# sj-shoff/ImageProcessor

Hardware: AMD Instinct MI355X
Metric: images/sec (resize+thumb+watermark) on 1080p batch at 1/2/4/8 MI355X (higher is better)
Workload: dtype f32+f64

## Files before the change

imageprocessor_amd/__init__.py:

```python
import ctypes as C

import numpy as np

from . import _lib
from ._lib import Config, Glyph, PlanInfo, PlanParams, Rect

OP_OVER = 0
DEEP_NRGBA64, DEEP_RGBA64, DEEP_GRAY16, DEEP_CMYK = 0, 1, 2, 3
PNG_GRAY, PNG_NRGBA, PNG_RGBA, PNG_PALETTED, PNG_GRAY16, PNG_RGBA64, PNG_NRGBA64 = range(7)
OP_SRC = 1
YCBCR_444, YCBCR_422, YCBCR_420, YCBCR_440, GRAY, YCBCR_411, YCBCR_410 = range(7)


class IpxError(RuntimeError):
    def __init__(self, status, text):
        super().__init__("ipx status %d: %s" % (status, text))
        self.status = status
        self.text = text


def lib():
    return _lib.load()


def _check(rc):
    if rc < 0:
        raise IpxError(rc, lib().ipx_last_error().decode(errors="replace"))
    return rc


def _rect(r):
    return r if isinstance(r, Rect) else Rect(*[int(v) for v in r])


def _bytes_array(files):
    keep = [bytes(f) for f in files]
    arr = (_lib.Bytes * max(len(keep), 1))()
    for i, f in enumerate(keep):
        arr[i].data = C.cast(C.c_char_p(f), C.c_void_p)
        arr[i].len = len(f)
    arr._keep = keep
    return arr


def _rows(a):
    a = np.asarray(a, dtype=np.uint8)
    row = int(np.prod(a.shape[1:]))
    if a.ndim < 2 or not a[:1].flags.c_contiguous or (a.shape[0] > 1 and a.strides[0] < row):
        a = np.ascontiguousarray(a)
    return a, (a.strides[0] if a.shape[0] > 1 else row)


def _frame(a):
    a, stride = _rows(a)
    if a.ndim != 3 or a.shape[2] != 4:
        raise ValueError("RGBA8 frame must be H x W x 4")
    return a, stride


def _dst(dst, shape=None):
    assert isinstance(dst, np.ndarray) and dst.dtype == np.uint8 and dst.ndim == 3 and dst.shape[2] == 4 and dst.flags.writeable
    assert shape is None or dst.shape == shape
    d, stride = _rows(dst)
    assert d is dst, "the destination's rows must be contiguous and strides[0] at least a row"
    return stride



def resize_dims(ow, oh, w, h, keep_aspect):
    nw, nh = C.c_int(), C.c_int()
    _check(lib().ipx_resize_dims(ow, oh, w, h, int(bool(keep_aspect)), C.byref(nw), C.byref(nh)))
    return nw.value, nh.value


def thumb_geometry(ow, oh, size, crop_to_fit):
    r, nw, nh = Rect(), C.c_int(), C.c_int()
    _check(lib().ipx_thumb_geometry(ow, oh, size, int(bool(crop_to_fit)), C.byref(r), C.byref(nw),
                                    C.byref(nh)))
    return (r.x0, r.y0, r.x1, r.y1), nw.value, nh.value


def text_height_px(font_size):
    return lib().ipx_text_height_px(float(font_size))


def watermark_anchor(position, w, h, width_px, height_px):
    px, py = C.c_int(), C.c_int()
    _check(lib().ipx_watermark_anchor(position.encode(), w, h, width_px, height_px, C.byref(px),
                                      C.byref(py)))
    return px.value, py.value


def parse_color(s, opacity):
    out = (C.c_uint8 * 4)()
    rc = _check(lib().ipx_parse_color(s.encode(), float(opacity), out))
    return tuple(out), rc == 1


def device_count():
    return lib().ipx_device_count()


def _glyph_array(glyphs):
    keep = []
    arr = (Glyph * max(1, len(glyphs)))()
    for i, g in enumerate(glyphs):
        m, mstride = _rows(g["mask"])
        if m.ndim != 2:
            raise ValueError("glyph mask must be mh x mw")
        keep.append(m)
        mp = g.get("mp", (0, 0))
        arr[i] = Glyph(m.ctypes.data, m.shape[1], m.shape[0], mstride, _rect(g["dr"]), int(mp[0]),
                       int(mp[1]))
    return arr, keep


def _text_array(texts):
    keep = []
    arr = (_lib.Text * max(1, len(texts)))()
    for i, (glyphs, col) in enumerate(texts):
        glyphs = list(glyphs)
        ga, gk = _glyph_array(glyphs)
        keep.append((ga, gk))
        arr[i].glyphs = ga if glyphs else None
        arr[i].n_glyphs = len(glyphs)
        for c in range(4):
            arr[i].col[c] = int(col[c])
    return arr, keep



class DevBuffer:

    def __init__(self, ctx, nbytes):
        self.ctx, self.nbytes = ctx, int(nbytes)
        self.ptr = lib().ipx_dev_alloc(ctx.handle, max(1, self.nbytes))
        if not self.ptr:
            raise IpxError(-2, lib().ipx_last_error().decode())

    def upload(self, arr, offset=0):
        arr = np.ascontiguousarray(arr)
        assert offset + arr.nbytes <= self.nbytes
        _check(lib().ipx_memcpy_h2d(self.ctx.handle, self.ptr + offset, arr.ctypes.data, arr.nbytes))
        return self

    def download(self, shape, dtype=np.uint8, offset=0):
        out = np.empty(shape, dtype)
        assert offset + out.nbytes <= self.nbytes
        _check(lib().ipx_memcpy_d2h(self.ctx.handle, out.ctypes.data, self.ptr + offset, out.nbytes))
        return out

    def free(self):
        if self.ptr:
            lib().ipx_dev_free(self.ctx.handle, self.ptr)
            self.ptr = None

    def __del__(self):
        try:
            self.free()
        except Exception:
            pass


class GlyphSet:

    def __init__(self, ctx, glyphs, col):
        self.ctx = ctx
        arr, keep = _glyph_array(list(glyphs))
        c = (C.c_uint8 * 4)(*[int(v) for v in col])
        h = C.c_void_p()
        _check(lib().ipx_glyphset_create(ctx.handle, arr, len(glyphs), c, C.byref(h)))
        self.handle = h.value

    def close(self):
        if self.handle:
            lib().ipx_glyphset_destroy(self.ctx.handle, self.handle)
            self.handle = None

    def __del__(self):
        try:
            self.close()
        except Exception:
            pass


class TextSet:

    def __init__(self, ctx, texts, w, h, stream=None):
        self.ctx = ctx
        texts = list(texts)
        arr, keep = _text_array(texts)
        hd = C.c_void_p()
        _check(lib().ipx_textset_create(ctx.handle, stream, arr, len(texts), int(w), int(h), C.byref(hd)))
        self.handle, self.n, self.w, self.h = hd.value, len(texts), int(w), int(h)

    def close(self):
        if self.handle:
            lib().ipx_textset_destroy(self.ctx.handle, self.handle)
            self.handle = None

    def __del__(self):
        try:
            self.close()
        except Exception:
            pass


class Plan:

    def __init__(self, ctx, sw, sh, resize=(1024, 768, True), thumbnail=(200, True), watermark=None):
        self.ctx = ctx
        self._sw, self._sh = sw, sh
        p = PlanParams()
        p.sw, p.sh = sw, sh
        if resize:
            p.do_resize, p.resize_w, p.resize_h, p.keep_aspect = 1, resize[0], resize[1], int(bool(resize[2]))
        if thumbnail:
            p.do_thumbnail, p.thumb_size, p.crop_to_fit = 1, thumbnail[0], int(bool(thumbnail[1]))
        self._gs = None
        if watermark is not None and watermark is not False:
            p.do_watermark = 1
            if isinstance(watermark, GlyphSet):
                self._gs = watermark
                p.glyphs = watermark.handle
        h = C.c_void_p()
        _check(lib().ipx_plan_create(ctx.handle, C.byref(p), C.byref(h)))
        self.handle = h.value
        self.info = PlanInfo()
        _check(lib().ipx_plan_query(self.handle, C.byref(self.info)))

    def _run(self, entry, head, n, src, ptrs, strides=(None, None, None)):
        i = self.info
        fs = [d if s is None else s for s, d in zip(strides, (i.resize_bytes, i.thumb_bytes, i.wm_bytes))]
        _check(entry(self.ctx.handle, *head, self.handle, n, *src, ptrs[0], fs[0], ptrs[1], fs[1], ptrs[2], fs[2]))

    def _run_host(self, entry, n, src, want, out=None):
        i = self.info
        out = dict(out) if out else {}
        for k, nbytes, h, w in (("resize", i.resize_bytes, i.resize_h, i.resize_w), ("thumbnail", i.thumb_bytes, i.thumb_h, i.thumb_w),
                                ("watermark", i.wm_bytes, i.wm_h, i.wm_w)):
            if k in want and nbytes and k not in out:
                out[k] = np.empty((n, h, w, 4), np.uint8)
        self._run(entry, (), n, src, [out[k].ctypes.data if k in out else None for k in ("resize", "thumbnail", "watermark")])
        return out

    def run_dev(self, n, src_ptr, resize_ptr=None, thumb_ptr=None, wm_ptr=None, stream=None,
                sstride=None, src_frame_stride=None, resize_frame_stride=None,
                thumb_frame_stride=None, wm_frame_stride=None):
        sstride = self._sw * 4 if sstride is None else sstride
        self._run(lib().ipx_plan_run_dev, (stream,), n,
                  (src_ptr, sstride, sstride * self._sh if src_frame_stride is None else src_frame_stride),
                  (resize_ptr, thumb_ptr, wm_ptr), (resize_frame_stride, thumb_frame_stride, wm_frame_stride))

    def run_host(self, frames, want=("resize", "thumbnail", "watermark"), out=None):
        frames = np.ascontiguousarray(frames, dtype=np.uint8)
        return self._run_host(lib().ipx_plan_run_host, frames.shape[0], (frames.ctypes.data, self._sw * 4, self._sw * self._sh * 4), want, out)

    def run_host_nrgba(self, frames, want=("resize", "thumbnail", "watermark")):
        frames = np.ascontiguousarray(frames, dtype=np.uint8)
        return self._run_host(lib().ipx_plan_run_host_nrgba, frames.shape[0], (frames.ctypes.data, self._sw * 4, self._sw * self._sh * 4), want)

    def run_host_deep(self, pix, kind, want=("resize", "thumbnail", "watermark")):
        pix = np.ascontiguousarray(pix, dtype=np.uint8)
        return self._run_host(lib().ipx_plan_run_host_deep, pix.shape[0], (kind, pix.ctypes.data, pix.shape[2], pix.shape[1] * pix.shape[2]), want)

    def run_host_gray(self, frames, want=("resize", "thumbnail", "watermark")):
        frames = np.ascontiguousarray(frames, dtype=np.uint8)
        return self._run_host(lib().ipx_plan_run_host_gray, frames.shape[0], (frames.ctypes.data, self._sw, self._sw * self._sh), want)

    def run_host_paletted(self, index, palettes, want=("resize", "thumbnail", "watermark")):
        index = np.ascontiguousarray(index, dtype=np.uint8)
        palettes = np.ascontiguousarray(palettes, dtype=np.uint8)
        n = index.shape[0]
        assert palettes.shape == (n, 256, 4)
        return self._run_host(lib().ipx_plan_run_host_paletted, n, (index.ctypes.data, self._sw, self._sw * self._sh, palettes.ctypes.data), want)

    def _run_streams(self, entry, n, want, copy, args, status=None):
        i = self.info
        arrs = {k: (_lib.Bytes * max(n, 1))() for k, present in (("resize", i.resize_bytes), ("thumbnail", i.thumb_bytes),
                                                                  ("watermark", i.wm_bytes)) if k in want and present}
        res = C.c_void_p()
        extra = () if status is None else (status,)
        _check(entry(self.ctx.handle, self.handle, n, *args, arrs.get("resize"), arrs.get("thumbnail"), arrs.get("watermark"), *extra,
                     C.byref(res)))
        out = {k: [(C.string_at(a[j].data, a[j].len) if copy else a[j].len) if a[j].data else None for j in range(n)]
               for k, a in arrs.items()}
        lib().ipx_jpeg_result_free(self.ctx.handle, res)
        return out

    def _run_files(self, entry, files, want, copy, args=()):
        n = len(files)
        status = (C.c_int * max(n, 1))()
        out = self._run_streams(entry, n, want, copy, (_bytes_array(files),) + args, status)
        return out, list(status)[:n]

    def run_host_jpeg(self, frames, quality=85, want=("resize", "thumbnail", "watermark"), copy=True):
        frames = np.ascontiguousarray(frames, dtype=np.uint8)
        return self._run_streams(lib().ipx_plan_run_host_jpeg, frames.shape[0], want, copy,
                                 (frames.ctypes.data, self._sw * 4, self._sw * self._sh * 4, int(quality)))

    def run_host_paletted_gif(self, index, palettes, quality=85, want=("resize", "thumbnail", "watermark"), copy=True):
        index = np.ascontiguousarray(index, dtype=np.uint8)
        palettes = np.ascontiguousarray(palettes, dtype=np.uint8)
        n = index.shape[0]
        assert index.shape[1:] == (self._sh, self._sw) and palettes.shape == (n, 256, 4)
        return self._run_streams(lib().ipx_plan_run_host_paletted_gif, n, want, copy,
                                 (index.ctypes.data, self._sw, self._sw * self._sh, palettes.ctypes.data, int(quality)))

    def run_host_png(self, frames, want=("resize", "thumbnail", "watermark"), copy=True):
        frames = np.ascontiguousarray(frames, dtype=np.uint8)
        assert frames.shape[1:] == (self._sh, self._sw, 4)
        return self._run_streams(lib().ipx_plan_run_host_png, frames.shape[0], want, copy,
                                 (frames.ctypes.data, self._sw * 4, self._sw * self._sh * 4))

# ... 720 lines not shown
```

imageprocessor_amd/_lib.py:

```python
import ctypes as C
import importlib.util
import os

HERE = os.path.dirname(os.path.abspath(__file__))
LIB_PATH = os.environ.get("IPX_LIB") or os.path.join(HERE, "libipx.so")


class Rect(C.Structure):
    _fields_ = [("x0", C.c_int32), ("y0", C.c_int32), ("x1", C.c_int32), ("y1", C.c_int32)]


class Glyph(C.Structure):
    _fields_ = [("mask", C.c_void_p), ("mw", C.c_int32), ("mh", C.c_int32), ("mstride", C.c_int32),
                ("dr", Rect), ("mpx", C.c_int32), ("mpy", C.c_int32)]


class Text(C.Structure):
    _fields_ = [("glyphs", C.POINTER(Glyph)), ("n_glyphs", C.c_int32), ("col", C.c_uint8 * 4)]


class Config(C.Structure):
    _fields_ = [("device", C.c_int32), ("lanes", C.c_int32), ("lane_bytes", C.c_size_t)]


class PlanParams(C.Structure):
    _fields_ = [("sw", C.c_int32), ("sh", C.c_int32),
                ("do_resize", C.c_int32), ("resize_w", C.c_int32), ("resize_h", C.c_int32),
                ("keep_aspect", C.c_int32),
                ("do_thumbnail", C.c_int32), ("thumb_size", C.c_int32), ("crop_to_fit", C.c_int32),
                ("do_watermark", C.c_int32), ("glyphs", C.c_void_p)]


class PlanInfo(C.Structure):
    _fields_ = [("resize_w", C.c_int32), ("resize_h", C.c_int32),
                ("thumb_w", C.c_int32), ("thumb_h", C.c_int32), ("thumb_crop", Rect),
                ("wm_w", C.c_int32), ("wm_h", C.c_int32),
                ("resize_bytes", C.c_size_t), ("thumb_bytes", C.c_size_t), ("wm_bytes", C.c_size_t),
                ("algorithmic_bytes", C.c_size_t)]


class YCbCr(C.Structure):
    _fields_ = [("y", C.c_void_p), ("cb", C.c_void_p), ("cr", C.c_void_p), ("ystride", C.c_int32),
                ("cstride", C.c_int32), ("w", C.c_int32), ("h", C.c_int32), ("ratio", C.c_int32)]


class YCbCrBatch(C.Structure):
    _fields_ = [("y", C.c_void_p), ("cb", C.c_void_p), ("cr", C.c_void_p), ("ystride", C.c_int32),
                ("cstride", C.c_int32), ("y_frame_stride", C.c_size_t), ("c_frame_stride", C.c_size_t),
                ("ratio", C.c_int32)]


class CmykBatch(C.Structure):
    _fields_ = [("pix", C.c_void_p), ("stride", C.c_int32), ("frame_stride", C.c_size_t)]


class PalettedBatch(C.Structure):
    _fields_ = [("index", C.c_void_p), ("stride", C.c_int32), ("frame_stride", C.c_size_t), ("palettes", C.c_void_p)]


class PngBatch(C.Structure):
    _fields_ = [("pix", C.c_void_p), ("stride", C.c_int32), ("frame_stride", C.c_size_t), ("palettes", C.c_void_p)]


class Param(C.Structure):
    _fields_ = [("key", C.c_char_p), ("type", C.c_int32), ("f64", C.c_double), ("i64", C.c_int64),
                ("str", C.c_char_p)]


class Image(C.Structure):
    _fields_ = [("pix", C.c_void_p), ("w", C.c_int32), ("h", C.c_int32), ("stride", C.c_int32)]


MEASURE_FN = C.CFUNCTYPE(C.c_int, C.c_void_p, C.c_char_p, C.c_double, C.POINTER(C.c_int))
GLYPHS_FN = C.CFUNCTYPE(C.c_int, C.c_void_p, C.c_char_p, C.c_double, C.c_int, C.c_int, C.c_int, C.c_int,
                        C.POINTER(C.POINTER(Glyph)), C.POINTER(C.c_int))
RELEASE_FN = C.CFUNCTYPE(None, C.c_void_p)


class Bytes(C.Structure):
    _fields_ = [("data", C.c_void_p), ("len", C.c_size_t)]


class TextRasterizer(C.Structure):
    _fields_ = [("user", C.c_void_p), ("measure", MEASURE_FN), ("glyphs", GLYPHS_FN), ("release", RELEASE_FN)]


class Operation(C.Structure):
    _fields_ = [("type", C.c_char_p), ("params", C.POINTER(Param)), ("nparams", C.c_int32)]


class Task(C.Structure):
    _fields_ = [("id", C.c_char_p), ("image_id", C.c_char_p), ("ops", C.POINTER(Operation)),
                ("nops", C.c_int32), ("format", C.c_char_p)]


class Processed(C.Structure):
    _fields_ = [("operation", C.c_char * 16), ("path", C.c_char * 320), ("content_type", C.c_char * 32),
                ("format", C.c_char * 8), ("image", Image)]


class PoolConfig(C.Structure):
    _fields_ = [("lanes_per_device", C.c_int32), ("lane_bytes", C.c_size_t)]


class PoolOps(C.Structure):
    _fields_ = [("sw", C.c_int32), ("sh", C.c_int32),
                ("do_resize", C.c_int32), ("resize_w", C.c_int32), ("resize_h", C.c_int32), ("keep_aspect", C.c_int32),
                ("do_thumbnail", C.c_int32), ("thumb_size", C.c_int32), ("crop_to_fit", C.c_int32),
                ("do_watermark", C.c_int32), ("glyphs", C.POINTER(Glyph)), ("n_glyphs", C.c_int32), ("col", C.c_uint8 * 4)]


class Job(C.Structure):
    _fields_ = [("kind", C.c_int32), ("ops", PoolOps), ("n", C.c_int32),
                ("src", C.c_void_p), ("sstride", C.c_int32), ("src_frame_stride", C.c_size_t),
                ("resize_out", C.c_void_p), ("resize_frame_stride", C.c_size_t),
                ("thumb_out", C.c_void_p), ("thumb_frame_stride", C.c_size_t),
                ("wm_out", C.c_void_p), ("wm_frame_stride", C.c_size_t),
                ("files", C.POINTER(Bytes)), ("quality", C.c_int32),
                ("resize_jpeg", C.POINTER(Bytes)), ("thumb_jpeg", C.POINTER(Bytes)), ("wm_jpeg", C.POINTER(Bytes)),
                ("status", C.POINTER(C.c_int32)), ("texts", C.POINTER(Text))]


class BatcherConfig(C.Structure):
    _fields_ = [("max_batch", C.c_int32), ("max_wait_us", C.c_int32), ("quality", C.c_int32)]


class BatchResult(C.Structure):
    _fields_ = [("status", C.c_int32), ("resize", Bytes), ("thumb", Bytes), ("wm", Bytes)]


class BatcherStats(C.Structure):
    _fields_ = [(k, C.c_longlong) for k in ("files", "batches", "flushed_by_size", "flushed_by_timer", "largest_batch", "pending_files", "flushed_when_idle")]


_P = C.c_void_p
_I = C.c_int
_Z = C.c_size_t

SIGNATURES = {
    "ipx_create": (_I, [C.POINTER(Config), C.POINTER(_P)]),
    "ipx_destroy": (None, [_P]),
    "ipx_last_error": (C.c_char_p, []),
    "ipx_abi_version": (_I, []),
    "ipx_device_count": (_I, []),
    "ipx_frame_supported": (_I, [_I, _I, C.c_longlong, _I]),
    "ipx_resize_dims": (_I, [_I, _I, _I, _I, _I, C.POINTER(_I), C.POINTER(_I)]),
    "ipx_thumb_geometry": (_I, [_I, _I, _I, _I, C.POINTER(Rect), C.POINTER(_I), C.POINTER(_I)]),
    "ipx_text_height_px": (_I, [C.c_double]),
    "ipx_watermark_anchor": (_I, [C.c_char_p, _I, _I, _I, _I, C.POINTER(_I), C.POINTER(_I)]),
    "ipx_parse_color": (_I, [C.c_char_p, C.c_double, _P]),
    "ipx_host_alloc": (_P, [_P, _Z]),
    "ipx_host_free": (_I, [_P, _P]),
    "ipx_dev_alloc": (_P, [_P, _Z]),
    "ipx_dev_free": (_I, [_P, _P]),
    "ipx_memcpy_h2d": (_I, [_P, _P, _P, _Z]),
    "ipx_memcpy_d2h": (_I, [_P, _P, _P, _Z]),
    "ipx_memcpy_d2d": (_I, [_P, _P, _P, _Z]),
    "ipx_stream_copy": (_I, [_P, _P, _P, _P, _Z]),
    "ipx_device_sync": (_I, [_P]),
    "ipx_stream_sync": (_I, [_P, _P]),
    "ipx_stream_create": (_P, [_P]),
    "ipx_stream_destroy": (_I, [_P, _P]),
    "ipx_scale_bilinear_rgba8": (_I, [_P, _P, _I, _I, _I, Rect, _P, _I, _I, _I, Rect, _I]),
    "ipx_draw_rgba8": (_I, [_P, _P, _I, _I, _I, Rect, _P, _I, _I, _I, _I, _I, _I]),
    "ipx_composite_glyphs_rgba8": (_I, [_P, _P, _I, _I, _I, C.POINTER(Glyph), _I, _P]),
    "ipx_scale_bilinear_nrgba8": (_I, [_P, _P, _I, _I, _I, Rect, _P, _I, _I, _I, Rect, _I]),
    "ipx_draw_nrgba8": (_I, [_P, _P, _I, _I, _I, Rect, _P, _I, _I, _I, _I, _I, _I]),
    "ipx_scale_bilinear_deep": (_I, [_P, _P, _I, _I, _I, Rect, _P, _I, _I, _I, _I, Rect, _I]),
    "ipx_draw_deep": (_I, [_P, _P, _I, _I, _I, Rect, _P, _I, _I, _I, _I, _I, _I, _I]),
    "ipx_scale_bilinear_ycbcr": (_I, [_P, _P, _I, _I, _I, Rect, C.POINTER(YCbCr), Rect]),
    "ipx_draw_ycbcr": (_I, [_P, _P, _I, _I, _I, Rect, C.POINTER(YCbCr), _I, _I]),
    "ipx_dev_scale_bilinear_rgba8": (_I, [_P, _P, _P, _I, _I, _I, Rect, _P, _I, _I, _I, Rect, _I]),
    "ipx_dev_draw_rgba8": (_I, [_P, _P, _P, _I, _I, _I, Rect, _P, _I, _I, _I, _I, _I, _I]),
    "ipx_glyphset_create": (_I, [_P, C.POINTER(Glyph), _I, _P, C.POINTER(_P)]),
    "ipx_glyphset_destroy": (None, [_P, _P]),
    "ipx_dev_composite_glyphs_rgba8": (_I, [_P, _P, _P, _I, _I, _I, _P]),
    "ipx_textset_create": (_I, [_P, _P, C.POINTER(Text), _I, _I, _I, C.POINTER(_P)]),
    "ipx_textset_destroy": (None, [_P, _P]),
    "ipx_dev_composite_texts_rgba8": (_I, [_P, _P, _P, _I, _I, _I, _Z, _I, _P, _I, C.POINTER(C.c_int32)]),
    "ipx_plan_create": (_I, [_P, C.POINTER(PlanParams), C.POINTER(_P)]),
    "ipx_plan_destroy": (None, [_P, _P]),
    "ipx_plan_query": (_I, [_P, C.POINTER(PlanInfo)]),
    "ipx_plan_run_dev": (_I, [_P, _P, _P, _I, _P, _I, _Z, _P, _Z, _P, _Z, _P, _Z]),
    "ipx_plan_run_host": (_I, [_P, _P, _I, _P, _I, _Z, _P, _Z, _P, _Z, _P, _Z]),
    "ipx_plan_run_dev_ycbcr": (_I, [_P, _P, _P, _I, C.POINTER(YCbCrBatch), _P, _Z, _P, _Z, _P, _Z]),
    "ipx_plan_run_dev_gray": (_I, [_P, _P, _P, _I, _P, _I, _Z, _P, _Z, _P, _Z, _P, _Z]),
    "ipx_plan_run_dev_paletted": (_I, [_P, _P, _P, _I, _P, _I, _Z, _P, _P, _Z, _P, _Z, _P, _Z]),
    "ipx_plan_run_host_nrgba": (_I, [_P, _P, _I, _P, _I, _Z, _P, _Z, _P, _Z, _P, _Z]),
    "ipx_plan_run_host_gray": (_I, [_P, _P, _I, _P, _I, _Z, _P, _Z, _P, _Z, _P, _Z]),
    "ipx_plan_run_host_paletted": (_I, [_P, _P, _I, _P, _I, _Z, _P, _P, _Z, _P, _Z, _P, _Z]),
    "ipx_plan_run_dev_nrgba": (_I, [_P, _P, _P, _I, _P, _I, _Z, _P, _Z, _P, _Z, _P, _Z]),
    "ipx_plan_run_dev_deep": (_I, [_P, _P, _P, _I, _I, _P, _I, _Z, _P, _Z, _P, _Z, _P, _Z]),
    "ipx_plan_run_host_deep": (_I, [_P, _P, _I, _I, _P, _I, _Z, _P, _Z, _P, _Z, _P, _Z]),
    "ipx_plan_run_host_ycbcr": (_I, [_P, _P, _I, C.POINTER(YCbCrBatch), _P, _Z, _P, _Z, _P, _Z]),
    "ipx_event_create": (_P, [_P]),
    "ipx_event_record": (_I, [_P, _P, _P]),
    "ipx_event_elapsed_ms": (_I, [_P, _P, _P, C.POINTER(C.c_float)]),
    "ipx_event_destroy": (None, [_P, _P]),
    "ipx_image_free": (None, [C.POINTER(Image)]),
    "ipx_resizer_process": (_I, [_P, C.POINTER(Image), C.c_char_p, C.POINTER(Param), _I, C.POINTER(Image), _P]),
    "ipx_thumbnailer_process": (_I, [_P, C.POINTER(Image), C.c_char_p, C.POINTER(Param), _I, C.POINTER(Image), _P]),
    "ipx_watermarker_process": (_I, [_P, C.POINTER(Image), C.c_char_p, C.POINTER(Param), _I,
                                     C.POINTER(TextRasterizer), C.POINTER(Image), _P]),
    "ipx_processor_process": (_I, [_P, C.POINTER(Task), C.POINTER(Image), C.c_char_p, C.POINTER(TextRasterizer),
                                   C.POINTER(Processed), C.POINTER(_I)]),
    "ipx_jpeg_coef_count": (_Z, [_I, _I]),
    "ipx_jpeg_quant_tables": (_I, [_I, _P]),
    "ipx_dev_jpeg_fdct_rgba8": (_I, [_P, _P, _P, _I, _I, _I, _Z, _I, _I, _P]),
    "ipx_jpeg_entropy_encode": (_I, [_P, _I, _I, _I, C.POINTER(_P), C.POINTER(_Z)]),
    "ipx_jpeg_encode_rgba8": (_I, [_P, _P, _I, _I, _I, _I, C.POINTER(_P), C.POINTER(_Z)]),
    "ipx_jpeg_encode_batch_dev": (_I, [_P, _P, _I, _I, _I, _Z, _I, _I, C.POINTER(_P), C.POINTER(_Z), C.POINTER(_Z)]),
    "ipx_buffer_free": (None, [_P]),
    "ipx_jpeg_decode_batch": (_I, [_P, _P, C.POINTER(Bytes), _I, C.POINTER(_I), C.POINTER(_I), C.POINTER(YCbCrBatch), C.POINTER(_I),
                                   C.POINTER(_P)]),
    "ipx_jpeg_planes_free": (None, [_P, _P]),
    "ipx_jpeg_scan_route": (_I, [_P, _Z, C.POINTER(_I)]),
    "ipx_jpeg_decode_counts": (_I, [_P, C.POINTER(C.c_longlong)]),
    "ipx_png_decode_counts": (_I, [_P, C.POINTER(C.c_longlong)]),
    "ipx_jpeg_decode_batch_cmyk": (_I, [_P, _P, C.POINTER(Bytes), _I, C.POINTER(_I), C.POINTER(_I), C.POINTER(CmykBatch), C.POINTER(_I),
                                        C.POINTER(_P)]),
    "ipx_jpeg_cmyk_files": (_I, [_P, C.POINTER(C.c_longlong)]),
    "ipx_plan_run_jpeg_jpeg": (_I, [_P, _P, _I, C.POINTER(Bytes), _I, C.POINTER(Bytes), C.POINTER(Bytes), C.POINTER(Bytes), C.POINTER(_I),
                                    C.POINTER(_P)]),
    "ipx_plan_run_host_jpeg": (_I, [_P, _P, _I, _P, _I, _Z, _I, C.POINTER(Bytes), C.POINTER(Bytes), C.POINTER(Bytes), C.POINTER(_P)]),
    "ipx_jpeg_result_free": (None, [_P, _P]),
    "ipx_plan_run_host_ycbcr_jpeg": (_I, [_P, _P, _I, C.POINTER(YCbCrBatch), _I, C.POINTER(Bytes), C.POINTER(Bytes), C.POINTER(Bytes),
                                          C.POINTER(_P)]),
    "ipx_gif_encode_rgba8": (_I, [_P, _P, _I, _I, _I, C.POINTER(_P), C.POINTER(_Z)]),
    "ipx_gif_encode_batch_dev": (_I, [_P, _P, _I, _I, _I, _Z, _I, C.POINTER(_P), C.POINTER(_Z), C.POINTER(_Z)]),
    "ipx_dev_gif_dither_rgba8": (_I, [_P, _P, _P, _I, _I, _I, _Z, _I, _P]),
    "ipx_plan_run_host_paletted_gif": (_I, [_P, _P, _I, _P, _I, _Z, _P, _I, C.POINTER(Bytes), C.POINTER(Bytes), C.POINTER(Bytes),
                                            C.POINTER(_P)]),
    "ipx_png_encode_rgba8": (_I, [_P, _P, _I, _I, _I, C.POINTER(_P), C.POINTER(_Z)]),
    "ipx_png_encode_batch_dev": (_I, [_P, _P, _I, _I, _I, _Z, _I, C.POINTER(_P), C.POINTER(_Z), C.POINTER(_Z)]),
    "ipx_plan_run_host_png": (_I, [_P, _P, _I, _P, _I, _Z, C.POINTER(Bytes), C.POINTER(Bytes), C.POINTER(Bytes), C.POINTER(_P)]),
    "ipx_gif_decode_batch": (_I, [_P, _P, C.POINTER(Bytes), _I, C.POINTER(_I), C.POINTER(_I), C.POINTER(PalettedBatch), C.POINTER(_I),
                                  C.POINTER(_P)]),
    "ipx_gif_frames_free": (None, [_P, _P]),
    "ipx_plan_run_gif_gif": (_I, [_P, _P, _I, C.POINTER(Bytes), _I, C.POINTER(Bytes), C.POINTER(Bytes), C.POINTER(Bytes), C.POINTER(_I),
                                  C.POINTER(_P)]),
    "ipx_png_decode_batch": (_I, [_P, _P, C.POINTER(Bytes), _I, C.POINTER(_I), C.POINTER(_I), C.POINTER(_I), C.POINTER(PngBatch),
                                  C.POINTER(_I), C.POINTER(_P)]),
    "ipx_png_frames_free": (None, [_P, _P]),
    "ipx_plan_run_png_png": (_I, [_P, _P, _I, C.POINTER(Bytes), C.POINTER(Bytes), C.POINTER(Bytes), C.POINTER(Bytes), C.POINTER(_I),
                                  C.POINTER(_P)]),
    "ipx_plan_run_jpeg_jpeg_texts": (_I, [_P, _P, _I, C.POINTER(Bytes), C.POINTER(Text), _I, C.POINTER(Bytes), C.POINTER(Bytes),
                                          C.POINTER(Bytes), C.POINTER(_I), C.POINTER(_P)]),
    "ipx_plan_run_png_png_texts": (_I, [_P, _P, _I, C.POINTER(Bytes), C.POINTER(Text), C.POINTER(Bytes), C.POINTER(Bytes), C.POINTER(Bytes),
                                        C.POINTER(_I), C.POINTER(_P)]),
    "ipx_plan_run_gif_gif_texts": (_I, [_P, _P, _I, C.POINTER(Bytes), C.POINTER(Text), _I, C.POINTER(Bytes), C.POINTER(Bytes),
                                        C.POINTER(Bytes), C.POINTER(_I), C.POINTER(_P)]),
    "ipx_font_create": (_I, [_P, _Z, C.POINTER(_P)]),
    "ipx_font_destroy": (None, [_P]),
    "ipx_font_glyph_index": (_I, [_P, C.c_uint32]),
    "ipx_font_glyph_advance": (_I, [_P, C.c_uint32, C.c_double, C.POINTER(C.c_int32)]),
    "ipx_font_kern": (_I, [_P, C.c_uint32, C.c_uint32, C.c_double, C.POINTER(C.c_int32)]),
    "ipx_font_text_width": (_I, [_P, C.c_char_p, C.c_double, C.POINTER(C.c_int32), C.POINTER(_I)]),
    "ipx_font_draw_string": (_I, [_P, C.c_char_p, C.c_double, _I, _I, _I, _I, C.POINTER(C.POINTER(Glyph)),
                                  C.POINTER(_I), C.POINTER(C.c_int32)]),
    "ipx_font_release_thread": (None, []),
    "ipx_font_rasterizer": (_I, [_P, C.POINTER(TextRasterizer)]),
    "ipx_pool_create": (_I, [C.POINTER(_I), _I, C.POINTER(PoolConfig), C.POINTER(_P)]),
    "ipx_pool_destroy": (None, [_P]),
    "ipx_pool_slots": (_I, [_P]),
    "ipx_pool_frames_done": (C.c_longlong, [_P, _I]),
    "ipx_pool_png_decode_counts": (_I, [_P, _I, C.POINTER(C.c_longlong)]),
    "ipx_pool_host_alloc": (_P, [_P, _I, _Z]),
    "ipx_pool_host_free": (_I, [_P, _I, _P]),
    "ipx_job_submit": (_I, [_P, C.POINTER(Job), C.POINTER(C.c_uint64)]),
    "ipx_job_poll": (_I, [_P, C.c_uint64, C.POINTER(_I)]),
    "ipx_job_wait": (_I, [_P, C.c_uint64, C.POINTER(_I)]),
    "ipx_job_release": (_I, [_P, C.c_uint64]),
    "ipx_pool_run_host": (_I, [_P, C.POINTER(Job), _I]),
    "ipx_plan_acquire": (_I, [_P, C.POINTER(PoolOps), C.POINTER(_P), C.POINTER(_I)]),
    "ipx_plan_release": (None, [_P, _P, _I]),
    "ipx_link_probe": (_I, [_P, _Z, _Z, _I, C.POINTER(C.c_double * 4)]),
    "ipx_batcher_create": (_I, [_P, C.POINTER(BatcherConfig), C.POINTER(_P)]),
    "ipx_batcher_destroy": (None, [_P]),
    "ipx_batcher_submit": (_I, [_P, C.POINTER(Bytes), C.POINTER(PoolOps), C.POINTER(C.c_uint64)]),
    "ipx_batcher_wait": (_I, [_P, C.c_uint64, C.POINTER(BatchResult)]),
    "ipx_batcher_release": (_I, [_P, C.c_uint64]),
    "ipx_batcher_get_stats": (_I, [_P, C.POINTER(BatcherStats)]),
}

_lib = None


def _preload_hip_runtime():
    if os.environ.get("IPX_SYSTEM_HIP") == "1":
        return
    try:
        spec = importlib.util.find_spec("torch")
    except (ImportError, ValueError):
        spec = None
    if spec is None or not spec.origin:
        return
    cand = os.path.join(os.path.dirname(spec.origin), "lib", "libamdhip64.so")
    if os.path.exists(cand):
        C.CDLL(cand, mode=C.RTLD_GLOBAL)


def load():
    global _lib
    if _lib is not None:
        return _lib
    if not os.path.exists(LIB_PATH):
        raise ImportError(
            "imageprocessor_amd: %s is missing -- build the HIP extension first "
            "(python imageprocessor_amd/build.py, or __graft_entry__.build()). "
            "There is no CPU fallback for the pixel path." % LIB_PATH)
    _preload_hip_runtime()
    L = C.CDLL(LIB_PATH)
    for name, (res, args) in SIGNATURES.items():
        fn = getattr(L, name)
        fn.restype = res
        fn.argtypes = args
    _lib = L
    return L
```

imageprocessor_amd/csrc/ipx_device.h:

```cpp
#pragma once

#include "ipx_internal.h"

namespace ipx {
namespace {

constexpr uint32_t kM = 0xffffu;

__device__ __forceinline__ uint32_t ycbcr_to_rgb8(uint32_t y, uint32_t cb, uint32_t cr)
{
    const int32_t yy1 = (int32_t)y * 0x10101, cb1 = (int32_t)cb - 128, cr1 = (int32_t)cr - 128;
    int32_t r = yy1 + 91881 * cr1, g = yy1 - 22554 * cb1 - 46802 * cr1, b = yy1 + 116130 * cb1;
    r = ((uint32_t)r & 0xff000000u) == 0 ? r >> 16 : ~(r >> 31);
    g = ((uint32_t)g & 0xff000000u) == 0 ? g >> 16 : ~(g >> 31);
    b = ((uint32_t)b & 0xff000000u) == 0 ? b >> 16 : ~(b >> 31);
    return ((uint32_t)r & 0xffu) | (((uint32_t)g & 0xffu) << 8) | (((uint32_t)b & 0xffu) << 16) | 0xff000000u;
}

template <int C>
__device__ __forceinline__ double widen(uint32_t px)
{
    constexpr uint32_t sel = 0x0c0c0000u | (uint32_t)C | ((uint32_t)C << 8);
    return (double)__builtin_amdgcn_perm(0u, px, sel);
}

template <int C>
__device__ __forceinline__ uint32_t lerp_channel(uint32_t p00, uint32_t p10, uint32_t p01,
                                                 uint32_t p11, double xw0, double xw1, double yw0,
                                                 double yw1)
{
    const double s00 = widen<C>(p00), s10 = widen<C>(p10);
    const double s01 = widen<C>(p01), s11 = widen<C>(p11);
    const double top = xw0 * s00 + xw1 * s10;
    const double bot = xw0 * s01 + xw1 * s11;
    const double v = yw0 * top + yw1 * bot;
    return (uint32_t)v;
}

__device__ __forceinline__ uint32_t pack_src(uint32_t pr, uint32_t pg, uint32_t pb, uint32_t pa)
{
    return (pr >> 8) | (pg & 0xff00u) | ((pb & 0xff00u) << 8) | ((pa & 0xff00u) << 16);
}

__device__ __forceinline__ uint32_t blend_over(uint32_t d, uint32_t pr, uint32_t pg, uint32_t pb,
                                               uint32_t pa)
{
    const uint32_t pa1 = (kM - pa) * 0x101u;
    const uint32_t r = (((d & 0xffu) * pa1 / kM + pr) >> 8) & 0xffu;
    const uint32_t g = ((((d >> 8) & 0xffu) * pa1 / kM + pg) >> 8) & 0xffu;
    const uint32_t b = ((((d >> 16) & 0xffu) * pa1 / kM + pb) >> 8) & 0xffu;
    const uint32_t a = (((d >> 24) * pa1 / kM + pa) >> 8) & 0xffu;
    return r | (g << 8) | (b << 16) | (a << 24);
}

__device__ __forceinline__ uint32_t glyph_over(uint32_t d, uint32_t mask8, uint32_t sr, uint32_t sg,
                                               uint32_t sb, uint32_t sa)
{
    const uint32_t ma = mask8 | (mask8 << 8);
    const uint32_t a = (kM - (sa * ma / kM)) * 0x101u;
    const uint32_t r = (((d & 0xffu) * a + sr * ma) / kM >> 8) & 0xffu;
    const uint32_t g = ((((d >> 8) & 0xffu) * a + sg * ma) / kM >> 8) & 0xffu;
    const uint32_t b = ((((d >> 16) & 0xffu) * a + sb * ma) / kM >> 8) & 0xffu;
    const uint32_t al = (((d >> 24) * a + sa * ma) / kM >> 8) & 0xffu;
    return r | (g << 8) | (b << 16) | (al << 24);
}

__device__ __forceinline__ uint32_t glyph_run(uint32_t d, int x, int y, const DevGlyph *__restrict__ gl,
                                              int n, uint32_t sr, uint32_t sg, uint32_t sb,
                                              uint32_t sa)
{
    for (int g = 0; g < n; g++) {
        const DevGlyph G = gl[g];
        if (x >= G.x0 && x < G.x1 && y >= G.y0 && y < G.y1) {
            const uint32_t m = G.mask[(size_t)(y - G.y0) * G.mstride + (x - G.x0)];
            if (m) d = glyph_over(d, m, sr, sg, sb, sa);
        }
    }
    return d;
}

template <int PX, int ROWS, int YSTEP>
__device__ __forceinline__ void glyph_walk(const DevGlyph *tab, int n, int x, int ybase, Rect bbox, uint32_t (&d)[ROWS][PX], uint32_t sr,
                                           uint32_t sg, uint32_t sb, uint32_t sa)
{
    static_assert(PX >= 1 && PX <= 4, "a row's mask bytes travel in one dword");
    for (int g = 0; g < n; g += 4) {
        uint32_t m[4][ROWS];
        bool any = false;
#pragma unroll
        for (int j = 0; j < 4; j++) {
            const DevGlyph G = tab[min(g + j, n - 1)];
#pragma unroll
            for (int r = 0; r < ROWS; r++) {
                const int y = ybase + YSTEP * r;
                const bool iny = g + j < n && y >= G.y0 && y < G.y1 && y < bbox.y1;
                uint32_t mm = 0u;
#pragma unroll
                for (int k = 0; k < PX; k++) {
                    const bool in = iny && x + k >= G.x0 && x + k < G.x1;
                    mm |= (in ? (uint32_t)G.mask[(size_t)(y - G.y0) * G.mstride + (x + k - G.x0)] : 0u) << (8 * k);
                    any |= in;
                }
                m[j][r] = mm;
            }
        }
        if (!__any(any)) continue;
#pragma unroll
        for (int j = 0; j < 4; j++)
#pragma unroll
            for (int r = 0; r < ROWS; r++)
#pragma unroll
                for (int k = 0; k < PX; k++) {
                    const uint32_t mk = (m[j][r] >> (8 * k)) & 0xffu;
                    if (mk) d[r][k] = glyph_over(d[r][k], mk, sr, sg, sb, sa);
                }
    }
}

}
}
```

imageprocessor_amd/csrc/ipx_host.cpp:

```cpp
#include <cmath>
#include <cstring>
#include <new>
#include <string>
#include <system_error>
#include <vector>

#include "ipx_internal.h"

namespace ipx {

static thread_local char g_err[512];

void set_error(const char *fmt, ...)
{
    va_list ap;
    va_start(ap, fmt);
    vsnprintf(g_err, sizeof g_err, fmt, ap);
    va_end(ap);
}
void clear_error() { g_err[0] = 0; }

int status_of_exception() noexcept
{
    try { throw; }
    catch (const std::bad_alloc &) { set_error("out of memory"); return IPX_ERR_NOMEM; }
    catch (const std::system_error &e) { set_error("system resource unavailable: %s", e.what()); return IPX_ERR_NOMEM; }
    catch (const std::exception &e) { set_error("internal error: %s", e.what()); return IPX_ERR_INVALID; }
    catch (...) { set_error("internal error"); return IPX_ERR_INVALID; }
}

Rect Rect::intersect(const Rect &s) const
{
    Rect r = *this;
    if (r.x0 < s.x0) r.x0 = s.x0;
    if (r.y0 < s.y0) r.y0 = s.y0;
    if (r.x1 > s.x1) r.x1 = s.x1;
    if (r.y1 > s.y1) r.y1 = s.y1;
    if (r.empty()) return Rect{0, 0, 0, 0};
    return r;
}

bool draw_clip(Rect &r, int dw, int dh, bool has_src, int sw, int sh, int &spx, int &spy,
               bool has_mask, int mw, int mh, int &mpx, int &mpy)
{
    const int ox = r.x0, oy = r.y0;
    r = r.intersect(Rect{0, 0, dw, dh});
    if (has_src) r = r.intersect(Rect{0, 0, sw, sh}.shifted(ox - spx, oy - spy));
    if (has_mask) r = r.intersect(Rect{0, 0, mw, mh}.shifted(ox - mpx, oy - mpy));
    if (r.empty()) return false;
    const int dx = r.x0 - ox, dy = r.y0 - oy;
    spx += dx; spy += dy;
    mpx += dx; mpy += dy;
    return true;
}

}

using namespace ipx;

extern "C" {

const char *ipx_last_error(void) { return g_err; }
int ipx_abi_version(void) { return IPX_ABI_VERSION; }

int ipx_frame_supported(int w, int h, long long stride, int bytes_per_pixel)
{
    clear_error();
    if (w < 0 || h < 0 || bytes_per_pixel <= 0 || stride < (long long)w * bytes_per_pixel) {
        set_error("ipx_frame_supported: bad argument");
        return IPX_ERR_INVALID;
    }
    if (frame_span_ok(w, h, stride, bytes_per_pixel)) return IPX_OK;
    set_error("a %dx%d frame (stride %lld) is beyond the 2 GiB / 65535-pixel span the kernels address", w, h, stride);
    return IPX_ERR_UNSUPPORTED;
}

int ipx_resize_dims(int ow, int oh, int w, int h, int keep_aspect, int *nw, int *nh)
{
    clear_error();
    if (!nw || !nh || ow <= 0 || oh <= 0) { set_error("ipx_resize_dims: bad argument"); return IPX_ERR_INVALID; }
    if (w <= 0 || h <= 0) { set_error("width and height must be positive numbers"); return IPX_ERR_INVALID; }
    if (keep_aspect) {
        const double wr = (double)w / (double)ow;
        const double hr = (double)h / (double)oh;
        const double ratio = std::fmin(wr, hr);
        *nw = (int)((double)ow * ratio);
        *nh = (int)((double)oh * ratio);
    } else {
        *nw = w;
        *nh = h;
    }
    return IPX_OK;
}

int ipx_thumb_geometry(int ow, int oh, int size, int crop_to_fit, ipx_rect *crop, int *nw, int *nh)
{
    clear_error();
    if (!crop || !nw || !nh || ow <= 0 || oh <= 0) { set_error("ipx_thumb_geometry: bad argument"); return IPX_ERR_INVALID; }
    if (size == 0) size = 200;
    if (size < 0) { set_error("size must be a positive number"); return IPX_ERR_INVALID; }
    if (crop_to_fit) {
        const int side = ow > oh ? oh : ow;
        const int cx = ow > oh ? (ow - oh) / 2 : 0;
        const int cy = ow > oh ? 0 : (oh - ow) / 2;
        *crop = ipx_rect{cx, cy, cx + side, cy + side};
        *nw = size;
        *nh = size;
    } else {
        *crop = ipx_rect{0, 0, ow, oh};
        if (ow > oh) {
            *nh = size;
            *nw = (int)((double)ow * (double)size / (double)oh);
        } else {
            *nw = size;
            *nh = (int)((double)oh * (double)size / (double)ow);
        }
    }
    return IPX_OK;
}

int ipx_text_height_px(double font_size)
{
    const int32_t h26_6 = (int32_t)(font_size * 64 * 1.2);
    return (h26_6 + 63) >> 6;
}

int ipx_watermark_anchor(const char *position, int w, int h, int width_px, int height_px, int *px,
                         int *py)
{
    clear_error();
    if (!position || !px || !py) { set_error("ipx_watermark_anchor: bad argument"); return IPX_ERR_INVALID; }
    enum { L, R, C } hx = R;
    enum { T, B, M } vy = B;
    const std::string p(position);
    if (p == "top-left") { hx = L; vy = T; }
    else if (p == "top-right") { hx = R; vy = T; }
    else if (p == "top-center") { hx = C; vy = T; }
    else if (p == "bottom-left") { hx = L; vy = B; }
    else if (p == "bottom-center") { hx = C; vy = B; }
    else if (p == "center") { hx = C; vy = M; }
    const int margin = 20;
    *px = hx == L ? margin : hx == R ? w - width_px - margin : (w - width_px) / 2;
    *py = vy == T ? margin + height_px : vy == B ? h - margin : (h + height_px) / 2;
    return IPX_OK;
}

static bool atoi_field(const std::string &f, long long *v)
{
    size_t i = 0;
    bool neg = false;
    if (f.empty()) return false;
    if (f[0] == '+' || f[0] == '-') { neg = f[0] == '-'; i = 1; }
    if (i == f.size()) return false;
    long long acc = 0;
    for (; i < f.size(); i++) {
        if (f[i] < '0' || f[i] > '9') return false;
        if (acc > 900000000000000000LL) return false;
        acc = acc * 10 + (f[i] - '0');
    }
    *v = neg ? -acc : acc;
    return true;
}

int ipx_parse_color(const char *s, double opacity, uint8_t rgba[4])
{
    clear_error();
    if (!s || !rgba) { set_error("ipx_parse_color: bad argument"); return IPX_ERR_INVALID; }
    const uint8_t alpha = (uint8_t)(int32_t)(255 * opacity);
    std::vector<std::string> parts(1);
    for (const char *c = s; *c; c++) {
        if (*c == ' ') continue;
        if (*c == ',') parts.emplace_back();
        else parts.back().push_back(*c);
    }
    long long v[4] = {0, 0, 0, 0};
    bool ok = parts.size() == 3 || parts.size() == 4;
    for (int i = 0; ok && i < 3; i++) ok = atoi_field(parts[i], &v[i]);
    if (!ok) {
        rgba[0] = rgba[1] = rgba[2] = 0;
        rgba[3] = alpha;
        return 1;
    }
    for (int i = 0; i < 3; i++) rgba[i] = (uint8_t)(v[i] < 0 ? 0 : v[i] > 255 ? 255 : v[i]);
    if (parts.size() == 4 && atoi_field(parts[3], &v[3])) rgba[3] = (uint8_t)(v[3] < 0 ? 0 : v[3] > 255 ? 255 : v[3]);
    else rgba[3] = alpha;
    return IPX_OK;
}

}
```

imageprocessor_amd/csrc/ipx_internal.h:

```cpp
#pragma once

#include <hip/hip_runtime.h>

#include <cstdarg>
#include <cstdint>
#include <cstdio>
#include <map>
#include <mutex>
#include <vector>

#include "../../include/ipx.h"

namespace ipx {

void set_error(const char *fmt, ...) __attribute__((format(printf, 1, 2)));
void clear_error();
int status_of_exception() noexcept;
#define IPX_CATCH_STATUS catch (...) { return ipx::status_of_exception(); }

#define IPX_HIP(call)                                                                        \
    do {                                                                                     \
        hipError_t e_ = (call);                                                              \
        if (e_ != hipSuccess) {                                                              \
            ipx::set_error("%s failed: %s (%s:%d)", #call, hipGetErrorString(e_), __FILE__,  \
                           __LINE__);                                                        \
            return IPX_ERR_HIP;                                                              \
        }                                                                                    \
    } while (0)

constexpr long long kMaxFrameSpan = 0x7fff0000LL;
constexpr int kMaxFrameSide = 65535;
inline bool frame_span_ok(long long w, long long h, long long stride, int bpp)
{
    if (w > kMaxFrameSide || h > kMaxFrameSide) return false;
    return w <= 0 || h <= 0 || (h - 1) * stride + w * bpp <= kMaxFrameSpan;
}

struct Rect {
    int x0, y0, x1, y1;
    int dx() const { return x1 - x0; }
    int dy() const { return y1 - y0; }
    bool empty() const { return x0 >= x1 || y0 >= y1; }
    Rect shifted(int ox, int oy) const { return Rect{x0 + ox, y0 + oy, x1 + ox, y1 + oy}; }
    Rect intersect(const Rect &s) const;
};
inline Rect to_rect(const ipx_rect &r) { return Rect{r.x0, r.y0, r.x1, r.y1}; }

bool draw_clip(Rect &r, int dw, int dh, bool has_src, int sw, int sh, int &spx, int &spy,
               bool has_mask, int mw, int mh, int &mpx, int &mpy);

enum SrcType { kSrcRGBA, kSrcNRGBA, kSrcGray, kSrcPaletted, kSrcYCbCr, kSrcNRGBA64, kSrcRGBA64, kSrcGray16, kSrcCMYK, kSrcTypes };
inline int src_bpp(int type) { static const int b[kSrcTypes] = {4, 4, 1, 1, 1, 8, 8, 2, 4}; return b[type]; }
inline int src_of_deep(int k) { return k >= IPX_DEEP_NRGBA64 && k <= IPX_DEEP_CMYK ? kSrcNRGBA64 + k : -1; }
inline int src_of_png(int k)
{
    static const int t[] = {kSrcGray, kSrcNRGBA, kSrcRGBA, kSrcPaletted, kSrcGray16, kSrcRGBA64, kSrcNRGBA64};
    return k >= 0 && k < 7 ? t[k] : -1;
}
inline int src_of_job(int k)
{
    static const int t[] = {kSrcRGBA, -1, kSrcNRGBA, kSrcGray, kSrcNRGBA64, kSrcRGBA64, kSrcGray16, kSrcCMYK};
    return k >= 0 && k < 8 ? t[k] : -1;
}
inline void chroma_size(int ratio, int w, int h, int *cw, int *ch)
{
    *cw = ratio == IPX_YCBCR_422 || ratio == IPX_YCBCR_420 ? (w + 1) / 2 : ratio == IPX_YCBCR_411 || ratio == IPX_YCBCR_410 ? (w + 3) / 4 : w;
    *ch = ratio == IPX_YCBCR_420 || ratio == IPX_YCBCR_440 || ratio == IPX_YCBCR_410 ? (h + 1) / 2 : h;
}
inline bool ycbcr_ratio_ok(int ratio) { return (ratio >= IPX_YCBCR_444 && ratio <= IPX_YCBCR_440) || ratio == IPX_YCBCR_411 || ratio == IPX_YCBCR_410; }
#if defined(__HIPCC__)
__host__ __device__
#endif
inline int ycbcr_hshift(int ratio) { return ratio == IPX_YCBCR_422 || ratio == IPX_YCBCR_420 ? 1 : ratio == IPX_YCBCR_411 || ratio == IPX_YCBCR_410 ? 2 : 0; }
#if defined(__HIPCC__)
__host__ __device__
#endif
inline int ycbcr_vshift(int ratio) { return ratio == IPX_YCBCR_420 || ratio == IPX_YCBCR_440 || ratio == IPX_YCBCR_410 ? 1 : 0; }
inline int ycbcr_ratio_of(int h0, int v0)
{
    return h0 == 4 ? (v0 == 1 ? IPX_YCBCR_411 : IPX_YCBCR_410) : h0 == 1 ? (v0 == 1 ? IPX_YCBCR_444 : IPX_YCBCR_440) : (v0 == 1 ? IPX_YCBCR_422 : IPX_YCBCR_420);
}

enum { IPX_SRC_RGBA = 0, IPX_SRC_NRGBA = 1, IPX_SRC_YCBCR = 2,
       IPX_SRC_TAP64 = 3  };
hipError_t launch_opaque_scan(const uint8_t *src, int sw, int sh, int sstride, int *flag,
                              hipStream_t s);
hipError_t launch_opaque_scan_tap64(const uint8_t *src, int sw, int sh, int sstride, int *flag, hipStream_t s);
hipError_t launch_draw(uint8_t *dst, int dstride, const uint8_t *src, int sstride, int w, int h,
                       int op, hipStream_t s);
hipError_t launch_draw_nrgba(uint8_t *dst, int dstride, const uint8_t *src, int sstride, int w, int h, int op,
                             hipStream_t s, int nframes = 1, size_t dst_fs = 0, size_t src_fs = 0);
hipError_t launch_deep_expand(uint8_t *dst, size_t dst_fs, const uint8_t *src, int sstride, size_t src_fs, int kind, int w, int h, int nframes, hipStream_t s);
hipError_t launch_draw_tap64(uint8_t *dst, int dstride, const uint8_t *src, int sstride, int w, int h, int op, hipStream_t s,
                             int nframes = 1, size_t dst_fs = 0, size_t src_fs = 0);
hipError_t launch_draw_ycbcr(uint8_t *dst, int dstride, const uint8_t *y, int ystride, const uint8_t *cb,
                             const uint8_t *cr, int cstride, int ratio, int spx, int spy, int w, int h, hipStream_t s,
                             int nframes = 1, size_t dst_fs = 0, size_t y_fs = 0, size_t c_fs = 0);

struct DevGlyph {
    const uint8_t *mask;
    int mstride;
    int x0, y0, x1, y1;
};
constexpr int kMaxGlyphs = 256;
hipError_t launch_stream_copy(void *dst, const void *src, size_t bytes, hipStream_t s);
hipError_t launch_composite(uint8_t *dst, int dstride, size_t frame_stride, int nframes,
                            const DevGlyph *glyphs_dev, int n, Rect bbox, uint32_t sr, uint32_t sg,
                            uint32_t sb, uint32_t sa, hipStream_t s);
struct DevText {
    int first, n;
    Rect bbox;
    uint16_t col[4];
};
hipError_t launch_composite_texts(uint8_t *dst, int dstride, size_t frame_stride, int nframes, const DevText *texts_dev,
                                  const DevGlyph *glyphs_dev, const int *map_dev, int first, int bw, int bh, hipStream_t s);

hipError_t launch_gray_expand(uint8_t *dst, size_t dst_fs, const uint8_t *src, int sstride, size_t src_fs, int w, int h, int n, hipStream_t s);
hipError_t launch_palette_expand(uint8_t *dst, size_t dst_fs, const uint8_t *src, int sstride, size_t src_fs, const uint8_t *palettes, int w,
                                 int h, int n, hipStream_t s);

struct KernelLaunchCache {
    std::mutex mu;
    size_t lds_max = 0;
    std::map<size_t, int> resident;
    bool said = false;
    hipError_t prepare(const void *fn, int threads, size_t lds, int *res)
    {
        std::lock_guard<std::mutex> lk(mu);
        if (lds > lds_max) {
            hipError_t e = hipFuncSetAttribute(fn, hipFuncAttributeMaxDynamicSharedMemorySize, (int)lds);
            if (e != hipSuccess) return e;
            lds_max = lds;
        }
        if (res) {
            auto it = resident.find(lds);
            if (it == resident.end()) {
                int n = 0;
                hipError_t e = hipOccupancyMaxActiveBlocksPerMultiprocessor(&n, fn, threads, lds);
                if (e != hipSuccess) return e;
                it = resident.emplace(lds, n > 1 ? n : 1).first;
            }
            *res = it->second;
        }
        return hipSuccess;
    }
    bool first_report() { std::lock_guard<std::mutex> lk(mu); const bool f = !said; said = true; return f; }
};


struct JpegTables {
    uint8_t quant[2][64];
    uint16_t div8[2][64];
    uint32_t recip[2][64];
};
void jpeg_tables(int quality, JpegTables *t);
struct JpegArgs {
    const uint8_t *src; size_t frame_stride; int stride, w, h;
    int aligned16;
    int16_t *coefs; int mcus_per_frame;
    const uint32_t *huff;
    uint32_t *aclen;
    int16_t *dcq;
    uint32_t recip[2][64];
    uint16_t div8[2][64];
};
hipError_t launch_jpeg_fdct(const JpegArgs &a, int n, hipStream_t s);


struct JpegDecInfo {
    int w, h, h0, v0, ratio, ri, ncomp;
    int host_scans;
    int progressive;
    int gpu_scans;
    uint8_t td[3], ta[3];
    size_t scan_off, scan_len;
};
struct JpegDecTables {
    uint16_t lut[4][256];
    int32_t maxcode[4][18];
    int32_t valoff[4][18];
    uint8_t vals[4][256];
    uint16_t qnat[3][64];
    uint32_t bound[4][8];
};
struct JpegDecImage {
    unsigned long long scan_off; uint32_t scan_len, img, first_mcu, n_mcu;
    uint8_t td[3], ta[3], valid, pad;
    uint8_t strict_end, rsv[3];
    unsigned long long uoff;
    uint32_t tab_img, rsv2;
};
struct JpegDecArgs {
    const uint8_t *blob; const JpegDecImage *img; const JpegDecTables *tab;
    int16_t *coefs; int *status;
    int16_t *dcs;
    int n, mxx, myy, h0, v0, nblk;
    int w, h;
    int bpm, ybl;
    int nitems;
    int shared_tables, first_valid;
};
#if defined(__HIPCC__)
__host__ __device__
#endif
inline int jpeg_status_key(uint32_t first_mcu, int status) { return -(int)(((0x3ffffffu - (first_mcu & 0x3ffffffu)) << 3) | (uint32_t)(-status)); }
constexpr uint32_t kJpegStatusLast = 0x3ffffffu;
inline int jpeg_status_of(int key) { return key >= 0 ? 0 : -(int)((uint32_t)(-key) & 7u); }
struct JpegPlanes { uint8_t *y, *cb, *cr; int ystride, cstride; size_t y_fs, c_fs; const uint8_t *valid;  };
struct JpegParImage { unsigned long long scan_off; uint32_t scan_len, img, nsub; size_t sub_off; uint8_t td[3], ta[3], pad[2]; };
struct JpegParArgs {
    const uint8_t *blob; const JpegDecTables *tab; const JpegParImage *img;
    uint8_t *ublob;
    int nimg, max_nsub, bpm, ybl, nblk;
    int stage_rows;
    int sub;
    uint32_t *stuffed;
    uint32_t *scan_end, *ulen;
    unsigned long long *entry, *exit_a, *exit_b;
    unsigned long long *ck_state; uint32_t *ck_ends;
    uint32_t *ends, *total_ends;
    uint32_t *changed;
    int16_t *coefs; int *status;
    int16_t *dcs;
};
int jpeg_par_sub_bytes();
int jpeg_par_checkpoints();
hipError_t launch_par_count(const JpegParArgs &a, hipStream_t s);
hipError_t launch_par_unstuff(const JpegParArgs &a, hipStream_t s);
hipError_t launch_par_sync(const JpegParArgs &a, int round, hipStream_t s);
hipError_t launch_par_write(const JpegParArgs &a, hipStream_t s);
hipError_t launch_par_dc(const JpegParArgs &a, hipStream_t s);
int jpeg_parse(const uint8_t *d, size_t len, JpegDecInfo *info, JpegDecTables *tab, bool cmyk = false, bool s411 = false);
int jpeg_host_decode(const uint8_t *d, size_t len, JpegDecInfo *info, int16_t *coefs, int16_t *dcs, size_t nblk, uint16_t qnat[3][64],
                     bool *progressive, bool s411 = false, int *alone = nullptr);
int jpeg_host_decode4(const uint8_t *d, size_t len, JpegDecInfo *info, int16_t *coefs, int16_t *dcs, size_t nblk, uint16_t qnat[4][64],
                      bool *progressive, int *transform);
constexpr int IPX_JPEG_PROG_MAX_SCANS = 64;
struct JpegProgHuff {
    uint16_t look[512];
    int32_t mincode[17], maxcode[17], valptr[17];
    uint8_t vals[256];
    int32_t ncodes;
};
static_assert(sizeof(JpegProgHuff) % 16 == 0, "copied to LDS in 16-byte units");
struct JpegProgScan {
    uint32_t off, len;
    uint8_t ns, ss, se, ah, al;
    uint8_t comp[3];
    uint16_t dc_def[3], ac_def[3];
    uint32_t rsv;
};
struct JpegProgFile { unsigned long long blob_off; uint32_t img, nscans, scan0, def0; };
struct JpegProgPlan {
    std::vector<JpegProgScan> scans;
    std::vector<JpegProgHuff> defs;
};
struct JpegProgArgs {
    const uint8_t *blob; const JpegProgFile *files; const JpegProgScan *scans; const JpegProgHuff *defs;
    int16_t *coefs, *dcs; int *status;
    int nfiles, mxx, myy, h0, v0, nblk, w, h, bpm, ybl;
// ... 51 lines not shown
```

imageprocessor_amd/csrc/ipx_kernels.hip:

```cpp
#include <algorithm>

#include "ipx_internal.h"

#pragma clang fp contract(off)

#include "ipx_device.h"

namespace ipx {

namespace {

__global__ __launch_bounds__(256) void opaque_scan_kernel(const uint8_t *src, int sw, int sh,
                                                          int sstride, int *flag)
{
    const int y = blockIdx.y;
    bool bad = false;
    for (int x = blockIdx.x * 256 + threadIdx.x; x < sw; x += gridDim.x * 256)
        bad |= src[(size_t)y * sstride + (size_t)x * 4 + 3] != 0xff;
    if (__any(bad) && (threadIdx.x & 63) == 0) atomicAnd(flag, 0);
}

__global__ __launch_bounds__(256) void opaque_scan_tap64_kernel(const uint8_t *src, int sw, int sh, int sstride, int *flag)
{
    const int y = blockIdx.y;
    bool bad = false;
    for (int x = blockIdx.x * 256 + threadIdx.x; x < sw; x += gridDim.x * 256)
        bad |= *(const uint16_t *)(src + (size_t)y * sstride + (size_t)x * 8 + 6) != 0xffffu;
    if (__any(bad) && (threadIdx.x & 63) == 0) atomicAnd(flag, 0);
}

__global__ __launch_bounds__(256) void draw_src_vec_kernel(uint4 *__restrict__ dst, int dstride,
                                                           const uint4 *__restrict__ src,
                                                           int sstride, int wchunks, int h)
{
    const int y = blockIdx.y;
    if (y >= h) return;
    const uint4 *s = (const uint4 *)((const uint8_t *)src + (size_t)y * sstride);
    uint4 *d = (uint4 *)((uint8_t *)dst + (size_t)y * dstride);
    for (int i = blockIdx.x * 256 + threadIdx.x; i < wchunks; i += gridDim.x * 256) d[i] = s[i];
}

__global__ __launch_bounds__(256) void draw_px_kernel(uint8_t *dst, int dstride, const uint8_t *src,
                                                      int sstride, int w, int h, int op)
{
    const int y = blockIdx.y;
    if (y >= h) return;
    for (int x = blockIdx.x * 256 + threadIdx.x; x < w; x += gridDim.x * 256) {
        const uint32_t s = *(const uint32_t *)(src + (size_t)y * sstride + (size_t)x * 4);
        uint32_t *dp = (uint32_t *)(dst + (size_t)y * dstride + (size_t)x * 4);
        if (op == IPX_OP_SRC) { *dp = s; continue; }
        const uint32_t d = *dp;
        const uint32_t sa = (s >> 24) * 0x101u;
        const uint32_t al = (kM - sa) * 0x101u;
        const uint32_t r = (((d & 0xffu) * al / kM + (s & 0xffu) * 0x101u) >> 8) & 0xffu;
        const uint32_t g = ((((d >> 8) & 0xffu) * al / kM + ((s >> 8) & 0xffu) * 0x101u) >> 8) & 0xffu;
        const uint32_t b = ((((d >> 16) & 0xffu) * al / kM + ((s >> 16) & 0xffu) * 0x101u) >> 8) & 0xffu;
        const uint32_t a = (((d >> 24) * al / kM + sa) >> 8) & 0xffu;
        *dp = r | (g << 8) | (b << 16) | (a << 24);
    }
}

__global__ __launch_bounds__(256) void draw_nrgba_kernel(uint8_t *dst, int dstride, const uint8_t *src,
                                                         int sstride, int w, int h, int op, size_t dst_fs, size_t src_fs)
{
    const int y = blockIdx.y;
    if (y >= h) return;
    dst += blockIdx.z * dst_fs; src += blockIdx.z * src_fs;
    for (int x = blockIdx.x * 256 + threadIdx.x; x < w; x += gridDim.x * 256) {
        const uint32_t s = *(const uint32_t *)(src + (size_t)y * sstride + (size_t)x * 4);
        uint32_t *dp = (uint32_t *)(dst + (size_t)y * dstride + (size_t)x * 4);
        const uint32_t sa = (s >> 24) * 0x101u;
        const uint32_t sr = (s & 0xffu) * sa / 0xffu, sg = ((s >> 8) & 0xffu) * sa / 0xffu, sb = ((s >> 16) & 0xffu) * sa / 0xffu;
        if (op == IPX_OP_SRC) { *dp = (sr >> 8) | (sg & 0xff00u) | ((sb & 0xff00u) << 8) | ((sa & 0xff00u) << 16); continue; }
        const uint32_t d = *dp;
        const uint32_t al = (kM - sa) * 0x101u;
        const uint32_t r = (((d & 0xffu) * al / kM + sr) >> 8) & 0xffu;
        const uint32_t g = ((((d >> 8) & 0xffu) * al / kM + sg) >> 8) & 0xffu;
        const uint32_t b = ((((d >> 16) & 0xffu) * al / kM + sb) >> 8) & 0xffu;
        const uint32_t a = (((d >> 24) * al / kM + sa) >> 8) & 0xffu;
        *dp = r | (g << 8) | (b << 16) | (a << 24);
    }
}

__device__ __forceinline__ uint32_t be16x2(uint32_t v) { return __builtin_amdgcn_perm(0u, v, 0x02030001u); }
template <int KIND>
__global__ __launch_bounds__(256) void deep_expand_kernel(uint8_t *dst, size_t dst_fs, const uint8_t *src, int sstride, size_t src_fs, int w, int h)
{
    const int y = blockIdx.y;
    dst += blockIdx.z * dst_fs; src += blockIdx.z * src_fs;
    const uint8_t *row = src + (size_t)y * sstride;
    uint2 *out = (uint2 *)(dst + (size_t)y * w * 8);
    for (int x = blockIdx.x * 256 + threadIdx.x; x < w; x += gridDim.x * 256) {
        uint2 o;
        if (KIND == IPX_DEEP_GRAY16) {
            const uint32_t v = (uint32_t)row[2 * x] << 8 | row[2 * x + 1];
            o.x = v | v << 16; o.y = v | 0xffff0000u;
        } else if (KIND == IPX_DEEP_CMYK) {
            const uint32_t p = *(const uint32_t *)(row + (size_t)x * 4);
            const uint32_t wk = 0xffffu - (p >> 24) * 0x101u;
            const uint32_t r = (0xffffu - (p & 0xffu) * 0x101u) * wk / 0xffffu, g = (0xffffu - ((p >> 8) & 0xffu) * 0x101u) * wk / 0xffffu,
                           b = (0xffffu - ((p >> 16) & 0xffu) * 0x101u) * wk / 0xffffu;
            o.x = r | g << 16; o.y = b | 0xffff0000u;
        } else {
            const uint16_t *p = (const uint16_t *)(row + (size_t)x * 8);
            const uint32_t rg = be16x2((uint32_t)p[0] | (uint32_t)p[1] << 16), ba = be16x2((uint32_t)p[2] | (uint32_t)p[3] << 16);
            if (KIND == IPX_DEEP_NRGBA64) {
                const uint32_t a = ba >> 16;
                const uint32_t r = (rg & 0xffffu) * a / 0xffffu, g = (rg >> 16) * a / 0xffffu, b = (ba & 0xffffu) * a / 0xffffu;
                o.x = r | g << 16; o.y = b | a << 16;
            } else { o.x = rg; o.y = ba; }
        }
        out[x] = o;
    }
}

__global__ __launch_bounds__(256) void draw_tap64_kernel(uint8_t *dst, int dstride, const uint8_t *src, int sstride, int w, int h, int op,
                                                         size_t dst_fs, size_t src_fs)
{
    const int y = blockIdx.y;
    if (y >= h) return;
    dst += blockIdx.z * dst_fs; src += blockIdx.z * src_fs;
    for (int x = blockIdx.x * 256 + threadIdx.x; x < w; x += gridDim.x * 256) {
        const uint2 t = *(const uint2 *)(src + (size_t)y * sstride + (size_t)x * 8);
        uint32_t *dp = (uint32_t *)(dst + (size_t)y * dstride + (size_t)x * 4);
        if (op == IPX_OP_SRC) { *dp = __builtin_amdgcn_perm(t.y, t.x, 0x07050301u); continue; }
        const uint32_t d = *dp;
        const uint32_t sr = t.x & 0xffffu, sg = t.x >> 16, sb = t.y & 0xffffu, sa = t.y >> 16;
        const uint32_t al = (kM - sa) * 0x101u;
        const uint32_t r = ((((d & 0xffu) * al + sr * kM) / kM) >> 8) & 0xffu;
        const uint32_t g = (((((d >> 8) & 0xffu) * al + sg * kM) / kM) >> 8) & 0xffu;
        const uint32_t b = (((((d >> 16) & 0xffu) * al + sb * kM) / kM) >> 8) & 0xffu;
        const uint32_t a = ((((d >> 24) * al + sa * kM) / kM) >> 8) & 0xffu;
        *dp = r | (g << 8) | (b << 16) | (a << 24);
    }
}

__global__ __launch_bounds__(256) void draw_ycbcr_kernel(uint8_t *dst, int dstride, const uint8_t *yp, int ystride,
                                                         const uint8_t *cb, const uint8_t *cr, int cstride, int ratio,
                                                         int spx, int spy, int w, int h, size_t dst_fs, size_t y_fs,
                                                         size_t c_fs)
{
    const int y = blockIdx.y;
    if (y >= h) return;
    dst += blockIdx.z * dst_fs; yp += blockIdx.z * y_fs; cb += blockIdx.z * c_fs; cr += blockIdx.z * c_fs;
    const int hs = ycbcr_hshift(ratio), vs = ycbcr_vshift(ratio);
    for (int x = blockIdx.x * 256 + threadIdx.x; x < w; x += gridDim.x * 256) {
        const int sx = spx + x, sy = spy + y;
        const int cx = sx >> hs, cy = sy >> vs;
        const size_t ci = (size_t)cy * cstride + cx;
        const int32_t yy1 = (int32_t)yp[(size_t)sy * ystride + sx] * 0x10101;
        const int32_t cb1 = (int32_t)cb[ci] - 128, cr1 = (int32_t)cr[ci] - 128;
        int32_t r = yy1 + 91881 * cr1, g = yy1 - 22554 * cb1 - 46802 * cr1, b = yy1 + 116130 * cb1;
        r = ((uint32_t)r & 0xff000000u) == 0 ? r >> 16 : ~(r >> 31);
        g = ((uint32_t)g & 0xff000000u) == 0 ? g >> 16 : ~(g >> 31);
        b = ((uint32_t)b & 0xff000000u) == 0 ? b >> 16 : ~(b >> 31);
        *(uint32_t *)(dst + (size_t)y * dstride + (size_t)x * 4) =
            ((uint32_t)r & 0xffu) | (((uint32_t)g & 0xffu) << 8) | (((uint32_t)b & 0xffu) << 16) | 0xff000000u;
    }
}

constexpr int kCompositeRows = 4;
__global__ __launch_bounds__(256) void composite_kernel(uint8_t *dst, int dstride, size_t frame_stride,
                                                        const DevGlyph *__restrict__ gl, int n,
                                                        Rect bbox, uint32_t sr, uint32_t sg,
                                                        uint32_t sb, uint32_t sa)
{
    __shared__ DevGlyph tab[kMaxGlyphs];
    const int lt = (int)(threadIdx.y * 64 + threadIdx.x);
    const int x = bbox.x0 + (int)(blockIdx.x * 64 + threadIdx.x);
    const int ybase = bbox.y0 + (int)(blockIdx.y * (4 * kCompositeRows) + threadIdx.y);
    uint8_t *frame = dst + blockIdx.z * frame_stride;
    uint32_t d[kCompositeRows][1], d0[kCompositeRows];
#pragma unroll
    for (int r = 0; r < kCompositeRows; r++) {
        const int y = ybase + 4 * r;
        d0[r] = d[r][0] = x < bbox.x1 && y < bbox.y1 ? *(const uint32_t *)(frame + (size_t)y * dstride + (size_t)x * 4) : 0u;
    }
    for (int g = lt; g < n; g += 256) tab[g] = gl[g];
    __syncthreads();
    glyph_walk<1, kCompositeRows, 4>(tab, n, x, ybase, bbox, d, sr, sg, sb, sa);
#pragma unroll
    for (int r = 0; r < kCompositeRows; r++) {
        const int y = ybase + 4 * r;
        if (x < bbox.x1 && y < bbox.y1 && d[r][0] != d0[r]) *(uint32_t *)(frame + (size_t)y * dstride + (size_t)x * 4) = d[r][0];
    }
}

__global__ __launch_bounds__(256) void composite_texts_kernel(uint8_t *dst, int dstride, size_t frame_stride,
                                                              const DevText *__restrict__ texts, const DevGlyph *__restrict__ glyphs,
                                                              const int *__restrict__ map, int first)
{
    __shared__ DevGlyph tab[kMaxGlyphs];
    const DevText T = texts[map ? map[blockIdx.z] : first + (int)blockIdx.z];
    const Rect bbox = T.bbox;
    if ((int)(blockIdx.x * 64) >= bbox.x1 - bbox.x0 || (int)(blockIdx.y * (4 * kCompositeRows)) >= bbox.y1 - bbox.y0) return;
    const DevGlyph *gl = glyphs + T.first;
    const int n = T.n;
    const uint32_t sr = T.col[0], sg = T.col[1], sb = T.col[2], sa = T.col[3];
    const int lt = (int)(threadIdx.y * 64 + threadIdx.x);
    const int x = bbox.x0 + (int)(blockIdx.x * 64 + threadIdx.x);
    const int ybase = bbox.y0 + (int)(blockIdx.y * (4 * kCompositeRows) + threadIdx.y);
    uint8_t *frame = dst + blockIdx.z * frame_stride;
    uint32_t d[kCompositeRows][1], d0[kCompositeRows];
#pragma unroll
    for (int r = 0; r < kCompositeRows; r++) {
        const int y = ybase + 4 * r;
        d0[r] = d[r][0] = x < bbox.x1 && y < bbox.y1 ? *(const uint32_t *)(frame + (size_t)y * dstride + (size_t)x * 4) : 0u;
    }
    for (int g = lt; g < n; g += 256) tab[g] = gl[g];
    __syncthreads();
    glyph_walk<1, kCompositeRows, 4>(tab, n, x, ybase, bbox, d, sr, sg, sb, sa);
#pragma unroll
    for (int r = 0; r < kCompositeRows; r++) {
        const int y = ybase + 4 * r;
        if (x < bbox.x1 && y < bbox.y1 && d[r][0] != d0[r]) *(uint32_t *)(frame + (size_t)y * dstride + (size_t)x * 4) = d[r][0];
    }
}

}

hipError_t launch_draw_nrgba(uint8_t *dst, int dstride, const uint8_t *src, int sstride, int w, int h, int op,
                             hipStream_t s, int nframes, size_t dst_fs, size_t src_fs)
{
    if (w <= 0 || h <= 0 || nframes <= 0) return hipSuccess;
    dim3 grid(min(8, (w + 255) / 256), h, nframes);
    hipLaunchKernelGGL(draw_nrgba_kernel, grid, dim3(256), 0, s, dst, dstride, src, sstride, w, h, op, dst_fs, src_fs);
    return hipGetLastError();
}

hipError_t launch_deep_expand(uint8_t *dst, size_t dst_fs, const uint8_t *src, int sstride, size_t src_fs, int kind, int w, int h, int nframes, hipStream_t s)
{
    if (w <= 0 || h <= 0 || nframes <= 0) return hipSuccess;
    dim3 grid(min(2, (w + 255) / 256), h, nframes);
    switch (kind) {
    case IPX_DEEP_NRGBA64: hipLaunchKernelGGL(deep_expand_kernel<IPX_DEEP_NRGBA64>, grid, dim3(256), 0, s, dst, dst_fs, src, sstride, src_fs, w, h); break;
    case IPX_DEEP_RGBA64: hipLaunchKernelGGL(deep_expand_kernel<IPX_DEEP_RGBA64>, grid, dim3(256), 0, s, dst, dst_fs, src, sstride, src_fs, w, h); break;
    case IPX_DEEP_GRAY16: hipLaunchKernelGGL(deep_expand_kernel<IPX_DEEP_GRAY16>, grid, dim3(256), 0, s, dst, dst_fs, src, sstride, src_fs, w, h); break;
    case IPX_DEEP_CMYK: hipLaunchKernelGGL(deep_expand_kernel<IPX_DEEP_CMYK>, grid, dim3(256), 0, s, dst, dst_fs, src, sstride, src_fs, w, h); break;
    default: return hipErrorInvalidValue;
    }
    return hipGetLastError();
}

hipError_t launch_draw_tap64(uint8_t *dst, int dstride, const uint8_t *src, int sstride, int w, int h, int op, hipStream_t s, int nframes,
                             size_t dst_fs, size_t src_fs)
{
    if (w <= 0 || h <= 0 || nframes <= 0) return hipSuccess;
    dim3 grid(min(2, (w + 255) / 256), h, nframes);
    hipLaunchKernelGGL(draw_tap64_kernel, grid, dim3(256), 0, s, dst, dstride, src, sstride, w, h, op, dst_fs, src_fs);
    return hipGetLastError();
}

__global__ __launch_bounds__(256) void gray_expand_kernel(uint8_t *dst, size_t dst_fs, const uint8_t *src, int sstride, size_t src_fs, int w, int h)
{
    const int y = blockIdx.y;
    dst += blockIdx.z * dst_fs; src += blockIdx.z * src_fs;
    const uint8_t *row = src + (size_t)y * sstride;
    uint32_t *out = (uint32_t *)(dst + (size_t)y * w * 4);
    for (int x = blockIdx.x * 256 + threadIdx.x; x < w; x += gridDim.x * 256) out[x] = (uint32_t)row[x] * 0x010101u | 0xff000000u;
}

hipError_t launch_gray_expand(uint8_t *dst, size_t dst_fs, const uint8_t *src, int sstride, size_t src_fs, int w, int h, int n, hipStream_t s)
{
    hipLaunchKernelGGL(gray_expand_kernel, dim3(std::min(8, (w + 255) / 256), h, n), dim3(256), 0, s, dst, dst_fs, src, sstride, src_fs, w, h);
    return hipGetLastError();
}

__global__ __launch_bounds__(256) void palette_expand_kernel(uint8_t *dst, size_t dst_fs, const uint8_t *src, int sstride, size_t src_fs,
                                                             const uint32_t *palettes, int w, int h, int rows_per_block, int vec)
{
    __shared__ uint32_t pal[256];
    pal[threadIdx.x] = palettes[(size_t)blockIdx.y * 256 + threadIdx.x];
    __syncthreads();
    dst += blockIdx.y * dst_fs; src += blockIdx.y * src_fs;
    const int y0 = blockIdx.x * rows_per_block, y1 = min(h, y0 + rows_per_block);
    for (int y = y0; y < y1; y++) {
        const uint8_t *row = src + (size_t)y * sstride;
        uint32_t *out = (uint32_t *)(dst + (size_t)y * w * 4);
        if (vec) {
            for (int c = threadIdx.x; c < (w >> 2); c += 256) {
                const uint32_t i4 = ((const uint32_t *)row)[c];
                ((uint4 *)out)[c] = make_uint4(pal[i4 & 0xffu], pal[(i4 >> 8) & 0xffu], pal[(i4 >> 16) & 0xffu], pal[i4 >> 24]);
            }
        } else {
            for (int x = threadIdx.x; x < w; x += 256) out[x] = pal[row[x]];
        }
    }
}

hipError_t launch_palette_expand(uint8_t *dst, size_t dst_fs, const uint8_t *src, int sstride, size_t src_fs, const uint8_t *palettes, int w,
                                 int h, int n, hipStream_t s)
{
    const int rows = 8;
    const int vec = !(w & 3) && !((((uintptr_t)src) | (uintptr_t)sstride | src_fs) & 3) && !((((uintptr_t)dst) | dst_fs) & 15);
    hipLaunchKernelGGL(palette_expand_kernel, dim3((h + rows - 1) / rows, n), dim3(256), 0, s, dst, dst_fs, src, sstride, src_fs,
                       (const uint32_t *)palettes, w, h, rows, vec);
    return hipGetLastError();
}

hipError_t launch_draw_ycbcr(uint8_t *dst, int dstride, const uint8_t *y, int ystride, const uint8_t *cb,
                             const uint8_t *cr, int cstride, int ratio, int spx, int spy, int w, int h, hipStream_t s,
                             int nframes, size_t dst_fs, size_t y_fs, size_t c_fs)
{
    if (w <= 0 || h <= 0 || nframes <= 0) return hipSuccess;
    dim3 grid(min(8, (w + 255) / 256), h, nframes);
    hipLaunchKernelGGL(draw_ycbcr_kernel, grid, dim3(256), 0, s, dst, dstride, y, ystride, cb, cr, cstride, ratio, spx,
                       spy, w, h, dst_fs, y_fs, c_fs);
    return hipGetLastError();
}

hipError_t launch_opaque_scan(const uint8_t *src, int sw, int sh, int sstride, int *flag,
                              hipStream_t s)
{
    hipError_t e = hipMemsetAsync(flag, 1, sizeof(int), s);
    if (e != hipSuccess) return e;
    if (sw <= 0 || sh <= 0) return hipSuccess;
    dim3 grid(min(8, (sw + 255) / 256), sh);
    hipLaunchKernelGGL(opaque_scan_kernel, grid, dim3(256), 0, s, src, sw, sh, sstride, flag);
    return hipGetLastError();
}

hipError_t launch_opaque_scan_tap64(const uint8_t *src, int sw, int sh, int sstride, int *flag, hipStream_t s)
{
    hipError_t e = hipMemsetAsync(flag, 1, sizeof(int), s);
    if (e != hipSuccess) return e;
    if (sw <= 0 || sh <= 0) return hipSuccess;
    dim3 grid(min(8, (sw + 255) / 256), sh);
    hipLaunchKernelGGL(opaque_scan_tap64_kernel, grid, dim3(256), 0, s, src, sw, sh, sstride, flag);
    return hipGetLastError();
}

hipError_t launch_draw(uint8_t *dst, int dstride, const uint8_t *src, int sstride, int w, int h,
                       int op, hipStream_t s)
{
    if (w <= 0 || h <= 0) return hipSuccess;
    const bool vec = op == IPX_OP_SRC && (w & 3) == 0 &&
                     ((((uintptr_t)dst) | ((uintptr_t)src) | (uintptr_t)dstride | (uintptr_t)sstride) & 15) == 0;
    if (vec) {
        const int wc = w / 4;
        dim3 grid(min(8, (wc + 255) / 256), h);
        hipLaunchKernelGGL(draw_src_vec_kernel, grid, dim3(256), 0, s, (uint4 *)dst, dstride,
                           (const uint4 *)src, sstride, wc, h);
    } else {
        dim3 grid(min(8, (w + 255) / 256), h);
        hipLaunchKernelGGL(draw_px_kernel, grid, dim3(256), 0, s, dst, dstride, src, sstride, w, h, op);
    }
    return hipGetLastError();
}

__global__ __launch_bounds__(256) void stream_copy_kernel(const uint4 *__restrict__ s, uint4 *__restrict__ d, size_t n)
{
    const size_t per = (n + gridDim.x - 1) / gridDim.x;
    const size_t i0 = (size_t)blockIdx.x * per, i1 = i0 + per < n ? i0 + per : n;
    size_t i = i0 + threadIdx.x;
    for (; i + 768 < i1; i += 1024) {
        const uint4 a = s[i], b = s[i + 256], c = s[i + 512], e = s[i + 768];
        d[i] = a; d[i + 256] = b; d[i + 512] = c; d[i + 768] = e;
    }
    for (; i < i1; i += 256) d[i] = s[i];
}

hipError_t launch_stream_copy(void *dst, const void *src, size_t bytes, hipStream_t s)
{
    const size_t n = bytes / 16;
    const unsigned blocks = (unsigned)std::min<size_t>(2048, (n + 255) / 256);
    hipLaunchKernelGGL(stream_copy_kernel, dim3(blocks), dim3(256), 0, s, (const uint4 *)src, (uint4 *)dst, n);
    return hipGetLastError();
}

hipError_t launch_composite(uint8_t *dst, int dstride, size_t frame_stride, int nframes,
                            const DevGlyph *glyphs_dev, int n, Rect bbox, uint32_t sr, uint32_t sg,
                            uint32_t sb, uint32_t sa, hipStream_t s)
{
    if (n <= 0 || bbox.empty() || nframes <= 0) return hipSuccess;
    dim3 block(64, 4), grid((bbox.dx() + 63) / 64, (bbox.dy() + 4 * kCompositeRows - 1) / (4 * kCompositeRows), nframes);
    hipLaunchKernelGGL(composite_kernel, grid, block, 0, s, dst, dstride, frame_stride, glyphs_dev, n,
                       bbox, sr, sg, sb, sa);
    return hipGetLastError();
}

hipError_t launch_composite_texts(uint8_t *dst, int dstride, size_t frame_stride, int nframes, const DevText *texts_dev,
                                  const DevGlyph *glyphs_dev, const int *map_dev, int first, int bw, int bh, hipStream_t s)
{
    if (nframes <= 0 || bw <= 0 || bh <= 0) return hipSuccess;
    dim3 block(64, 4), grid((bw + 63) / 64, (bh + 4 * kCompositeRows - 1) / (4 * kCompositeRows), nframes);
    hipLaunchKernelGGL(composite_texts_kernel, grid, block, 0, s, dst, dstride, frame_stride, texts_dev, glyphs_dev, map_dev, first);
    return hipGetLastError();
}

}
```

imageprocessor_amd/csrc/ipx_ks.h:

```cpp
#pragma once

#include <vector>

#include "ipx_internal.h"

namespace ipx {

struct KsAxis {
    int dw = 0, sw = 0;
    int ntap = 0;
    std::vector<int32_t> lo, cnt;
    std::vector<double> w;
    std::vector<double> itw, itwffff;
    std::vector<double> ones;
};
bool ks_build_axis(int dw, int sw, KsAxis *out);

struct KsAxisDev {
    const int32_t *lo, *cnt;
    const double *w, *itw, *itwffff, *ones;
    int ntap;
};
size_t ks_axis_bytes(const KsAxis &a);
void ks_axis_pack(const KsAxis &a, uint8_t *h, const uint8_t *d, KsAxisDev *out);

enum {
    IPX_SRC_RGBA_CROP = 8,
    IPX_SRC_NRGBA_CROP = 9,
    IPX_SRC_YCBCR_CROP = 10,
    IPX_SRC_TAP64_CROP = 11
};
inline int ks_crop_kind(int kind)
{
    return kind == IPX_SRC_NRGBA ? IPX_SRC_NRGBA_CROP : kind == IPX_SRC_YCBCR ? IPX_SRC_YCBCR_CROP : kind == IPX_SRC_TAP64 ? IPX_SRC_TAP64_CROP
                                                                                                                           : IPX_SRC_RGBA_CROP;
}

struct KsGenArgs {
    uint8_t *dst; int dstride; size_t dst_fs;
    int dr_x0, dr_y0;
    int adr_x0, adr_y0, adr_x1, adr_y1;
    int sr_x0, sr_y0;
    KsAxisDev ax, ay;
    int op;
    const int *opaque_flag;
    int kind;
    const uint8_t *src; int sstride; size_t src_fs;
    const uint8_t *cb, *cr; int cstride, ratio; size_t c_fs;
    int nframes;
    int src_w;
};
hipError_t launch_ks_generic(const KsGenArgs &a, hipStream_t s);

}

namespace ipx {

struct KsStrip { int c0, c1, t0, tw; };
struct KsSeg { int ys, r0, r1; };
template <int NACC> struct KsRowT { double w[NACC], itw[NACC], ones[NACC]; int32_t emit[NACC]; float wf[NACC]; };
static_assert(sizeof(KsRowT<2>) == 64 && sizeof(KsRowT<4>) == 128, "row entries are copied dword-wise");

struct KsFusedOut {
    uint8_t *out; size_t frame_stride; int ostride, obytes;
    int dw, dh, sr_x0, sr_y0;
    int kind;
    int mode, aone;
    int pk;
    int ntap;
    int waves, cpl;
    int wcols;
    const double *wx;
    const float *wxf;
    int split, ntapf;
    float feps;
    const double *itwf;
    const int32_t *xlo;
    const int32_t *colb;
    const void *rows;
    const int32_t *rowoff;
};
struct KsFusedArgs {
    const uint8_t *src; size_t src_fs; int sstride, sw, sh;
    int src_kind;
    int taps_le_alpha;
    const uint8_t *cb, *cr; int cstride, ratio; size_t c_fs;
    uint8_t *wm; size_t wm_fs; int wm_stride;
    int nframes, nstrips, nseg, nthreads, pitch, dbuf;
    const KsStrip *strips; const KsSeg *segs;
    int nout; KsFusedOut o[2];
    int lds_w[2], lds_rows, lds_open;
    int open_per_wave;
    uint8_t wave_role[16];
    unsigned long long *stamps;
    int *redo;
    uint2 *fix; int *fix_count; int fix_cap[2], fix_stride;
};
struct KsText { const DevGlyph *gl; int n; Rect bbox; uint32_t sr, sg, sb, sa; };
struct KsFix { uint2 *list = nullptr; int *count = nullptr; int cap[2] = {0, 0}; KsAxisDev ax[2], ay[2]; };
struct KsFusedGeom { int nseg = 0; const KsSeg *segs = nullptr; const void *rows[2] = {nullptr, nullptr}; const int32_t *rowoff[2] = {nullptr, nullptr}; };
struct KsFusedPlan {
    bool ok = false;
    int nacc = 2, rows = 4, pitch = 0, nstrips = 0, nthreads = 0, nstg = 0, dbuf = 0;
    int lds_w[2] = {0, 0}, lds_rows = 0, lds_open = 0, lds_bytes = 0;
    struct Lds { int dbuf = 0, lds_w[2] = {0, 0}, lds_rows = 0, lds_open = 0, open_per_wave = 0, lds_bytes = 0; } fast;
    const KsStrip *strips = nullptr;
    struct Out { int ntap = 0, waves = 0, cpl = 0, wcols = 0; const double *wx = nullptr, *itwf = nullptr; const int32_t *xlo = nullptr, *colb = nullptr;
                 const float *wxf = nullptr; float feps = 0; int split = 1, ntapf = 0; } o[2];
    KsFusedGeom whole, split;
};
constexpr int kKsSplitRows = 96;
constexpr int kKsRows = 4;
constexpr int kKsMaxStage = 3;
constexpr int kKsMaxWaves = 12;
constexpr int kKsMaxThreads = 64 * kKsMaxWaves;
constexpr int kKsMaxCpl = 2;
constexpr int kKsSplitTaps = 16;
constexpr int kKsOpenPerWave = 128;
struct KsFusedIn { int dw, dh, sr_x0, sr_y0; const KsAxis *hx, *hy; int top_taps = 0; };
bool ks_fused_plan(int sw, int sh, const KsFusedIn *sc0, const KsFusedIn *sc1, int px_bytes, std::vector<uint8_t> *blob, KsFusedPlan *out);
void ks_fused_rebase(KsFusedPlan *p, const uint8_t *dev_blob);
hipError_t launch_ks_fused(const KsFusedPlan &p, KsFusedArgs &a, const KsFix *fix, const KsText *text, int cus, hipStream_t s, bool *matched, bool *text_done);
hipError_t launch_ks_fix(const KsGenArgs &g, const uint2 *list, size_t list_stride, const int *count, int count_stride, int cap, hipStream_t s);

struct KsTailArgs {
    KsGenArgs g[2];
    const uint2 *list[2]; const int *count[2]; int cap[2];
    size_t list_stride; int count_stride;
    int nframes;
    int R[2], chunks[2];
    uint8_t *wm; int wm_stride; size_t wm_fs;
    KsText text;
    int tbx, tby;
};
hipError_t launch_ks_tail(KsTailArgs t, hipStream_t s);

}
```

imageprocessor_amd/csrc/ipx_ks_tail.hip:

```cpp
#include <algorithm>
#include <cstdlib>

#include "ipx_ks_exact.h"

namespace ipx {
namespace {

constexpr int kTailThreads = 256;
constexpr int kTextRows = 4;

template <int KIND>
__device__ __forceinline__ void tail_exact(KsGenArgs a, const uint2 *list, size_t list_stride, const int *count, int count_stride, int cap, int R,
                                           int frame, int chunk, int chunks)
{
    const int n = min(count[(size_t)frame * count_stride], cap);
    list += (size_t)frame * list_stride;
    a.dst += frame * a.dst_fs;
    a.src += frame * a.src_fs;
    if (KIND == IPX_SRC_YCBCR || KIND == IPX_SRC_YCBCR_CROP) { a.cb += frame * a.c_fs; a.cr += frame * a.c_fs; }
    const int lane = (int)threadIdx.x & 63, wv = (int)threadIdx.x >> 6;
    const int per_wave = 64 / R, sub = lane / R, sl = lane - sub * R, per_block = (kTailThreads >> 6) * per_wave;
    ks_exact_list<KIND>(a, list, n, chunk * per_block, chunks * per_block, wv * per_wave + sub, R, sub, sl);
}

__device__ __forceinline__ void tail_text(const KsTailArgs &t, DevGlyph *tab, int f, int rb)
{
    const int by = rb / t.tbx, bx = rb - by * t.tbx;
    const Rect bbox = t.text.bbox;
    const int n = t.text.n;
    const int x = bbox.x0 + bx * 64 + ((int)threadIdx.x & 63);
    const int ybase = bbox.y0 + by * (4 * kTextRows) + ((int)threadIdx.x >> 6);
    uint8_t *frame = t.wm + (size_t)f * t.wm_fs;
    uint32_t d[kTextRows][1], d0[kTextRows];
#pragma unroll
    for (int r = 0; r < kTextRows; r++) {
        const int y = ybase + 4 * r;
        d0[r] = d[r][0] = x < bbox.x1 && y < bbox.y1 ? *(const uint32_t *)(frame + (size_t)y * t.wm_stride + (size_t)x * 4) : 0u;
    }
    for (int g = (int)threadIdx.x; g < n; g += kTailThreads) tab[g] = t.text.gl[g];
    __syncthreads();
    glyph_walk<1, kTextRows, 4>(tab, n, x, ybase, bbox, d, t.text.sr, t.text.sg, t.text.sb, t.text.sa);
#pragma unroll
    for (int r = 0; r < kTextRows; r++) {
        const int y = ybase + 4 * r;
        if (x < bbox.x1 && y < bbox.y1 && d[r][0] != d0[r]) *(uint32_t *)(frame + (size_t)y * t.wm_stride + (size_t)x * 4) = d[r][0];
    }
}

template <int K0, int K1>
__global__ __launch_bounds__(kTailThreads) void ks_tail_kernel(KsTailArgs t)
{
    __shared__ DevGlyph tab[kMaxGlyphs];
    const int nx = t.chunks[0] + t.chunks[1], per = nx + t.tbx * t.tby, b = (int)blockIdx.x;
    const int frame = b / per, c = b - frame * per;
    if (c < nx) {
        const int k = c >= t.chunks[0] ? 1 : 0, chunk = c - (k ? t.chunks[0] : 0);
        if (K0 == K1 || k == 0)
            tail_exact<K0>(k ? t.g[1] : t.g[0], t.list[k], t.list_stride, t.count[k], t.count_stride, t.cap[k], t.R[k], frame, chunk, t.chunks[k]);
        else
            tail_exact<K1>(t.g[1], t.list[1], t.list_stride, t.count[1], t.count_stride, t.cap[1], t.R[1], frame, chunk, t.chunks[1]);
        return;
    }
    tail_text(t, tab, frame, c - nx);
}

template <int K0, int K1>
void tail_go(const KsTailArgs &t, unsigned blocks, hipStream_t s)
{
    hipLaunchKernelGGL((ks_tail_kernel<K0, K1>), dim3(blocks), dim3(kTailThreads), 0, s, t);
}

template <int S, int C>
bool tail_pair(int k0, int k1, const KsTailArgs &t, unsigned blocks, hipStream_t s)
{
    if (k0 == S && k1 == S) tail_go<S, S>(t, blocks, s);
    else if (k0 == S && k1 == C) tail_go<S, C>(t, blocks, s);
    else if (k0 == C && k1 == C) tail_go<C, C>(t, blocks, s);
    else return false;
    return true;
}

}

hipError_t launch_ks_tail(KsTailArgs t, hipStream_t s)
{
    if (t.nframes <= 0) return hipSuccess;
    const char *ev = getenv("IPX_KS_TAIL_BLOCKS");
    const int budget = ev && atoi(ev) > 0 ? atoi(ev) : 2048;
    for (int k = 0; k < 2; k++) {
        t.R[k] = 8; t.chunks[k] = 0;
        if (!t.list[k] || t.cap[k] <= 0) { t.cap[k] = 0; continue; }
        const int ntap = t.g[k].ay.ntap;
        t.R[k] = ntap <= 4 ? 4 : ntap <= 8 ? 8 : ntap <= 16 ? 16 : 64;
        const int per_block = (kTailThreads / 64) * (64 / t.R[k]), most = (t.cap[k] + per_block - 1) / per_block;
        t.chunks[k] = std::max(1, std::min(most, std::max(1, budget / t.nframes)));
    }
    const bool text = t.wm && t.text.gl && t.text.n > 0 && !t.text.bbox.empty();
    if (!text) t.text.n = 0;
    t.tbx = text ? (t.text.bbox.dx() + 63) / 64 : 0;
    t.tby = text ? (t.text.bbox.dy() + 4 * kTextRows - 1) / (4 * kTextRows) : 0;
    const long long blocks = (long long)t.nframes * (t.chunks[0] + t.chunks[1]) + (long long)t.nframes * t.tbx * t.tby;
    if (blocks <= 0) return hipSuccess;
    if (blocks > 0x7fffffffLL) return hipErrorInvalidValue;
    const int k0 = t.chunks[0] ? t.g[0].kind : t.g[1].kind, k1 = t.chunks[1] ? t.g[1].kind : k0;
    const bool none = !t.chunks[0] && !t.chunks[1];
    if (none) { tail_go<IPX_SRC_RGBA, IPX_SRC_RGBA>(t, (unsigned)blocks, s); return hipGetLastError(); }
    if (!tail_pair<IPX_SRC_RGBA, IPX_SRC_RGBA_CROP>(k0, k1, t, (unsigned)blocks, s) && !tail_pair<IPX_SRC_NRGBA, IPX_SRC_NRGBA_CROP>(k0, k1, t, (unsigned)blocks, s) &&
        !tail_pair<IPX_SRC_YCBCR, IPX_SRC_YCBCR_CROP>(k0, k1, t, (unsigned)blocks, s) && !tail_pair<IPX_SRC_TAP64, IPX_SRC_TAP64_CROP>(k0, k1, t, (unsigned)blocks, s))
        return hipErrorInvalidValue;
    return hipGetLastError();
}

}
```

imageprocessor_amd/csrc/ipx_runtime.hip:

```cpp
#include <algorithm>
#include <chrono>
#include <condition_variable>
#include <cstdlib>
#include <cstring>
#include <map>
#include <mutex>
#include <new>
#include <thread>
#include <utility>
#include <vector>

#include "ipx_runtime_internal.h"
#include "ipx_ks.h"

#ifndef IPX_DIAG
#define IPX_DIAG 0
#endif

namespace {

struct ScalePrep {
    bool empty;
    Rect adr;
};
// ... 21 lines not shown
    if (it != ctx->ks_axes.end()) { *out = it->second.second; return IPX_OK; }
    KsAxis ax;
    if (!ks_build_axis(dw, sw, &ax)) { set_error("scale: cannot tabulate an axis of %d <- %d", dw, sw); return IPX_ERR_INVALID; }
    if (ctx->ks_axes.size() >= kMaxKsAxes) {
        IPX_HIP(hipDeviceSynchronize());
        for (auto &e : ctx->ks_axes) (void)hipFree(e.second.first);
        ctx->ks_axes.clear();
    }
    const size_t bytes = ks_axis_bytes(ax);
    std::vector<uint8_t> h(bytes);
    uint8_t *d = nullptr;
    IPX_HIP(hipMalloc((void **)&d, bytes));
    KsAxisDev dev;
    ks_axis_pack(ax, h.data(), d, &dev);
    hipError_t e = hipMemcpy(d, h.data(), bytes, hipMemcpyHostToDevice);
    if (e != hipSuccess) { (void)hipFree(d); set_error("axis table upload failed: %s", hipGetErrorString(e)); return IPX_ERR_HIP; }
    ctx->ks_axes[{dw, sw}] = {d, dev};
    *out = dev;
    return IPX_OK;
}

struct DevSrc {
    int kind = IPX_SRC_RGBA;
    const uint8_t *pix = nullptr;
    int stride = 0;
    const uint8_t *cb = nullptr, *cr = nullptr;
    int cstride = 0, ratio = 0;
    int w = 0, h = 0;
    int nframes = 1;
    size_t frame_stride = 0, c_frame_stride = 0;
    bool le_alpha = false;
};

int dev_draw_src(hipStream_t s, uint8_t *dst, int dw, int dh, int dstride, Rect r, const DevSrc &src, int spx,
                 int spy, int op, size_t dst_fs = 0)
{
    if (op != IPX_OP_OVER && op != IPX_OP_SRC) { set_error("draw: unknown op %d", op); return IPX_ERR_INVALID; }
    int mx = 0, my = 0;
    if (!draw_clip(r, dw, dh, true, src.w, src.h, spx, spy, false, 0, 0, mx, my)) return IPX_OK;
    uint8_t *d = dst + (size_t)r.y0 * dstride + (size_t)r.x0 * 4;
    if (src.kind == IPX_SRC_YCBCR)
        IPX_HIP(launch_draw_ycbcr(d, dstride, src.pix, src.stride, src.cb, src.cr, src.cstride, src.ratio, spx, spy,
                                  r.dx(), r.dy(), s, src.nframes, dst_fs, src.frame_stride, src.c_frame_stride));
    else if (src.kind == IPX_SRC_NRGBA)
        IPX_HIP(launch_draw_nrgba(d, dstride, src.pix + (size_t)spy * src.stride + (size_t)spx * 4, src.stride, r.dx(),
                                  r.dy(), op, s, src.nframes, dst_fs, src.frame_stride));
    else if (src.kind == IPX_SRC_TAP64)
        IPX_HIP(launch_draw_tap64(d, dstride, src.pix + (size_t)spy * src.stride + (size_t)spx * 8, src.stride, r.dx(), r.dy(), op, s,
                                  src.nframes, dst_fs, src.frame_stride));
    else
        for (int i = 0; i < std::max(1, src.nframes); i++)
            IPX_HIP(launch_draw(d + (size_t)i * dst_fs, dstride, src.pix + (size_t)i * src.frame_stride + (size_t)spy * src.stride + (size_t)spx * 4,
                                src.stride, r.dx(), r.dy(), op, s));
    return IPX_OK;
}

int dev_scale_src(ipx_ctx *ctx, hipStream_t s, int *flag, uint8_t *dst, int dw, int dh, int dstride, const Rect &dr,
                  const DevSrc &src, const Rect &sr, int op, size_t dst_fs = 0, int kind_override = -1, const KsAxisDev *axes = nullptr)
{
    ScalePrep pr;
    int rc = scale_prepare(dw, dh, dr, src.w, src.h, sr, op, &pr);
    if (rc) return rc;
    if (pr.empty) return IPX_OK;
    if (src.kind == IPX_SRC_YCBCR) op = IPX_OP_SRC;
    if (op == IPX_OP_OVER && src.kind == IPX_SRC_TAP64) IPX_HIP(launch_opaque_scan_tap64(src.pix, src.w, src.h, src.stride, flag, s));
    else if (op == IPX_OP_OVER) IPX_HIP(launch_opaque_scan(src.pix, src.w, src.h, src.stride, flag, s));
    KsGenArgs a{};
    if (axes) { a.ax = axes[0]; a.ay = axes[1]; }
    else {
        if ((rc = ks_axis_get(ctx, dr.dx(), sr.dx(), &a.ax))) return rc;
        if ((rc = ks_axis_get(ctx, dr.dy(), sr.dy(), &a.ay))) return rc;
    }
    a.dst = dst; a.dstride = dstride; a.src = src.pix; a.sstride = src.stride;
    a.dr_x0 = dr.x0; a.dr_y0 = dr.y0;
    a.adr_x0 = pr.adr.x0; a.adr_y0 = pr.adr.y0; a.adr_x1 = pr.adr.x1; a.adr_y1 = pr.adr.y1;
    a.sr_x0 = sr.x0; a.sr_y0 = sr.y0;
    a.op = op; a.opaque_flag = op == IPX_OP_OVER ? flag : nullptr;
    a.kind = kind_override >= 0 ? kind_override : src.kind;
    a.cb = src.cb; a.cr = src.cr; a.cstride = src.cstride; a.ratio = src.ratio;
    a.nframes = src.nframes; a.src_fs = src.frame_stride; a.c_fs = src.c_frame_stride; a.dst_fs = dst_fs;
    IPX_HIP(launch_ks_generic(a, s));
    return IPX_OK;
}

DevSrc rgba_src(const uint8_t *p, int w, int h, int stride, int kind = IPX_SRC_RGBA)
{
    DevSrc d;
    d.kind = kind; d.pix = p; d.stride = stride; d.w = w; d.h = h;
    return d;
}

int dev_draw(hipStream_t s, uint8_t *dst, int dw, int dh, int dstride, Rect r, const uint8_t *src,
             int sw, int sh, int sstride, int spx, int spy, int op)
{
    return dev_draw_src(s, dst, dw, dh, dstride, r, rgba_src(src, sw, sh, sstride), spx, spy, op);
}

int dev_scale(ipx_ctx *ctx, hipStream_t s, int *flag, uint8_t *dst, int dw, int dh, int dstride, const Rect &dr,
              const uint8_t *src, int sw, int sh, int sstride, const Rect &sr, int op)
{
    return dev_scale_src(ctx, s, flag, dst, dw, dh, dstride, dr, rgba_src(src, sw, sh, sstride), sr, op);
}

Rect clip_glyphs(const GlyphHost *g, size_t n, const uint8_t *masks_dev, int dw, int dh, std::vector<DevGlyph> *tab)
{
    Rect bb{0, 0, 0, 0};
    const size_t before = tab->size();
    for (size_t i = 0; i < n; i++) {
        Rect r = g[i].dr;
        int spx = 0, spy = 0, mpx = g[i].mpx, mpy = g[i].mpy;
        if (!draw_clip(r, dw, dh, false, 0, 0, spx, spy, true, g[i].mw, g[i].mh, mpx, mpy)) continue;
        DevGlyph d;
        d.mask = masks_dev + g[i].mask_off + (size_t)mpy * g[i].mw + mpx;
        d.mstride = g[i].mw;
        d.x0 = r.x0; d.y0 = r.y0; d.x1 = r.x1; d.y1 = r.y1;
        if (tab->size() == before) bb = r;
        else {
            bb.x0 = std::min(bb.x0, r.x0); bb.y0 = std::min(bb.y0, r.y0);
            bb.x1 = std::max(bb.x1, r.x1); bb.y1 = std::max(bb.y1, r.y1);
        }
        tab->push_back(d);
    }
    return bb;
}

bool pack_glyph(const ipx_glyph &g, std::vector<uint8_t> *blob, GlyphHost *h)
{
    if (g.mw < 0 || g.mh < 0 || (g.mw && g.mh && (!g.mask || g.mstride < g.mw))) return false;
    h->mask_off = blob->size();
    h->mw = g.mw; h->mh = g.mh; h->dr = to_rect(g.dr); h->mpx = g.mpx; h->mpy = g.mpy;
    for (int y = 0; y < g.mh; y++) blob->insert(blob->end(), g.mask + (size_t)y * g.mstride, g.mask + (size_t)y * g.mstride + g.mw);
    return true;
}

int glyphs_for_frame(const ipx_glyphset *gs, int dw, int dh, ClippedGlyphs *out)
{
    std::lock_guard<std::mutex> lk(gs->mu);
    auto it = gs->clipped.find({dw, dh});
    if (it != gs->clipped.end()) { *out = it->second; return IPX_OK; }
    std::vector<DevGlyph> tab;
    const Rect bb = clip_glyphs(gs->g.data(), gs->g.size(), gs->masks_dev, dw, dh, &tab);
    ClippedGlyphs c;
    c.n = (int)tab.size();
    c.bbox = bb;
    if (c.n) {
        IPX_HIP(hipMalloc((void **)&c.dev, tab.size() * sizeof(DevGlyph)));
        IPX_HIP(hipMemcpy(c.dev, tab.data(), tab.size() * sizeof(DevGlyph), hipMemcpyHostToDevice));
    }
    gs->clipped[{dw, dh}] = c;
    *out = c;
    return IPX_OK;
}

int dev_composite(hipStream_t s, uint8_t *dst, int dw, int dh, int dstride, size_t frame_stride,
                  int nframes, const ipx_glyphset *gs)
{
    ClippedGlyphs c;
    int rc = glyphs_for_frame(gs, dw, dh, &c);
    if (rc) return rc;
    IPX_HIP(launch_composite(dst, dstride, frame_stride, nframes, c.dev, c.n, c.bbox,
                             gs->col[0] * 0x101u, gs->col[1] * 0x101u, gs->col[2] * 0x101u,
                             gs->col[3] * 0x101u, s));
    return IPX_OK;
}

}

int texts_check(const char *who, const ipx_text *texts, int n)
{
    if (n < 0 || (n && !texts)) { set_error("%s: bad text list", who); return IPX_ERR_INVALID; }
    for (int t = 0; t < n; t++) {
        const ipx_text &x = texts[t];
        if (x.n_glyphs < 0 || (x.n_glyphs && !x.glyphs)) { set_error("%s: text %d has a bad glyph list", who, t); return IPX_ERR_INVALID; }
        if (x.n_glyphs > kMaxGlyphs) { set_error("%s: text %d has %d glyphs, the limit is %d", who, t, x.n_glyphs, kMaxGlyphs); return IPX_ERR_UNSUPPORTED; }
        for (int i = 0; i < x.n_glyphs; i++) {
            const ipx_glyph &g = x.glyphs[i];
            if (g.mw < 0 || g.mh < 0 || (g.mw && g.mh && (!g.mask || g.mstride < g.mw))) { set_error("%s: glyph %d of text %d has a bad mask", who, i, t); return IPX_ERR_INVALID; }
        }
    }
    return IPX_OK;
}

int textset_build(hipStream_t s, const char *who, const ipx_text *texts, int n, int w, int h, ipx_textset *ts)
{
    int rc = texts_check(who, texts, n);
    if (rc) return rc;
    if (w < 0 || h < 0) { set_error("%s: bad frame size", who); return IPX_ERR_INVALID; }
    std::vector<uint8_t> blob;
    std::vector<GlyphHost> gh;
    std::vector<int> start(n + 1, 0);
    for (int t = 0; t < n; t++) {
        for (int i = 0; i < texts[t].n_glyphs; i++) {
            GlyphHost g;
            (void)pack_glyph(texts[t].glyphs[i], &blob, &g);
            gh.push_back(g);
        }
        start[t + 1] = (int)gh.size();
    }
    ts->mem.s = s;
    ts->w = w; ts->h = h; ts->n = n;
    uint8_t *masks_dev = nullptr;
    IPX_HIP(ts->mem.get(&masks_dev, blob.size()));
    std::vector<DevGlyph> tab;
    std::vector<DevText> desc(n);
    ts->bbox.assign(n, Rect{0, 0, 0, 0});
    for (int t = 0; t < n; t++) {
        DevText &d = desc[t];
        d.first = (int)tab.size();
        d.bbox = ts->bbox[t] = clip_glyphs(gh.data() + start[t], (size_t)(start[t + 1] - start[t]), masks_dev, w, h, &tab);
        d.n = (int)tab.size() - d.first;
        for (int c = 0; c < 4; c++) d.col[c] = (uint16_t)(texts[t].col[c] * 0x101u);
    }
    IPX_HIP(ts->mem.get(&ts->glyphs_dev, tab.size() * sizeof(DevGlyph)));
    IPX_HIP(ts->mem.get(&ts->texts_dev, desc.size() * sizeof(DevText)));
    if (!blob.empty()) IPX_HIP(hipMemcpyAsync(masks_dev, blob.data(), blob.size(), hipMemcpyHostToDevice, s));
    if (!tab.empty()) IPX_HIP(hipMemcpyAsync(ts->glyphs_dev, tab.data(), tab.size() * sizeof(DevGlyph), hipMemcpyHostToDevice, s));
    if (!desc.empty()) IPX_HIP(hipMemcpyAsync(ts->texts_dev, desc.data(), desc.size() * sizeof(DevText), hipMemcpyHostToDevice, s));
    IPX_HIP(hipStreamSynchronize(s));
    return IPX_OK;
}

int dev_composite_texts(hipStream_t s, AsyncFree *mem, uint8_t *dst, int dstride, size_t frame_stride, int n_frames, const ipx_textset &ts,
                        int first, const int *map)
{
    if (n_frames <= 0) return IPX_OK;
    if (!map && (first < 0 || (long long)first + n_frames > ts.n)) {
        set_error("composite texts: frames %d .. %lld of a set of %d texts", first, (long long)first + n_frames, ts.n);
        return IPX_ERR_INVALID;
    }
    int bw = 0, bh = 0;
    for (int z = 0; z < n_frames; z++) {
        const int t = map ? map[z] : first + z;
        if (t < 0 || t >= ts.n) { set_error("composite texts: frame %d names text %d of %d", z, t, ts.n); return IPX_ERR_INVALID; }
        const Rect &b = ts.bbox[t];
        if (b.empty()) continue;
        bw = std::max(bw, b.dx()); bh = std::max(bh, b.dy());
    }
    if (!bw || !bh) return IPX_OK;
    int *map_dev = nullptr;
    if (map) {
        if (!mem) { set_error("composite texts: a frame-to-text map needs scratch"); return IPX_ERR_INVALID; }
        IPX_HIP(mem->get(&map_dev, (size_t)n_frames * sizeof(int)));
        IPX_HIP(hipMemcpyAsync(map_dev, map, (size_t)n_frames * sizeof(int), hipMemcpyHostToDevice, s));
    }
    for (int z0 = 0; z0 < n_frames; z0 += 65535)
        IPX_HIP(launch_composite_texts(dst + (size_t)z0 * frame_stride, dstride, frame_stride, std::min(65535, n_frames - z0), ts.texts_dev,
                                       ts.glyphs_dev, map_dev ? map_dev + z0 : nullptr, first + z0, bw, bh, s));
    return IPX_OK;
}

int leg_entry_check(const char *who, const ipx_plan *pl, int n, const ipx_bytes *files, const int *status, ipx_jpeg_result **result,
                    bool texts_entry, const ipx_text *texts)
{
    const bool ok = pl && n >= 0 && files && status && result;
    if (ok) *result = nullptr;
    if (!ok || (texts_entry && !texts)) { set_error("%s: bad argument", who); return IPX_ERR_INVALID; }
    if (!texts_entry) return IPX_OK;
    if (pl->p.glyphs) {
        set_error("%s: the plan carries a glyph set of its own; per-file texts need a plan created with glyphs == NULL (copy only)", who);
        return IPX_ERR_INVALID;
    }
    return texts_check(who, texts, n);
}

extern "C" {

static void prepare_hip_env();
int ipx_device_count(void) try
{
    prepare_hip_env();
    clear_error();
    int n = 0;
    hipError_t e = hipGetDeviceCount(&n);
    if (e != hipSuccess) { (void)hipGetLastError(); set_error("hipGetDeviceCount: %s", hipGetErrorString(e)); return IPX_ERR_NODEVICE; }
    return n;
}
IPX_CATCH_STATUS

static void prepare_hip_env()
{
    static std::once_flag once;
    std::call_once(once, [] {
        if (!getenv("GPU_MAX_HW_QUEUES")) {
            char v[16];
            snprintf(v, sizeof v, "%d", std::max(8, env_int("IPX_LANES", 5) + 3));
            setenv("GPU_MAX_HW_QUEUES", v, 0);
        }
    });
}

int ipx_create(const ipx_config *cfg, ipx_ctx **out) try
{
    clear_error();
    if (!out) { set_error("ipx_create: null out"); return IPX_ERR_INVALID; }
    *out = nullptr;
    prepare_hip_env();
    int ndev = 0;
    if (hipGetDeviceCount(&ndev) != hipSuccess || ndev <= 0) {
        (void)hipGetLastError();
        set_error("no HIP device visible: the pixel path has no CPU fallback");
        return IPX_ERR_NODEVICE;
    }
    int dev = cfg ? cfg->device : -1;
    if (dev < 0) dev = env_int("IPX_DEVICE", env_int("LOCAL_RANK", 0) % ndev);
    if (dev >= ndev) { set_error("device %d out of range (%d visible)", dev, ndev); return IPX_ERR_INVALID; }
    IPX_HIP(hipSetDevice(dev));
    hipDeviceProp_t prop;
    IPX_HIP(hipGetDeviceProperties(&prop, dev));
    if (strncmp(prop.gcnArchName, "gfx950", 6) != 0) {
        set_error("device %d is %s; libipx carries gfx950 code only", dev, prop.gcnArchName);
        return IPX_ERR_NODEVICE;
    }
    ipx_ctx *c = new (std::nothrow) ipx_ctx;
// ... 202 lines not shown
    if (e == hipSuccess) e = hipMalloc((void **)&dd, down_bytes);
    if (e == hipSuccess) e = hipStreamCreateWithFlags(&s1, hipStreamNonBlocking);
    if (e == hipSuccess) e = hipStreamCreateWithFlags(&s2, hipStreamNonBlocking);
    if (e == hipSuccess) e = hipEventCreate(&e0);
    if (e == hipSuccess) e = hipEventCreate(&e1);
    if (e == hipSuccess) { memset(hu, 1, up_bytes); e = hipMemset(dd, 2, down_bytes); }
    uint8_t *hd_dev = nullptr;
    if (e == hipSuccess && hipHostGetDevicePointer((void **)&hd_dev, hd, 0) != hipSuccess) { (void)hipGetLastError(); hd_dev = nullptr; }
    const size_t piece = (size_t)std::max(1, env_int("IPX_PROBE_CHUNK_MB", 32)) << 20;
    auto timed = [&](bool up, bool down, bool down_by_kernel, double *gb_up, double *gb_down) {
        double best = 1e30;
        for (int r = 0; r < reps + 1 && e == hipSuccess; r++) {
            const auto t0 = std::chrono::steady_clock::now();
            if (down && down_by_kernel) {
                hipLaunchKernelGGL(link_store_kernel, dim3(512), dim3(256), 0, s2, (uint4 *)hd_dev, (const uint4 *)dd, down_bytes / 16);
                e = hipGetLastError();
            }
            for (size_t o = 0; e == hipSuccess && (o < up_bytes || o < down_bytes); o += piece) {
                if (up && o < up_bytes) e = hipMemcpyAsync(du + o, hu + o, std::min(piece, up_bytes - o), hipMemcpyHostToDevice, s1);
                if (down && !down_by_kernel && o < down_bytes && e == hipSuccess) e = hipMemcpyAsync(hd + o, dd + o, std::min(piece, down_bytes - o), hipMemcpyDeviceToHost, s2);
            }
            if (e == hipSuccess) e = hipStreamSynchronize(s1);
            if (e == hipSuccess) e = hipStreamSynchronize(s2);
            const double sec = std::chrono::duration<double>(std::chrono::steady_clock::now() - t0).count();
            if (r > 0) best = std::min(best, sec);
        }
        if (gb_up) *gb_up = up ? up_bytes / best / 1e9 : 0;
        if (gb_down) *gb_down = down ? down_bytes / best / 1e9 : 0;
    };
    if (e == hipSuccess) timed(true, false, false, &out_gbps[0], nullptr);
    if (e == hipSuccess) timed(false, true, false, nullptr, &out_gbps[1]);
    if (e == hipSuccess) timed(true, true, false, &out_gbps[2], &out_gbps[3]);
    if (e == hipSuccess && hd_dev) {
        double u = 0, d = 0;
        timed(false, true, true, nullptr, &d);
        out_gbps[1] = std::max(out_gbps[1], d);
        if (e == hipSuccess) timed(true, true, true, &u, &d);
        if (e == hipSuccess && u + d > out_gbps[2] + out_gbps[3]) { out_gbps[2] = u; out_gbps[3] = d; }
    }
    if (e0) (void)hipEventDestroy(e0);
    if (e1) (void)hipEventDestroy(e1);
    if (s1) (void)hipStreamDestroy(s1);
    if (s2) (void)hipStreamDestroy(s2);
    if (du) (void)hipFree(du);
    if (dd) (void)hipFree(dd);
    if (hu) (void)ipx_host_free(ctx, hu);
    if (hd) (void)ipx_host_free(ctx, hd);
    if (e != hipSuccess) { set_error("ipx_link_probe: %s", hipGetErrorString(e)); return e == hipErrorOutOfMemory ? IPX_ERR_NOMEM : IPX_ERR_HIP; }
    return IPX_OK;
}
IPX_CATCH_STATUS

int ipx_device_sync(ipx_ctx *ctx) try
{
    IPX_ENTER(ctx);
    IPX_HIP(hipDeviceSynchronize());
    return IPX_OK;
}
IPX_CATCH_STATUS

int ipx_stream_sync(ipx_ctx *ctx, void *stream) try
{
    IPX_ENTER(ctx);
    IPX_HIP(hipStreamSynchronize(stream ? (hipStream_t)stream : ctx->stream));
    return IPX_OK;
}
IPX_CATCH_STATUS

void *ipx_stream_create(ipx_ctx *ctx)
{
    clear_error();
    if (!ctx) return nullptr;
    (void)hipSetDevice(ctx->device);
    hipStream_t st = nullptr;
    if (hipStreamCreateWithFlags(&st, hipStreamNonBlocking) != hipSuccess) { (void)hipGetLastError(); set_error("hipStreamCreate failed"); return nullptr; }
    return st;
}

int ipx_stream_destroy(ipx_ctx *ctx, void *stream) try
{
    IPX_ENTER(ctx);
    if (!stream) return IPX_OK;
    IPX_HIP(hipStreamSynchronize((hipStream_t)stream));
    IPX_HIP(hipStreamDestroy((hipStream_t)stream));
    return IPX_OK;
}
IPX_CATCH_STATUS

void *ipx_event_create(ipx_ctx *ctx)
{
    clear_error();
    if (!ctx) return nullptr;
    (void)hipSetDevice(ctx->device);
    hipEvent_t ev = nullptr;
    if (hipEventCreate(&ev) != hipSuccess) { (void)hipGetLastError(); set_error("hipEventCreate failed"); return nullptr; }
    return ev;
}

int ipx_event_record(ipx_ctx *ctx, void *event, void *stream) try
{
    IPX_ENTER(ctx);
    if (!event) { set_error("ipx_event_record: null event"); return IPX_ERR_INVALID; }
    IPX_HIP(hipEventRecord((hipEvent_t)event, stream ? (hipStream_t)stream : ctx->stream));
    return IPX_OK;
}
IPX_CATCH_STATUS

int ipx_event_elapsed_ms(ipx_ctx *ctx, void *start, void *stop, float *ms) try
{
    IPX_ENTER(ctx);
    if (!start || !stop || !ms) { set_error("ipx_event_elapsed_ms: bad argument"); return IPX_ERR_INVALID; }
    IPX_HIP(hipEventSynchronize((hipEvent_t)stop));
    IPX_HIP(hipEventElapsedTime(ms, (hipEvent_t)start, (hipEvent_t)stop));
    return IPX_OK;
}
IPX_CATCH_STATUS

void ipx_event_destroy(ipx_ctx *ctx, void *event)
{
    if (!ctx || !event) return;
    (void)hipSetDevice(ctx->device);
    (void)hipEventDestroy((hipEvent_t)event);
}

int ipx_dev_scale_bilinear_rgba8(ipx_ctx *ctx, void *stream, uint8_t *dst, int dw, int dh,
                                 int dstride, ipx_rect dr, const uint8_t *src, int sw, int sh,
                                 int sstride, ipx_rect sr, int op) try
{
    IPX_ENTER(ctx);
    IPX_FRAME("ipx_dev_scale_bilinear_rgba8", "destination", dst, dw, dh, dstride);
    IPX_DEV_OUT("ipx_dev_scale_bilinear_rgba8", "destination", dst, (unsigned)dstride);
    IPX_FRAME("ipx_dev_scale_bilinear_rgba8", "source", src, sw, sh, sstride);
    hipStream_t s = stream ? (hipStream_t)stream : ctx->stream;
    AsyncFree mem{s, {}};
    int *flag = nullptr;
    if (op == IPX_OP_OVER) IPX_HIP(mem.get(&flag, sizeof(int)));
    return dev_scale(ctx, s, flag, dst, dw, dh, dstride, to_rect(dr), src, sw, sh, sstride, to_rect(sr), op);
}
IPX_CATCH_STATUS

int ipx_dev_draw_rgba8(ipx_ctx *ctx, void *stream, uint8_t *dst, int dw, int dh, int dstride,
                       ipx_rect r, const uint8_t *src, int sw, int sh, int sstride, int spx, int spy,
                       int op) try
{
    IPX_ENTER(ctx);
    IPX_FRAME("ipx_dev_draw_rgba8", "destination", dst, dw, dh, dstride);
    IPX_DEV_OUT("ipx_dev_draw_rgba8", "destination", dst, (unsigned)dstride);
    IPX_FRAME("ipx_dev_draw_rgba8", "source", src, sw, sh, sstride);
    return dev_draw(stream ? (hipStream_t)stream : ctx->stream, dst, dw, dh, dstride, to_rect(r), src,
                    sw, sh, sstride, spx, spy, op);
}
IPX_CATCH_STATUS

int ipx_glyphset_create(ipx_ctx *ctx, const ipx_glyph *glyphs, int n, const uint8_t col[4],
                        ipx_glyphset **out) try
{
    IPX_ENTER(ctx);
    if (!out || n < 0 || (n && !glyphs) || !col) { set_error("ipx_glyphset_create: bad argument"); return IPX_ERR_INVALID; }
    if (n > kMaxGlyphs) { set_error("ipx_glyphset_create: %d glyphs exceed the limit of %d", n, kMaxGlyphs); return IPX_ERR_UNSUPPORTED; }
    *out = nullptr;
    ipx_glyphset *gs = new (std::nothrow) ipx_glyphset;
    if (!gs) { set_error("out of memory"); return IPX_ERR_NOMEM; }
    gs->device = ctx->device;
    memcpy(gs->col, col, 4);
    std::vector<uint8_t> blob;
    for (int i = 0; i < n; i++) {
        const ipx_glyph &g = glyphs[i];
        GlyphHost h;
        if (!pack_glyph(g, &blob, &h)) {
            set_error("ipx_glyphset_create: glyph %d has a bad mask", i);
            delete gs;
            return IPX_ERR_INVALID;
        }
        gs->g.push_back(h);
    }
    gs->masks_bytes = blob.size();
    if (!blob.empty()) {
        hipError_t e = hipMalloc((void **)&gs->masks_dev, blob.size());
        if (e == hipSuccess) e = hipMemcpy(gs->masks_dev, blob.data(), blob.size(), hipMemcpyHostToDevice);
        if (e != hipSuccess) {
            set_error("glyph mask upload failed: %s", hipGetErrorString(e));
            ipx_glyphset_destroy(ctx, gs);
            return IPX_ERR_HIP;
        }
    }
    *out = gs;
    return IPX_OK;
}
IPX_CATCH_STATUS

void ipx_glyphset_destroy(ipx_ctx *ctx, ipx_glyphset *gs)
{
    if (!gs) return;
    (void)hipSetDevice(ctx ? ctx->device : gs->device);
    for (auto &kv : gs->clipped) if (kv.second.dev) (void)hipFree(kv.second.dev);
    if (gs->masks_dev) (void)hipFree(gs->masks_dev);
    delete gs;
}

int ipx_dev_composite_glyphs_rgba8(ipx_ctx *ctx, void *stream, uint8_t *dst, int dw, int dh,
                                   int dstride, const ipx_glyphset *gs) try
{
    IPX_ENTER(ctx);
    if (!gs) { set_error("ipx_dev_composite_glyphs_rgba8: bad argument"); return IPX_ERR_INVALID; }
    IPX_FRAME("ipx_dev_composite_glyphs_rgba8", "destination", dst, dw, dh, dstride);
    IPX_DEV_OUT("ipx_dev_composite_glyphs_rgba8", "destination", dst, (unsigned)dstride);
    return dev_composite(stream ? (hipStream_t)stream : ctx->stream, dst, dw, dh, dstride, 0, 1, gs);
}
IPX_CATCH_STATUS

int ipx_textset_create(ipx_ctx *ctx, void *stream, const ipx_text *texts, int n, int w, int h, ipx_textset **out) try
{
    IPX_ENTER(ctx);
    if (!out) { set_error("ipx_textset_create: bad argument"); return IPX_ERR_INVALID; }
    *out = nullptr;
    ipx_textset *ts = new (std::nothrow) ipx_textset;
    if (!ts) { set_error("out of memory"); return IPX_ERR_NOMEM; }
    ts->device = ctx->device;
    const int rc = textset_build(stream ? (hipStream_t)stream : ctx->stream, "ipx_textset_create", texts, n, w, h, ts);
    if (rc) { delete ts; return rc; }
    *out = ts;
    return IPX_OK;
}
IPX_CATCH_STATUS

void ipx_textset_destroy(ipx_ctx *ctx, ipx_textset *ts)
{
    if (!ts) return;
    (void)hipSetDevice(ctx ? ctx->device : ts->device);
    delete ts;
}

int ipx_dev_composite_texts_rgba8(ipx_ctx *ctx, void *stream, uint8_t *dst, int w, int h, int dstride, size_t frame_stride, int n_frames,
                                  const ipx_textset *ts, int first, const int32_t *map) try
{
    IPX_ENTER(ctx);
    if (!ts || n_frames < 0) { set_error("ipx_dev_composite_texts_rgba8: bad argument"); return IPX_ERR_INVALID; }
    if (w != ts->w || h != ts->h) { set_error("ipx_dev_composite_texts_rgba8: the text set was clipped for %dx%d frames, not %dx%d", ts->w, ts->h, w, h); return IPX_ERR_INVALID; }
    IPX_FRAME("ipx_dev_composite_texts_rgba8", "destination", dst, w, h, dstride);
    IPX_DEV_OUT("ipx_dev_composite_texts_rgba8", "destination", dst, (unsigned)dstride, frame_stride);
    hipStream_t s = stream ? (hipStream_t)stream : ctx->stream;
    AsyncFree mem{s, {}};
    const int rc = dev_composite_texts(s, &mem, dst, dstride, frame_stride, n_frames, *ts, first, (const int *)map);
    if (map) (void)hipStreamSynchronize(s);
    return rc;
}
IPX_CATCH_STATUS

int ipx_scale_bilinear_rgba8(ipx_ctx *ctx, uint8_t *dst, int dw, int dh, int dstride, ipx_rect dr,
                             const uint8_t *src, int sw, int sh, int sstride, ipx_rect sr, int op) try
{
    IPX_ENTER(ctx);
    IPX_FRAME("ipx_scale_bilinear_rgba8", "destination", dst, dw, dh, dstride);
    IPX_FRAME("ipx_scale_bilinear_rgba8", "source", src, sw, sh, sstride);
    ScalePrep pr;
    int rc = scale_prepare(dw, dh, to_rect(dr), sw, sh, to_rect(sr), op, &pr);
    if (rc) return rc;
    if (pr.empty || dw == 0 || dh == 0) return IPX_OK;
    LaneLease lane(ctx);
    const size_t sbytes = align256((size_t)sw * sh * 4), dbytes = align256((size_t)dw * dh * 4);
    rc = lane_reserve(lane.get(), sbytes + dbytes);
    if (rc) return rc;
    uint8_t *dsrc = lane->dev, *ddst = lane->dev + sbytes;
    hipStream_t s = lane->stream;
    if (sw && sh) IPX_HIP(hipMemcpy2DAsync(dsrc, (size_t)sw * 4, src, sstride, (size_t)sw * 4, sh, hipMemcpyHostToDevice, s));
    IPX_HIP(hipMemcpy2DAsync(ddst, (size_t)dw * 4, dst, dstride, (size_t)dw * 4, dh, hipMemcpyHostToDevice, s));
    rc = dev_scale(ctx, s, lane->flag, ddst, dw, dh, dw * 4, to_rect(dr), dsrc, sw, sh, sw * 4, to_rect(sr), op);
    if (rc) { (void)hipStreamSynchronize(s); return rc; }
    IPX_HIP(hipMemcpy2DAsync(dst, dstride, ddst, (size_t)dw * 4, (size_t)dw * 4, dh, hipMemcpyDeviceToHost, s));
    IPX_HIP(hipStreamSynchronize(s));
    return IPX_OK;
}
IPX_CATCH_STATUS

int ipx_draw_rgba8(ipx_ctx *ctx, uint8_t *dst, int dw, int dh, int dstride, ipx_rect r,
                   const uint8_t *src, int sw, int sh, int sstride, int spx, int spy, int op) try
{
    IPX_ENTER(ctx);
    IPX_FRAME("ipx_draw_rgba8", "destination", dst, dw, dh, dstride);
    IPX_FRAME("ipx_draw_rgba8", "source", src, sw, sh, sstride);
    if (op != IPX_OP_OVER && op != IPX_OP_SRC) { set_error("draw: unknown op %d", op); return IPX_ERR_INVALID; }
    if (!dw || !dh || !sw || !sh) return IPX_OK;
    LaneLease lane(ctx);
    const size_t sbytes = align256((size_t)sw * sh * 4), dbytes = align256((size_t)dw * dh * 4);
    int rc = lane_reserve(lane.get(), sbytes + dbytes);
    if (rc) return rc;
    uint8_t *dsrc = lane->dev, *ddst = lane->dev + sbytes;
    hipStream_t s = lane->stream;
    IPX_HIP(hipMemcpy2DAsync(dsrc, (size_t)sw * 4, src, sstride, (size_t)sw * 4, sh, hipMemcpyHostToDevice, s));
    IPX_HIP(hipMemcpy2DAsync(ddst, (size_t)dw * 4, dst, dstride, (size_t)dw * 4, dh, hipMemcpyHostToDevice, s));
    rc = dev_draw(s, ddst, dw, dh, dw * 4, to_rect(r), dsrc, sw, sh, sw * 4, spx, spy, op);
    if (rc) { (void)hipStreamSynchronize(s); return rc; }
    IPX_HIP(hipMemcpy2DAsync(dst, dstride, ddst, (size_t)dw * 4, (size_t)dw * 4, dh, hipMemcpyDeviceToHost, s));
    IPX_HIP(hipStreamSynchronize(s));
    return IPX_OK;
}
IPX_CATCH_STATUS

int ipx_composite_glyphs_rgba8(ipx_ctx *ctx, uint8_t *dst, int dw, int dh, int dstride,
                               const ipx_glyph *glyphs, int n, const uint8_t col[4]) try
{
    IPX_ENTER(ctx);
    if (n < 0 || (n && !glyphs) || !col) { set_error("ipx_composite_glyphs_rgba8: bad argument"); return IPX_ERR_INVALID; }
    IPX_FRAME("ipx_composite_glyphs_rgba8", "destination", dst, dw, dh, dstride);
    if (!n || !dw || !dh) return IPX_OK;
    ipx_glyphset *gs = nullptr;
    int rc = ipx_glyphset_create(ctx, glyphs, n, col, &gs);
    if (rc) return rc;
    {
        LaneLease lane(ctx);
        rc = lane_reserve(lane.get(), align256((size_t)dw * dh * 4));
        hipStream_t s = lane->stream;
        hipError_t e = hipSuccess;
        if (!rc) {
            e = hipMemcpy2DAsync(lane->dev, (size_t)dw * 4, dst, dstride, (size_t)dw * 4, dh, hipMemcpyHostToDevice, s);
            if (e == hipSuccess) rc = dev_composite(s, lane->dev, dw, dh, dw * 4, 0, 1, gs);
            if (e == hipSuccess && !rc)
                e = hipMemcpy2DAsync(dst, dstride, lane->dev, (size_t)dw * 4, (size_t)dw * 4, dh, hipMemcpyDeviceToHost, s);
            hipError_t e2 = hipStreamSynchronize(s);
            if (e == hipSuccess) e = e2;
            if (e != hipSuccess && !rc) { set_error("composite staging failed: %s", hipGetErrorString(e)); rc = IPX_ERR_HIP; }
        }
    }
    ipx_glyphset_destroy(ctx, gs);
    return rc;
}
IPX_CATCH_STATUS

}

namespace {

template <typename F>
int stage_and_run(ipx_ctx *ctx, uint8_t *dst, int dw, int dh, int dstride, size_t src_bytes, F &&upload_and_run)
{
    LaneLease lane(ctx);
    const size_t dbytes = align256((size_t)dw * dh * 4);
    int rc = lane_reserve(lane.get(), dbytes + src_bytes + 1024);
    if (rc) return rc;
    uint8_t *ddst = lane->dev, *dsrc = lane->dev + dbytes;
    hipStream_t s = lane->stream;
    IPX_HIP(hipMemcpy2DAsync(ddst, (size_t)dw * 4, dst, dstride, (size_t)dw * 4, dh, hipMemcpyHostToDevice, s));
    rc = upload_and_run(s, lane->flag, ddst, dsrc);
    if (rc) { (void)hipStreamSynchronize(s); return rc; }
    IPX_HIP(hipMemcpy2DAsync(dst, dstride, ddst, (size_t)dw * 4, (size_t)dw * 4, dh, hipMemcpyDeviceToHost, s));
    IPX_HIP(hipStreamSynchronize(s));
    return IPX_OK;
}

bool ycbcr_ok(const ipx_ycbcr *y, int *cw, int *ch)
{
    if (!y || !y->y || !y->cb || !y->cr || y->w <= 0 || y->h <= 0 || !ycbcr_ratio_ok(y->ratio)) return false;
    chroma_size(y->ratio, y->w, y->h, cw, ch);
    return y->ystride >= y->w && y->cstride >= *cw;
}

int upload_ycbcr(hipStream_t s, const ipx_ycbcr *y, int cw, int ch, uint8_t *dsrc, DevSrc *out)
{
    const size_t yb = align256((size_t)y->w * y->h), cbytes = align256((size_t)cw * ch);
    IPX_HIP(hipMemcpy2DAsync(dsrc, y->w, y->y, y->ystride, y->w, y->h, hipMemcpyHostToDevice, s));
    IPX_HIP(hipMemcpy2DAsync(dsrc + yb, cw, y->cb, y->cstride, cw, ch, hipMemcpyHostToDevice, s));
    IPX_HIP(hipMemcpy2DAsync(dsrc + yb + cbytes, cw, y->cr, y->cstride, cw, ch, hipMemcpyHostToDevice, s));
    out->kind = IPX_SRC_YCBCR; out->pix = dsrc; out->stride = y->w;
    out->cb = dsrc + yb; out->cr = dsrc + yb + cbytes; out->cstride = cw; out->ratio = y->ratio;
    out->w = y->w; out->h = y->h;
    return IPX_OK;
}

}

extern "C" {

int ipx_scale_bilinear_nrgba8(ipx_ctx *ctx, uint8_t *dst, int dw, int dh, int dstride, ipx_rect dr,
                              const uint8_t *src, int sw, int sh, int sstride, ipx_rect sr, int op) try
{
    IPX_ENTER(ctx);
    IPX_FRAME("ipx_scale_bilinear_nrgba8", "destination", dst, dw, dh, dstride);
    IPX_FRAME("ipx_scale_bilinear_nrgba8", "source", src, sw, sh, sstride);
    if (!dw || !dh || !sw || !sh) return IPX_OK;
    return stage_and_run(ctx, dst, dw, dh, dstride, align256((size_t)sw * sh * 4), [&](hipStream_t s, int *flag, uint8_t *ddst, uint8_t *dsrc) -> int {
        IPX_HIP(hipMemcpy2DAsync(dsrc, (size_t)sw * 4, src, sstride, (size_t)sw * 4, sh, hipMemcpyHostToDevice, s));
        return dev_scale_src(ctx, s, flag, ddst, dw, dh, dw * 4, to_rect(dr), rgba_src(dsrc, sw, sh, sw * 4, IPX_SRC_NRGBA), to_rect(sr), op);
    });
}
IPX_CATCH_STATUS

int ipx_draw_nrgba8(ipx_ctx *ctx, uint8_t *dst, int dw, int dh, int dstride, ipx_rect r, const uint8_t *src,
                    int sw, int sh, int sstride, int spx, int spy, int op) try
{
    IPX_ENTER(ctx);
    IPX_FRAME("ipx_draw_nrgba8", "destination", dst, dw, dh, dstride);
    IPX_FRAME("ipx_draw_nrgba8", "source", src, sw, sh, sstride);
    if (!dw || !dh || !sw || !sh) return IPX_OK;
    return stage_and_run(ctx, dst, dw, dh, dstride, align256((size_t)sw * sh * 4), [&](hipStream_t s, int *, uint8_t *ddst, uint8_t *dsrc) -> int {
        IPX_HIP(hipMemcpy2DAsync(dsrc, (size_t)sw * 4, src, sstride, (size_t)sw * 4, sh, hipMemcpyHostToDevice, s));
        return dev_draw_src(s, ddst, dw, dh, dw * 4, to_rect(r), rgba_src(dsrc, sw, sh, sw * 4, IPX_SRC_NRGBA), spx, spy, op);
    });
}
IPX_CATCH_STATUS

static int upload_deep(hipStream_t s, const uint8_t *src, int sw, int sh, int sstride, int kind, uint8_t *dsrc, DevSrc *out)
{
    const int bpp = src_bpp(src_of_deep(kind));
    uint8_t *pix = dsrc + align256((size_t)sw * sh * 8);
    IPX_HIP(hipMemcpy2DAsync(pix, (size_t)sw * bpp, src, sstride, (size_t)sw * bpp, sh, hipMemcpyHostToDevice, s));
    IPX_HIP(launch_deep_expand(dsrc, 0, pix, sw * bpp, 0, kind, sw, sh, 1, s));
    out->kind = IPX_SRC_TAP64; out->pix = dsrc; out->stride = sw * 8; out->w = sw; out->h = sh;
    return IPX_OK;
}
static int deep_args_status(const char *who, const void *dst, int dw, int dh, int dstride, const void *src, int sw, int sh, int sstride, int kind)
{
    if (src_of_deep(kind) < 0) { set_error("%s: unknown source type %d", who, kind); return IPX_ERR_INVALID; }
    int rc = frame_status(who, "destination", dst, dw, dh, dstride);
    if (!rc) rc = frame_status(who, "source", src, sw, sh, sstride, src_bpp(src_of_deep(kind)));
    if (!rc) rc = frame_status(who, "source", src, sw, sh, (long long)sw * 8, 8);
    return rc;
}

int ipx_scale_bilinear_deep(ipx_ctx *ctx, uint8_t *dst, int dw, int dh, int dstride, ipx_rect dr, const uint8_t *src, int sw, int sh,
                            int sstride, int kind, ipx_rect sr, int op) try
{
    IPX_ENTER(ctx);
    const int rc = deep_args_status("ipx_scale_bilinear_deep", dst, dw, dh, dstride, src, sw, sh, sstride, kind);
    if (rc) return rc;
    if (!dw || !dh || !sw || !sh) return IPX_OK;
    return stage_and_run(ctx, dst, dw, dh, dstride, align256((size_t)sw * sh * 8) * 2, [&](hipStream_t s, int *flag, uint8_t *ddst, uint8_t *dsrc) -> int {
        DevSrc t;
        const int r2 = upload_deep(s, src, sw, sh, sstride, kind, dsrc, &t);
        return r2 ? r2 : dev_scale_src(ctx, s, flag, ddst, dw, dh, dw * 4, to_rect(dr), t, to_rect(sr), op);
    });
}
IPX_CATCH_STATUS

int ipx_draw_deep(ipx_ctx *ctx, uint8_t *dst, int dw, int dh, int dstride, ipx_rect r, const uint8_t *src, int sw, int sh, int sstride,
                  int kind, int spx, int spy, int op) try
{
    IPX_ENTER(ctx);
    const int rc = deep_args_status("ipx_draw_deep", dst, dw, dh, dstride, src, sw, sh, sstride, kind);
    if (rc) return rc;
    if (!dw || !dh || !sw || !sh) return IPX_OK;
    return stage_and_run(ctx, dst, dw, dh, dstride, align256((size_t)sw * sh * 8) * 2, [&](hipStream_t s, int *, uint8_t *ddst, uint8_t *dsrc) -> int {
        DevSrc t;
        const int r2 = upload_deep(s, src, sw, sh, sstride, kind, dsrc, &t);
        return r2 ? r2 : dev_draw_src(s, ddst, dw, dh, dw * 4, to_rect(r), t, spx, spy, op);
    });
}
IPX_CATCH_STATUS

int ipx_scale_bilinear_ycbcr(ipx_ctx *ctx, uint8_t *dst, int dw, int dh, int dstride, ipx_rect dr,
                             const ipx_ycbcr *src, ipx_rect sr) try
{
    IPX_ENTER(ctx);
    int cw = 0, ch = 0;
    IPX_FRAME("ipx_scale_bilinear_ycbcr", "destination", dst, dw, dh, dstride);
    if (!ycbcr_ok(src, &cw, &ch)) { set_error("ipx_scale_bilinear_ycbcr: bad arguments"); return IPX_ERR_INVALID; }
    if (!frame_span_ok(src->w, src->h, src->ystride, 1)) { set_error("ipx_scale_bilinear_ycbcr: source planes beyond the addressable span"); return IPX_ERR_UNSUPPORTED; }
    if (!dw || !dh) return IPX_OK;
    const size_t bytes = align256((size_t)src->w * src->h) + 2 * align256((size_t)cw * ch);
    return stage_and_run(ctx, dst, dw, dh, dstride, bytes, [&](hipStream_t s, int *flag, uint8_t *ddst, uint8_t *dsrc) -> int {
        DevSrc d;
// ... 94 lines not shown
            set_error("ipx_plan_create: cannot tabulate the axes of a %dx%d <- %dx%d scale", sk.dw, sk.dh, sk.sr.dx(), sk.sr.dy());
            delete pl;
            return IPX_ERR_INVALID;
        }
        have[k] = true;
        axoff[k][0] = put(ks_axis_bytes(sk.hx));
        axoff[k][1] = put(ks_axis_bytes(sk.hy));
    }
    KsFusedIn fin[2];
    for (int k = 0; k < 2; k++) {
        const PlanScale &sk = pl->sc[k];
        fin[k].dw = sk.dw; fin[k].dh = sk.dh; fin[k].sr_x0 = sk.sr.x0; fin[k].sr_y0 = sk.sr.y0; fin[k].hx = &sk.hx; fin[k].hy = &sk.hy;
    }
    size_t fused_off[3] = {0, 0, 0};
    if (!env_int("IPX_NO_FUSE", 0)) {
        const int px_bytes[3] = {4, 8, 2};
        for (int f = 0; f < 3; f++) {
            std::vector<uint8_t> fblob;
            fin[1].top_taps = f == 1 && pl->p.crop_to_fit;
            if (ks_fused_plan(sw, sh, have[0] ? &fin[0] : nullptr, have[1] ? &fin[1] : nullptr, px_bytes[f], &fblob, &pl->fused[f])) {
                fused_off[f] = put(fblob.size());
                memcpy(blob.data() + fused_off[f], fblob.data(), fblob.size());
            }
        }
    }
    if (!blob.empty()) {
        hipError_t e = hipMalloc((void **)&pl->blob, blob.size());
        if (e != hipSuccess) {
            set_error("plan table allocation failed: %s", hipGetErrorString(e));
            ipx_plan_destroy(ctx, pl);
            return IPX_ERR_NOMEM;
        }
        for (int k = 0; k < 2; k++) {
            if (!have[k]) continue;
            ks_axis_pack(pl->sc[k].hx, blob.data() + axoff[k][0], pl->blob + axoff[k][0], &pl->sc[k].ax[0]);
            ks_axis_pack(pl->sc[k].hy, blob.data() + axoff[k][1], pl->blob + axoff[k][1], &pl->sc[k].ax[1]);
        }
        for (int f = 0; f < 3; f++)
            if (pl->fused[f].ok) ks_fused_rebase(&pl->fused[f], pl->blob + fused_off[f]);
        e = hipMemcpy(pl->blob, blob.data(), blob.size(), hipMemcpyHostToDevice);
        if (e != hipSuccess) {
            set_error("plan table upload failed: %s", hipGetErrorString(e));
            ipx_plan_destroy(ctx, pl);
            return IPX_ERR_HIP;
        }
    }
    *out = pl;
    return IPX_OK;
}
IPX_CATCH_STATUS

void ipx_plan_destroy(ipx_ctx *ctx, ipx_plan *plan)
{
    if (!plan) return;
    if (ctx) (void)hipSetDevice(ctx->device);
    if (plan->blob) (void)hipFree(plan->blob);
    if (plan->owned_gs) ipx_glyphset_destroy(ctx, plan->owned_gs);
    delete plan;
}

static size_t max_cached_plans() { return (size_t)std::max(1, env_int("IPX_PLAN_CACHE_MAX", 256)); }

static int ops_key(const ipx_pool_ops &in, std::string *key)
{
    if (in.n_glyphs < 0 || (in.n_glyphs && !in.glyphs)) { set_error("bad glyph list"); return IPX_ERR_INVALID; }
    key->assign((const char *)&in, offsetof(ipx_pool_ops, glyphs));
    key->append((const char *)in.col, 4);
    for (int i = 0; i < in.n_glyphs; i++) {
        const ipx_glyph &g = in.glyphs[i];
        if (g.mw < 0 || g.mh < 0 || (g.mw && g.mh && (!g.mask || g.mstride < g.mw))) { set_error("glyph %d has a bad mask", i); return IPX_ERR_INVALID; }
        key->append((const char *)&g.mw, sizeof(int32_t) * 2);
        key->append((const char *)&g.dr, sizeof g.dr);
        key->append((const char *)&g.mpx, sizeof(int32_t) * 2);
        for (int y = 0; y < g.mh; y++) key->append((const char *)g.mask + (size_t)y * g.mstride, (size_t)g.mw);
    }
    return IPX_OK;
}

int ipx_plan_acquire(ipx_ctx *ctx, const ipx_pool_ops *ops, ipx_plan **plan, int *cached) try
{
    IPX_ENTER(ctx);
    if (!ops || !plan || !cached) { set_error("ipx_plan_acquire: bad argument"); return IPX_ERR_INVALID; }
    *plan = nullptr; *cached = 0;
    std::string key;
    int rc = ops_key(*ops, &key);
    if (rc) return rc;
    std::lock_guard<std::mutex> lk(ctx->plan_mu);
    const bool use_cache = env_int("IPX_PLAN_CACHE", 1) != 0;
    auto it = ctx->plan_cache.find(key);
    if (use_cache && it != ctx->plan_cache.end()) {
        *plan = it->second.second; *cached = 1;
        (*plan)->cache_refs++; (*plan)->cache_stamp = ++ctx->plan_clock;
        return IPX_OK;
    }
    ipx_glyphset *gs = nullptr;
    if (ops->do_watermark && ops->n_glyphs > 0) {
        rc = ipx_glyphset_create(ctx, ops->glyphs, ops->n_glyphs, ops->col, &gs);
        if (rc) return rc;
    }
    ipx_plan_params pp;
    memset(&pp, 0, sizeof pp);
    pp.sw = ops->sw; pp.sh = ops->sh;
    pp.do_resize = ops->do_resize; pp.resize_w = ops->resize_w; pp.resize_h = ops->resize_h; pp.keep_aspect = ops->keep_aspect;
    pp.do_thumbnail = ops->do_thumbnail; pp.thumb_size = ops->thumb_size; pp.crop_to_fit = ops->crop_to_fit;
    pp.do_watermark = ops->do_watermark; pp.glyphs = gs;
    ipx_plan *pl = nullptr;
    rc = ipx_plan_create(ctx, &pp, &pl);
    if (rc) { if (gs) ipx_glyphset_destroy(ctx, gs); return rc; }
    pl->owned_gs = gs;
    if (use_cache && ctx->plan_cache.size() >= max_cached_plans()) {
        auto victim = ctx->plan_cache.end();
        for (auto i2 = ctx->plan_cache.begin(); i2 != ctx->plan_cache.end(); ++i2)
            if (i2->second.second->cache_refs == 0 && (victim == ctx->plan_cache.end() || i2->second.second->cache_stamp < victim->second.second->cache_stamp))
                victim = i2;
        if (victim != ctx->plan_cache.end()) {
            ipx_plan_destroy(ctx, victim->second.second);
            ctx->plan_cache.erase(victim);
        }
    }
    if (use_cache && ctx->plan_cache.size() < max_cached_plans()) {
        pl->cache_refs = 1; pl->cache_stamp = ++ctx->plan_clock;
        ctx->plan_cache.emplace(std::move(key), std::make_pair(gs, pl));
        *cached = 1;
    }
    *plan = pl;
    return IPX_OK;
}
IPX_CATCH_STATUS

void ipx_plan_release(ipx_ctx *ctx, ipx_plan *plan, int cached)
{
    if (!plan) return;
    if (!cached) { ipx_plan_destroy(ctx, plan); return; }
    if (!ctx) return;
    std::lock_guard<std::mutex> lk(ctx->plan_mu);
    if (plan->cache_refs > 0) plan->cache_refs--;
}

int ipx_plan_query(const ipx_plan *plan, ipx_plan_info *info) try
{
    clear_error();
    if (!plan || !info) { set_error("ipx_plan_query: bad argument"); return IPX_ERR_INVALID; }
    *info = plan->info;
    return IPX_OK;
}
IPX_CATCH_STATUS

}

static hipError_t composite_text(const ipx_plan *pl, uint8_t *wm, size_t wm_frame_stride, int n, hipStream_t s)
{
    if (!wm || pl->glyphs.n <= 0 || !pl->p.glyphs) return hipSuccess;
    const uint8_t *c = pl->p.glyphs->col;
    return launch_composite(wm, pl->p.sw * 4, wm_frame_stride, n, pl->glyphs.dev, pl->glyphs.n, pl->glyphs.bbox, c[0] * 0x101u, c[1] * 0x101u,
                            c[2] * 0x101u, c[3] * 0x101u, s);
}

static int run_dev_any(ipx_ctx *ctx, hipStream_t s, const ipx_plan *pl, int n, const DevSrc &src, const BatchDst &dst)
{
    const int sw = pl->p.sw, sh = pl->p.sh;
    uint8_t *outs[2] = {pl->sc[0].on ? dst.out[kOutResize] : nullptr, pl->sc[1].on ? dst.out[kOutThumb] : nullptr};
    const size_t *ostr = dst.frame_stride;
    uint8_t *wm = pl->p.do_watermark ? dst.out[kOutWm] : nullptr;
    const size_t wm_frame_stride = dst.frame_stride[kOutWm];
    for (int k = 0; k < 2; k++)
        if (pl->sc[k].dw <= 0 || pl->sc[k].dh <= 0) outs[k] = nullptr;
    if (!wm && !outs[0] && !outs[1]) return IPX_OK;
    int kinds[2] = {src.kind, pl->p.crop_to_fit ? ks_crop_kind(src.kind) : src.kind};

    const bool gray = src.kind == IPX_SRC_YCBCR && src.cstride == 0;
    const KsFusedPlan &fp = pl->fused[src.kind == IPX_SRC_RGBA ? 0 : gray ? 2 : 1];
    if (fp.ok && env_int("IPX_FUSED", 1)) {
        KsFusedArgs a{};
        a.src = src.pix; a.src_fs = src.frame_stride; a.sstride = src.stride; a.sw = sw; a.sh = sh;
        a.src_kind = src.kind; a.cb = src.cb; a.cr = src.cr; a.cstride = src.cstride; a.ratio = src.ratio; a.c_fs = src.c_frame_stride;
        a.wm = wm; a.wm_fs = wm_frame_stride; a.wm_stride = sw * 4;
        a.nframes = n;
        a.taps_le_alpha = src.le_alpha;
        for (int k = 0; k < 2; k++) {
            if (!outs[k]) continue;
            const PlanScale &ps = pl->sc[k];
            KsFusedOut &o = a.o[a.nout++];
            o.out = outs[k]; o.frame_stride = ostr[k]; o.ostride = ps.dw * 4; o.obytes = ps.dw * ps.dh * 4;
            o.dw = ps.dw; o.dh = ps.dh; o.sr_x0 = ps.sr.x0; o.sr_y0 = ps.sr.y0;
            o.kind = kinds[k]; o.pk = k;
        }
        AsyncFree mem{s, {}};
        int *redo = nullptr;
        KsFix fixv, *fix = nullptr;
        const int max_items = n * fp.nstrips * std::max(fp.whole.nseg, fp.split.nseg);
        const bool spec = src.kind == IPX_SRC_RGBA && env_int("IPX_KS_SPEC", 1);
        const bool fast = (spec || src.kind == IPX_SRC_YCBCR || src.kind == IPX_SRC_NRGBA || (src.kind == IPX_SRC_TAP64 && src.le_alpha)) &&
                          env_int("IPX_KS_FAST", 1) != 0;
        if (spec || fast) {
            const int cap_env = env_int("IPX_KS_FIX_CAP", 0);
            int cap[2] = {0, 0};
            for (int k = 0; k < 2; k++)
                if (fast && outs[k]) cap[k] = cap_env > 0 ? cap_env : (int)std::min<size_t>(std::max<size_t>((size_t)pl->sc[k].dw * pl->sc[k].dh / 96, 256), (size_t)1 << 20);
            const size_t flags = align256((size_t)max_items * sizeof(int)), counts = fast ? align256((size_t)n * 2 * sizeof(int)) : 0;
            IPX_HIP(mem.get(&redo, flags + counts + (size_t)n * (cap[0] + cap[1]) * sizeof(uint2)));
            if (fast) {
                fixv.count = (int *)((uint8_t *)redo + flags);
                fixv.list = (uint2 *)((uint8_t *)redo + flags + counts);
                fixv.cap[0] = cap[0]; fixv.cap[1] = cap[1];
                for (int k = 0; k < 2; k++) { fixv.ax[k] = pl->sc[k].ax[0]; fixv.ay[k] = pl->sc[k].ax[1]; }
                IPX_HIP(hipMemsetAsync(fixv.count, 0, (size_t)n * 2 * sizeof(int), s));
                fix = &fixv;
            }
        }
        a.redo = redo;
#if IPX_DIAG
        static unsigned long long *stamp_buf = nullptr;
        if (env_int("IPX_STAMPS", 0)) {
            if (!stamp_buf) IPX_HIP(hipMalloc((void **)&stamp_buf, 24 * sizeof(unsigned long long)));
            IPX_HIP(hipMemsetAsync(stamp_buf, 0, 24 * sizeof(unsigned long long), s));
            a.stamps = stamp_buf;
        }
#endif
        KsText text{}, *txt = nullptr;
        if (wm && pl->glyphs.n > 0 && pl->p.glyphs) {
            const uint8_t *c = pl->p.glyphs->col;
            text = KsText{pl->glyphs.dev, pl->glyphs.n, pl->glyphs.bbox, c[0] * 0x101u, c[1] * 0x101u, c[2] * 0x101u, c[3] * 0x101u};
            txt = &text;
        }
        bool matched = false, text_done = false;
        hipError_t e = launch_ks_fused(fp, a, fix, txt, ctx->cus, s, &matched, &text_done);
        if (fix && matched && e == hipSuccess && env_int("IPX_KS_STATS", 0)) {
            std::vector<int> cnt((size_t)n * 2), flags((size_t)max_items);
            (void)hipMemcpyAsync(cnt.data(), fixv.count, cnt.size() * sizeof(int), hipMemcpyDeviceToHost, s);
            (void)hipMemcpyAsync(flags.data(), redo, flags.size() * sizeof(int), hipMemcpyDeviceToHost, s);
            (void)hipStreamSynchronize(s);
            long long tot[2] = {0, 0}; int mx[2] = {0, 0}, nredo = 0;
            for (int i = 0; i < n; i++) for (int k = 0; k < 2; k++) { tot[k] += cnt[2 * i + k]; mx[k] = std::max(mx[k], cnt[2 * i + k]); }
            for (int f : flags) nredo += f != 0;
            fprintf(stderr, "[ipx ks stats] %d frames: undecided pixels per frame resize mean %.1f max %d (room %d), thumbnail mean %.1f max %d (room %d); %d of %d items redone in float64\n", n,
                    (double)tot[0] / n, mx[0], fixv.cap[0], (double)tot[1] / n, mx[1], fixv.cap[1], nredo, max_items);
        }
#if IPX_DIAG
        if (a.stamps && matched) {
            unsigned long long h[24];
            IPX_HIP(hipMemcpyAsync(h, a.stamps, sizeof h, hipMemcpyDeviceToHost, s));
            IPX_HIP(hipStreamSynchronize(s));
            const char *who[3] = {"resize waves", "thumbnail waves", "idle waves"};
            for (int r = 0; r < 3; r++) {
                double tot = 0;
                for (int i = 0; i < 6; i++) tot += (double)h[r * 8 + i];
                if (tot > 0)
                    fprintf(stderr, "[ipx stamps] %-16s share of wave time: wait-loads %.1f%%  drain %.1f%%  barrier %.1f%%  issue %.1f%%  scaleX %.1f%%  scaleY %.1f%%  (%.3g cycles)\n", who[r],
                            100 * h[r * 8] / tot, 100 * h[r * 8 + 1] / tot, 100 * h[r * 8 + 2] / tot, 100 * h[r * 8 + 3] / tot, 100 * h[r * 8 + 4] / tot, 100 * h[r * 8 + 5] / tot, tot);
            }
        }
#endif
        if (e != hipSuccess) { set_error("one-pass kernel launch failed: %s", hipGetErrorString(e)); return IPX_ERR_HIP; }
        if (matched) {
            if (!text_done) IPX_HIP(composite_text(pl, wm, wm_frame_stride, n, s));
            return IPX_OK;
        }
    }

    if (wm) {
        const int rc = dev_draw_src(s, wm, sw, sh, sw * 4, Rect{0, 0, sw, sh}, src, 0, 0, IPX_OP_SRC, wm_frame_stride);
        if (rc) return rc;
        IPX_HIP(composite_text(pl, wm, wm_frame_stride, n, s));
    }
    for (int k = 0; k < 2; k++) {
        if (!outs[k]) continue;
        const PlanScale &ps = pl->sc[k];
        const int rc = dev_scale_src(ctx, s, nullptr, outs[k], ps.dw, ps.dh, ps.dw * 4, Rect{0, 0, ps.dw, ps.dh}, src, ps.sr, IPX_OP_SRC, ostr[k],
                                     kinds[k], ps.ax);
        if (rc) return rc;
    }
    return IPX_OK;
}


int src_check(const char *who, const ipx_plan *pl, const BatchSrc &b, int n, bool in_hbm)
{
    if (b.type < 0 || b.type >= kSrcTypes) { set_error("%s: unknown source type", who); return IPX_ERR_INVALID; }
    const int bpp = src_bpp(b.type);
    bool ok = pl && n >= 0 && b.plane[0] && (long long)b.stride[0] >= (long long)pl->p.sw * bpp;
    if (ok && b.type == kSrcYCbCr) {
        int cw = 0, ch = 0;
        chroma_size(b.ratio, pl->p.sw, pl->p.sh, &cw, &ch);
        ok = b.plane[1] && b.plane[2] && ycbcr_ratio_ok(b.ratio) && b.stride[1] >= cw;
    }
    if (ok && b.type == kSrcPaletted) ok = b.palettes && !(in_hbm && ((uintptr_t)b.palettes & 3));
    if (ok && in_hbm && b.type >= kSrcNRGBA64)
        ok = !(((uintptr_t)b.plane[0] | (uintptr_t)b.stride[0] | b.frame_stride[0]) & (b.type == kSrcCMYK ? 3 : 1));
    if (!ok) { set_error("%s: bad argument", who); return IPX_ERR_INVALID; }
    const int sw = pl->p.sw, sh = pl->p.sh;
    if (!frame_span_ok(sw, sh, b.stride[0], bpp) || (b.type == kSrcYCbCr && !frame_span_ok(sw, sh, b.stride[1], 1)) ||
        (b.type >= kSrcNRGBA64 && !frame_span_ok(sw, sh, (long long)sw * 8, 8))) {
        set_error("%s: %dx%d frames with row strides of %d / %d bytes are beyond the 2 GiB span the kernels address", who, sw, sh, b.stride[0], b.stride[1]);
        return IPX_ERR_UNSUPPORTED;
    }
    if (in_hbm && n > 65535) { set_error("%s: at most 65535 frames per call", who); return IPX_ERR_UNSUPPORTED; }
    return IPX_OK;
}

SrcLayout src_layout(const ipx_plan *pl, const BatchSrc &b, size_t (*frame_rule)(size_t))
{
    SrcLayout L{};
    int cw = 0, ch = 0;
    if (b.type == kSrcYCbCr) chroma_size(b.ratio, pl->p.sw, pl->p.sh, &cw, &ch);
    L.planes = b.type == kSrcYCbCr ? 3 : 1;
    L.row[0] = (size_t)pl->p.sw * src_bpp(b.type); L.h[0] = pl->p.sh; L.fs[0] = frame_rule(L.row[0] * L.h[0]);
    L.row[1] = cw; L.h[1] = ch; L.fs[1] = frame_rule((size_t)cw * ch);
    L.pal = b.type == kSrcPaletted ? 1024 : 0;
    return L;
}

hipError_t src_upload(const BatchSrc &host, const SrcLayout &L, int i0, int m, uint8_t *scratch, int slots, hipStream_t s, const CopyPolicy &cp,
                      BatchSrc *in_hbm)
{
    *in_hbm = host;
    hipError_t e = hipSuccess;
    uint8_t *d = scratch;
    for (int p = 0; p < L.planes && e == hipSuccess; p++) {
        const int k = p ? 1 : 0;
        const size_t row = L.row[k], dfs = L.fs[k], hfs = host.frame_stride[k], bytes = dfs * m;
        const uint8_t *h = host.plane[p] + hfs * i0;
        const bool tight_rows = (size_t)host.stride[k] == row;
        if (cp.join_frames && tight_rows && hfs == dfs) {
            const size_t piece = cp.piece ? cp.piece : bytes;
            for (size_t o = 0; o < bytes && e == hipSuccess; o += piece) e = hipMemcpyAsync(d + o, h + o, std::min(piece, bytes - o), hipMemcpyHostToDevice, s);
        } else {
            for (int i = 0; i < m && e == hipSuccess; i++)
                e = cp.join_rows && tight_rows ? hipMemcpyAsync(d + dfs * i, h + hfs * i, row * L.h[k], hipMemcpyHostToDevice, s)
                                               : hipMemcpy2DAsync(d + dfs * i, row, h + hfs * i, host.stride[k], row, L.h[k], hipMemcpyHostToDevice, s);
        }
        in_hbm->plane[p] = d; in_hbm->stride[k] = (int)row; in_hbm->frame_stride[k] = dfs;
        d += dfs * slots;
    }
    if (L.pal && e == hipSuccess) {
        e = hipMemcpyAsync(d, host.palettes + L.pal * i0, L.pal * m, hipMemcpyHostToDevice, s);
        in_hbm->palettes = d;
    }
    return e;
}

int run_dev_src(ipx_ctx *ctx, hipStream_t s, const ipx_plan *pl, int m, const BatchSrc &b, const BatchDst &dst)
{
    if (m > 65535) { set_error("at most 65535 frames per device call"); return IPX_ERR_UNSUPPORTED; }
    const int sw = pl->p.sw, sh = pl->p.sh;
    AsyncFree mem{s, {}};
    DevSrc d;
    d.pix = b.plane[0]; d.stride = b.stride[0]; d.frame_stride = b.frame_stride[0]; d.w = sw; d.h = sh; d.nframes = m;
    switch (b.type) {
    case kSrcRGBA: break;
    case kSrcNRGBA: d.kind = IPX_SRC_NRGBA; break;
    case kSrcYCbCr:
        d.kind = IPX_SRC_YCBCR; d.cb = b.plane[1]; d.cr = b.plane[2]; d.cstride = b.stride[1]; d.ratio = b.ratio; d.c_frame_stride = b.frame_stride[1];
        break;
    case kSrcGray:
        if ((size_t)sw + 8 > ipx_ctx::kFlatChromaBytes) { set_error("Gray frames wider than %zu pixels", ipx_ctx::kFlatChromaBytes - 8); return IPX_ERR_UNSUPPORTED; }
        d.kind = IPX_SRC_YCBCR; d.cb = d.cr = ctx->flat_chroma; d.ratio = IPX_YCBCR_444;
        break;
    case kSrcPaletted: {
        const size_t fs = align256((size_t)sw * sh * 4);
        uint8_t *nrgba = nullptr;
        IPX_HIP(mem.get(&nrgba, fs * m));
        const hipError_t e = launch_palette_expand(nrgba, fs, b.plane[0], b.stride[0], b.frame_stride[0], b.palettes, sw, sh, m, s);
        if (e != hipSuccess) { set_error("palette expansion failed: %s", hipGetErrorString(e)); return IPX_ERR_HIP; }
        d.kind = IPX_SRC_NRGBA; d.pix = nrgba; d.stride = sw * 4; d.frame_stride = fs;
        break;
    }
    default: {
        const size_t tfs = align256((size_t)sw * sh * 8);
        uint8_t *taps = nullptr;
        IPX_HIP(mem.get(&taps, tfs * m));
        const hipError_t e = launch_deep_expand(taps, tfs, b.plane[0], b.stride[0], b.frame_stride[0], b.type - kSrcNRGBA64, sw, sh, m, s);
        if (e != hipSuccess) { set_error("tap expansion failed: %s", hipGetErrorString(e)); return IPX_ERR_HIP; }
        d.kind = IPX_SRC_TAP64; d.pix = taps; d.stride = sw * 8; d.frame_stride = tfs;
        d.le_alpha = b.type != kSrcRGBA64;
        break;
// ... 325 lines not shown
```

imageprocessor_amd/csrc/ipx_runtime_internal.h:

```cpp
#pragma once

#include <atomic>
#include <sched.h>

#include <algorithm>
#include <cctype>
#include <cstdio>
#include <condition_variable>
#include <cstdlib>
#include <cstring>
#include <deque>
#include <map>
#include <mutex>
#include <string>
#include <utility>
#include <vector>

#include "ipx_internal.h"
#include "ipx_ks.h"

using namespace ipx;

struct Lane {
    hipStream_t stream = nullptr;
    uint8_t *dev = nullptr;
    size_t dev_bytes = 0;
    int *flag = nullptr;
    uint8_t *dec = nullptr;
    size_t dec_bytes = 0;
    uint8_t *pin = nullptr;
    size_t pin_bytes = 0;
    hipEvent_t ev[3] = {nullptr, nullptr, nullptr};
    bool busy = false;
};

struct ipx_ctx {
    int device = 0;
    int cus = 256;
    hipStream_t stream = nullptr;
    std::vector<Lane> lanes;
    size_t lane_bytes = 0;
    std::mutex mu;
    std::condition_variable cv;
    std::mutex host_mu;
    std::map<void *, size_t> host_size;
    std::multimap<size_t, void *> host_free_blocks;
    std::deque<void *> host_lru;
    size_t host_cached = 0, host_cache_limit = (size_t)8 << 30;
    int jj_active = 0;
    uint8_t *flat_chroma = nullptr;
    std::mutex plan_mu;
    std::map<std::string, std::pair<ipx_glyphset *, ipx_plan *>> plan_cache;
    uint64_t plan_clock = 0;
    std::mutex ks_mu;
    std::map<std::pair<int, int>, std::pair<uint8_t *, KsAxisDev>> ks_axes;
    std::atomic<long long> jpeg_counts[4] = {{0}, {0}, {0}, {0}};
    std::atomic<long long> png_counts[5] = {{0}, {0}, {0}, {0}, {0}};
    std::atomic<long long> jpeg_cmyk_files{0};
    static constexpr size_t kFlatChromaBytes = (size_t)64 << 10;
};

struct GlyphHost {
    size_t mask_off;
    int mw, mh;
    Rect dr;
    int mpx, mpy;
};

struct ClippedGlyphs {
    DevGlyph *dev = nullptr;
    int n = 0;
    Rect bbox{0, 0, 0, 0};
};

struct ipx_glyphset {
    int device = 0;
    std::vector<GlyphHost> g;
    uint8_t *masks_dev = nullptr;
    size_t masks_bytes = 0;
    uint8_t col[4] = {0, 0, 0, 0};
    mutable std::mutex mu;
    mutable std::map<std::pair<int, int>, ClippedGlyphs> clipped;
};

struct PlanScale {
    bool on = false;
    int dw = 0, dh = 0;
    Rect sr{0, 0, 0, 0};
    KsAxis hx, hy;
    KsAxisDev ax[2]{};
};

struct ipx_plan {
    ipx_plan_params p{};
    ipx_plan_info info{};
    PlanScale sc[2];
    KsFusedPlan fused[3];
    uint8_t *blob = nullptr;
    ClippedGlyphs glyphs;
    mutable std::mutex mu;
    ipx_glyphset *owned_gs = nullptr;
    int cache_refs = 0;
    uint64_t cache_stamp = 0;
};

inline int env_int(const char *name, int dflt)
{
    const char *v = getenv(name);
    return v && *v ? atoi(v) : dflt;
}

struct DeviceGuard {
    explicit DeviceGuard(int dev) { ok = hipSetDevice(dev) == hipSuccess; }
    bool ok;
};

#define IPX_ENTER(ctx)                                                         \
    clear_error();                                                             \
    if (!(ctx)) { set_error("%s: null context", __func__); return IPX_ERR_INVALID; } \
    DeviceGuard guard_((ctx)->device);                                         \
    if (!guard_.ok) { set_error("hipSetDevice(%d) failed", (ctx)->device); return IPX_ERR_HIP; }

class LaneLease {
public:
    explicit LaneLease(ipx_ctx *c) : c_(c)
    {
        std::unique_lock<std::mutex> lk(c->mu);
        c->cv.wait(lk, [&] {
            for (auto &l : c->lanes) if (!l.busy) return true;
            return false;
        });
        for (auto &l : c->lanes) if (!l.busy) { l.busy = true; lane_ = &l; break; }
    }
    ~LaneLease()
    {
        {
            std::lock_guard<std::mutex> lk(c_->mu);
            lane_->busy = false;
        }
        c_->cv.notify_all();
    }
    Lane *operator->() { return lane_; }
    Lane &get() { return *lane_; }
private:
    ipx_ctx *c_;
    Lane *lane_ = nullptr;
};

inline int lane_reserve_dec(Lane &l, size_t bytes)
{
    if (bytes <= l.dec_bytes) return IPX_OK;
    if (l.dec) { IPX_HIP(hipStreamSynchronize(l.stream)); IPX_HIP(hipFree(l.dec)); l.dec = nullptr; l.dec_bytes = 0; }
    const size_t want = bytes + bytes / 8;
    hipError_t e = hipMalloc((void **)&l.dec, want);
    if (e != hipSuccess) {
        (void)hipGetLastError();
        set_error("device allocation of %zu bytes failed: %s", want, hipGetErrorString(e));
        return IPX_ERR_NOMEM;
    }
    l.dec_bytes = want;
    return IPX_OK;
}

inline int lane_reserve(Lane &l, size_t bytes)
{
    if (bytes <= l.dev_bytes) return IPX_OK;
    if (l.dev) { IPX_HIP(hipStreamSynchronize(l.stream)); IPX_HIP(hipFree(l.dev)); l.dev = nullptr; l.dev_bytes = 0; }
    const size_t want = std::max(bytes, l.dev_bytes * 2);
    hipError_t e = hipMalloc((void **)&l.dev, want);
    if (e != hipSuccess) {
        (void)hipGetLastError();
        set_error("device allocation of %zu bytes failed: %s", want, hipGetErrorString(e));
        return IPX_ERR_NOMEM;
    }
    l.dev_bytes = want;
    return IPX_OK;
}

inline int frame_status(const char *who, const char *what, const void *p, int w, int h, long long stride, int bpp = 4)
{
    if (!p || w < 0 || h < 0 || stride < (long long)w * bpp) { set_error("%s: bad %s frame arguments", who, what); return IPX_ERR_INVALID; }
    if (!frame_span_ok(w, h, stride, bpp)) {
        set_error("%s: %s frame %dx%d (stride %lld) is beyond the 2 GiB / 65535-pixel span the kernels address", who, what, w, h, stride);
        return IPX_ERR_UNSUPPORTED;
    }
    return IPX_OK;
}
#define IPX_FRAME(who, what, p, w, h, stride) do { const int rc_ = frame_status(who, what, p, w, h, stride); if (rc_) return rc_; } while (0)

inline int dev_out_status(const char *who, const char *what, const void *p, unsigned long long stride, unsigned long long frame_stride = 0)
{
    if (p && (((uintptr_t)p | stride | frame_stride) & 3)) {
        set_error("%s: the %s frames' address and strides must be multiples of 4", who, what);
        return IPX_ERR_INVALID;
    }
    return IPX_OK;
}
#define IPX_DEV_OUT(who, what, p, ...) do { const int rc_ = dev_out_status(who, what, p, __VA_ARGS__); if (rc_) return rc_; } while (0)

template <class F> inline int guarded_status(F &&fn, std::string *text) noexcept
{
    try { fn(); return IPX_OK; }
    catch (...) {
        const int rc = status_of_exception();
        if (text) { try { *text = ipx_last_error(); } catch (...) { } }
        return rc;
    }
}

inline void bind_near_device(int device)
{
    if (env_int("IPX_POOL_NUMA", 1) == 0) return;
    char bus[32] = {0};
    if (hipDeviceGetPCIBusId(bus, sizeof bus, device) != hipSuccess) { (void)hipGetLastError(); return; }
    for (char *c = bus; *c; c++) *c = (char)tolower((unsigned char)*c);
    char path[128];
    snprintf(path, sizeof path, "/sys/bus/pci/devices/%s/local_cpulist", bus);
    FILE *f = fopen(path, "r");
    if (!f) return;
    char line[4096] = {0};
    const bool ok = fgets(line, sizeof line, f) != nullptr;
    fclose(f);
    if (!ok) return;
    cpu_set_t allowed, want;
    if (sched_getaffinity(0, sizeof allowed, &allowed) != 0) return;
    CPU_ZERO(&want);
    for (char *p = line; *p;) {
        char *e = nullptr;
        long a = strtol(p, &e, 10);
        if (e == p) break;
        long b = a;
        if (*e == '-') { p = e + 1; b = strtol(p, &e, 10); }
// ... 219 lines not shown
```

include/ipx.h:

```cpp
#ifndef IPX_H
#define IPX_H

#include <stddef.h>
#include <stdint.h>

#ifdef __cplusplus
extern "C" {
#endif

#define IPX_ABI_VERSION 1

typedef struct ipx_ctx ipx_ctx;
typedef struct ipx_glyphset ipx_glyphset;
typedef struct ipx_plan ipx_plan;

typedef enum {
    IPX_OK = 0,
    IPX_ERR_INVALID = -1,
    IPX_ERR_NOMEM = -2,
    IPX_ERR_HIP = -3,
    IPX_ERR_UNSUPPORTED = -4,
    IPX_ERR_NODEVICE = -5
} ipx_status;

enum { IPX_OP_OVER = 0, IPX_OP_SRC = 1 };

typedef struct { int32_t x0, y0, x1, y1; } ipx_rect;

typedef struct {
    const uint8_t *mask;
    int32_t mw, mh, mstride;
    ipx_rect dr;
    int32_t mpx, mpy;
} ipx_glyph;

typedef struct {
    int32_t device;
    int32_t lanes;
    size_t lane_bytes;
} ipx_config;


int ipx_create(const ipx_config *cfg, ipx_ctx **out);
void ipx_destroy(ipx_ctx *ctx);
const char *ipx_last_error(void);
int ipx_abi_version(void);
int ipx_device_count(void);

int ipx_frame_supported(int w, int h, long long stride, int bytes_per_pixel);


int ipx_resize_dims(int ow, int oh, int w, int h, int keep_aspect, int *nw, int *nh);
int ipx_thumb_geometry(int ow, int oh, int size, int crop_to_fit, ipx_rect *crop, int *nw, int *nh);
int ipx_text_height_px(double font_size);
int ipx_watermark_anchor(const char *position, int w, int h, int width_px, int height_px,
                         int *px, int *py);
int ipx_parse_color(const char *s, double opacity, uint8_t rgba[4]);


void *ipx_host_alloc(ipx_ctx *ctx, size_t bytes);
int ipx_host_free(ipx_ctx *ctx, void *p);
void *ipx_dev_alloc(ipx_ctx *ctx, size_t bytes);
int ipx_dev_free(ipx_ctx *ctx, void *p);
int ipx_memcpy_h2d(ipx_ctx *ctx, void *dst_dev, const void *src_host, size_t bytes);
int ipx_memcpy_d2h(ipx_ctx *ctx, void *dst_host, const void *src_dev, size_t bytes);
int ipx_memcpy_d2d(ipx_ctx *ctx, void *dst_dev, const void *src_dev, size_t bytes);
int ipx_stream_copy(ipx_ctx *ctx, void *stream, void *dst_dev, const void *src_dev, size_t bytes);
int ipx_link_probe(ipx_ctx *ctx, size_t up_bytes, size_t down_bytes, int reps, double out_gbps[4]);
int ipx_device_sync(ipx_ctx *ctx);
int ipx_stream_sync(ipx_ctx *ctx, void *stream);

void *ipx_stream_create(ipx_ctx *ctx);
int ipx_stream_destroy(ipx_ctx *ctx, void *stream);


int ipx_scale_bilinear_rgba8(ipx_ctx *ctx, uint8_t *dst, int dw, int dh, int dstride, ipx_rect dr,
                             const uint8_t *src, int sw, int sh, int sstride, ipx_rect sr, int op);
int ipx_draw_rgba8(ipx_ctx *ctx, uint8_t *dst, int dw, int dh, int dstride, ipx_rect r,
                   const uint8_t *src, int sw, int sh, int sstride, int spx, int spy, int op);
int ipx_composite_glyphs_rgba8(ipx_ctx *ctx, uint8_t *dst, int dw, int dh, int dstride,
                               const ipx_glyph *glyphs, int n, const uint8_t col[4]);

int ipx_scale_bilinear_nrgba8(ipx_ctx *ctx, uint8_t *dst, int dw, int dh, int dstride, ipx_rect dr,
                              const uint8_t *src, int sw, int sh, int sstride, ipx_rect sr, int op);
int ipx_draw_nrgba8(ipx_ctx *ctx, uint8_t *dst, int dw, int dh, int dstride, ipx_rect r,
                    const uint8_t *src, int sw, int sh, int sstride, int spx, int spy, int op);

enum { IPX_YCBCR_444 = 0, IPX_YCBCR_422 = 1, IPX_YCBCR_420 = 2, IPX_YCBCR_440 = 3,
       IPX_GRAY = 4 ,
       IPX_YCBCR_411 = 5, IPX_YCBCR_410 = 6 };
typedef struct {
    const uint8_t *y, *cb, *cr;
    int32_t ystride, cstride, w, h, ratio;
} ipx_ycbcr;
int ipx_scale_bilinear_ycbcr(ipx_ctx *ctx, uint8_t *dst, int dw, int dh, int dstride, ipx_rect dr,
                             const ipx_ycbcr *src, ipx_rect sr);
int ipx_draw_ycbcr(ipx_ctx *ctx, uint8_t *dst, int dw, int dh, int dstride, ipx_rect r,
                   const ipx_ycbcr *src, int spx, int spy);


int ipx_dev_scale_bilinear_rgba8(ipx_ctx *ctx, void *stream, uint8_t *dst, int dw, int dh,
                                 int dstride, ipx_rect dr, const uint8_t *src, int sw, int sh,
                                 int sstride, ipx_rect sr, int op);
int ipx_dev_draw_rgba8(ipx_ctx *ctx, void *stream, uint8_t *dst, int dw, int dh, int dstride,
                       ipx_rect r, const uint8_t *src, int sw, int sh, int sstride, int spx,
                       int spy, int op);
int ipx_glyphset_create(ipx_ctx *ctx, const ipx_glyph *glyphs, int n, const uint8_t col[4],
                        ipx_glyphset **out);
void ipx_glyphset_destroy(ipx_ctx *ctx, ipx_glyphset *gs);
int ipx_dev_composite_glyphs_rgba8(ipx_ctx *ctx, void *stream, uint8_t *dst, int dw, int dh,
                                   int dstride, const ipx_glyphset *gs);

typedef struct { const ipx_glyph *glyphs; int32_t n_glyphs; uint8_t col[4]; } ipx_text;
typedef struct ipx_textset ipx_textset;
int ipx_textset_create(ipx_ctx *ctx, void *stream, const ipx_text *texts, int n, int w, int h, ipx_textset **out);
void ipx_textset_destroy(ipx_ctx *ctx, ipx_textset *ts);
int ipx_dev_composite_texts_rgba8(ipx_ctx *ctx, void *stream, uint8_t *dst, int w, int h, int dstride, size_t frame_stride,
                                  int n_frames, const ipx_textset *ts, int first, const int32_t *map );


typedef struct {
    int32_t sw, sh;
    int32_t do_resize;
    int32_t resize_w, resize_h, keep_aspect;
    int32_t do_thumbnail;
    int32_t thumb_size, crop_to_fit;
    int32_t do_watermark;
    const ipx_glyphset *glyphs;
} ipx_plan_params;

typedef struct {
    int32_t resize_w, resize_h;
    int32_t thumb_w, thumb_h;
    ipx_rect thumb_crop;
    int32_t wm_w, wm_h;
    size_t resize_bytes, thumb_bytes, wm_bytes;
    size_t algorithmic_bytes;
} ipx_plan_info;

int ipx_plan_create(ipx_ctx *ctx, const ipx_plan_params *p, ipx_plan **out);
void ipx_plan_destroy(ipx_ctx *ctx, ipx_plan *plan);
int ipx_plan_query(const ipx_plan *plan, ipx_plan_info *info);

int ipx_plan_run_dev(ipx_ctx *ctx, void *stream, const ipx_plan *plan, int n, const uint8_t *src,
                     int sstride, size_t src_frame_stride, uint8_t *resize_out,
                     size_t resize_frame_stride, uint8_t *thumb_out, size_t thumb_frame_stride,
                     uint8_t *wm_out, size_t wm_frame_stride);

int ipx_plan_run_host(ipx_ctx *ctx, const ipx_plan *plan, int n, const uint8_t *src, int sstride,
                      size_t src_frame_stride, uint8_t *resize_out, size_t resize_frame_stride,
                      uint8_t *thumb_out, size_t thumb_frame_stride, uint8_t *wm_out,
                      size_t wm_frame_stride);

typedef struct {
    const uint8_t *y, *cb, *cr;
    int32_t ystride, cstride;
    size_t y_frame_stride, c_frame_stride;
    int32_t ratio;
} ipx_ycbcr_batch;
int ipx_plan_run_dev_ycbcr(ipx_ctx *ctx, void *stream, const ipx_plan *plan, int n, const ipx_ycbcr_batch *src,
                           uint8_t *resize_out, size_t resize_frame_stride, uint8_t *thumb_out,
                           size_t thumb_frame_stride, uint8_t *wm_out, size_t wm_frame_stride);
int ipx_plan_run_dev_nrgba(ipx_ctx *ctx, void *stream, const ipx_plan *plan, int n, const uint8_t *src, int sstride,
                           size_t src_frame_stride, uint8_t *resize_out, size_t resize_frame_stride, uint8_t *thumb_out,
                           size_t thumb_frame_stride, uint8_t *wm_out, size_t wm_frame_stride);
int ipx_plan_run_dev_gray(ipx_ctx *ctx, void *stream, const ipx_plan *plan, int n, const uint8_t *gray, int stride,
                          size_t frame_stride, uint8_t *resize_out, size_t resize_frame_stride, uint8_t *thumb_out,
                          size_t thumb_frame_stride, uint8_t *wm_out, size_t wm_frame_stride);
int ipx_plan_run_dev_paletted(ipx_ctx *ctx, void *stream, const ipx_plan *plan, int n, const uint8_t *index, int stride,
                              size_t frame_stride, const uint8_t *palettes, uint8_t *resize_out, size_t resize_frame_stride,
                              uint8_t *thumb_out, size_t thumb_frame_stride, uint8_t *wm_out, size_t wm_frame_stride);
int ipx_plan_run_host_nrgba(ipx_ctx *ctx, const ipx_plan *plan, int n, const uint8_t *src, int sstride, size_t src_frame_stride,
                            uint8_t *resize_out, size_t resize_frame_stride, uint8_t *thumb_out, size_t thumb_frame_stride,
                            uint8_t *wm_out, size_t wm_frame_stride);
int ipx_plan_run_host_gray(ipx_ctx *ctx, const ipx_plan *plan, int n, const uint8_t *gray, int stride, size_t frame_stride,
                           uint8_t *resize_out, size_t resize_frame_stride, uint8_t *thumb_out, size_t thumb_frame_stride,
                           uint8_t *wm_out, size_t wm_frame_stride);
int ipx_plan_run_host_paletted(ipx_ctx *ctx, const ipx_plan *plan, int n, const uint8_t *index, int stride, size_t frame_stride,
                               const uint8_t *palettes, uint8_t *resize_out, size_t resize_frame_stride, uint8_t *thumb_out,
                               size_t thumb_frame_stride, uint8_t *wm_out, size_t wm_frame_stride);
enum { IPX_DEEP_NRGBA64 = 0, IPX_DEEP_RGBA64 = 1, IPX_DEEP_GRAY16 = 2, IPX_DEEP_CMYK = 3 };
int ipx_scale_bilinear_deep(ipx_ctx *ctx, uint8_t *dst, int dw, int dh, int dstride, ipx_rect dr, const uint8_t *src, int sw, int sh,
                            int sstride, int kind, ipx_rect sr, int op);
int ipx_draw_deep(ipx_ctx *ctx, uint8_t *dst, int dw, int dh, int dstride, ipx_rect r, const uint8_t *src, int sw, int sh, int sstride,
                  int kind, int spx, int spy, int op);
int ipx_plan_run_dev_deep(ipx_ctx *ctx, void *stream, const ipx_plan *plan, int n, int kind, const uint8_t *src, int sstride,
                          size_t src_frame_stride, uint8_t *resize_out, size_t resize_frame_stride, uint8_t *thumb_out,
                          size_t thumb_frame_stride, uint8_t *wm_out, size_t wm_frame_stride);
int ipx_plan_run_host_deep(ipx_ctx *ctx, const ipx_plan *plan, int n, int kind, const uint8_t *src, int sstride,
                           size_t src_frame_stride, uint8_t *resize_out, size_t resize_frame_stride, uint8_t *thumb_out,
                           size_t thumb_frame_stride, uint8_t *wm_out, size_t wm_frame_stride);
int ipx_plan_run_host_ycbcr(ipx_ctx *ctx, const ipx_plan *plan, int n, const ipx_ycbcr_batch *src,
                            uint8_t *resize_out, size_t resize_frame_stride, uint8_t *thumb_out,
                            size_t thumb_frame_stride, uint8_t *wm_out, size_t wm_frame_stride);

void *ipx_event_create(ipx_ctx *ctx);
int ipx_event_record(ipx_ctx *ctx, void *event, void *stream);
int ipx_event_elapsed_ms(ipx_ctx *ctx, void *start, void *stop, float *ms);
void ipx_event_destroy(ipx_ctx *ctx, void *event);


typedef enum {
    IPX_PT_FLOAT64 = 1, IPX_PT_INT = 2, IPX_PT_INT64 = 3, IPX_PT_INT32 = 4, IPX_PT_BOOL = 5, IPX_PT_STRING = 6
} ipx_param_type;
typedef struct {
    const char *key;
    int32_t type;
    double f64;
    int64_t i64;
    const char *str;
} ipx_param;

typedef struct { uint8_t *pix; int32_t w, h, stride; } ipx_image;
void ipx_image_free(ipx_image *img);

typedef struct {
    void *user;
    int (*measure)(void *user, const char *text, double font_size, int *width_px);
    int (*glyphs)(void *user, const char *text, double font_size, int px, int py, int w, int h,
                  const ipx_glyph **out, int *n);
    void (*release)(void *user);
} ipx_text_rasterizer;

typedef struct ipx_font ipx_font;
int ipx_font_create(const uint8_t *ttf, size_t len, ipx_font **out);
void ipx_font_destroy(ipx_font *font);
int ipx_font_glyph_index(const ipx_font *font, uint32_t rune);
int ipx_font_glyph_advance(const ipx_font *font, uint32_t rune, double font_size, int32_t *advance26_6);
int ipx_font_kern(const ipx_font *font, uint32_t rune0, uint32_t rune1, double font_size, int32_t *kern26_6);
int ipx_font_text_width(const ipx_font *font, const char *text, double font_size, int32_t *width26_6,
                        int *width_px);
int ipx_font_draw_string(ipx_font *font, const char *text, double font_size, int px, int py, int clip_w,
                         int clip_h, const ipx_glyph **out, int *n, int32_t *end_x26_6);
void ipx_font_release_thread(void);
int ipx_font_rasterizer(ipx_font *font, ipx_text_rasterizer *out);

int ipx_resizer_process(ipx_ctx *ctx, const ipx_image *img, const char *format,
                        const ipx_param *params, int nparams, ipx_image *out, char out_format[8]);
int ipx_thumbnailer_process(ipx_ctx *ctx, const ipx_image *img, const char *format,
                            const ipx_param *params, int nparams, ipx_image *out, char out_format[8]);
int ipx_watermarker_process(ipx_ctx *ctx, const ipx_image *img, const char *format,
                            const ipx_param *params, int nparams, const ipx_text_rasterizer *font,
                            ipx_image *out, char out_format[8]);

typedef struct { const char *type; const ipx_param *params; int32_t nparams; } ipx_operation;
typedef struct {
    const char *id, *image_id;
    const ipx_operation *ops; int32_t nops;
    const char *format;
} ipx_task;
typedef struct {
    char operation[16];
    char path[320];
    char content_type[32];
    char format[8];
    ipx_image image;
} ipx_processed;
int ipx_processor_process(ipx_ctx *ctx, const ipx_task *task, const ipx_image *decoded,
                          const char *decoded_format, const ipx_text_rasterizer *font,
                          ipx_processed *out, int *n_out);

size_t ipx_jpeg_coef_count(int w, int h);
// ... 155 lines not shown
```

Before: 250,300.

## Precompute glyph coverage map and composite watermark text from it

Builds a two-plane coverage map on the host when a glyphset is created. Each pixel holds up to two overlapping glyph mask values, and the map is uploaded to the device. The composite and fused tail kernels then read the map per pixel instead of walking every glyph for each pixel, which removes the per-pixel glyph loop and the shared-memory glyph table (now dynamic LDS, allocated only when it is needed). Deep overlaps of three or more glyphs, or oversized maps, fall back to the glyph walk. The tail block order is also rotated per frame to spread text blocks, and each mapped glyphset costs extra device memory.

```diff
diff --git a/imageprocessor_amd/__init__.py b/imageprocessor_amd/__init__.py
--- a/imageprocessor_amd/__init__.py
+++ b/imageprocessor_amd/__init__.py
@@ -160,6 +160,20 @@
             self.free()
         except Exception:
             pass
+
+
+def debug_cover_map(glyphs):
+    glyphs = list(glyphs)
+    arr, keep = _glyph_array(glyphs)
+    box, pitch, deep = _lib.Rect(), C.c_int(), C.c_int()
+    _check(lib().ipx_debug_cover_map(arr, len(glyphs), C.byref(box), C.byref(pitch), C.byref(deep), None, 0))
+    w, h = box.x1 - box.x0, box.y1 - box.y0
+    if deep.value or w <= 0 or h <= 0:
+        return (box.x0, box.y0, box.x1, box.y1), None, None, bool(deep.value)
+    planes = np.empty((2, h, pitch.value), np.uint8)
+    _check(lib().ipx_debug_cover_map(arr, len(glyphs), C.byref(box), C.byref(pitch), C.byref(deep), planes.ctypes.data, planes.nbytes))
+    assert not planes[:, :, w:].any()
+    return (box.x0, box.y0, box.x1, box.y1), planes[0, :, :w].copy(), planes[1, :, :w].copy(), False
 
 
 class GlyphSet:
diff --git a/imageprocessor_amd/_lib.py b/imageprocessor_amd/_lib.py
--- a/imageprocessor_amd/_lib.py
+++ b/imageprocessor_amd/_lib.py
@@ -174,6 +174,7 @@
     "ipx_dev_draw_rgba8": (_I, [_P, _P, _P, _I, _I, _I, Rect, _P, _I, _I, _I, _I, _I, _I]),
     "ipx_glyphset_create": (_I, [_P, C.POINTER(Glyph), _I, _P, C.POINTER(_P)]),
     "ipx_glyphset_destroy": (None, [_P, _P]),
+    "ipx_debug_cover_map": (_I, [C.POINTER(Glyph), _I, C.POINTER(Rect), C.POINTER(_I), C.POINTER(_I), _P, _Z]),
     "ipx_dev_composite_glyphs_rgba8": (_I, [_P, _P, _P, _I, _I, _I, _P]),
     "ipx_textset_create": (_I, [_P, _P, C.POINTER(Text), _I, _I, _I, C.POINTER(_P)]),
     "ipx_textset_destroy": (None, [_P, _P]),
diff --git a/imageprocessor_amd/csrc/ipx_device.h b/imageprocessor_amd/csrc/ipx_device.h
--- a/imageprocessor_amd/csrc/ipx_device.h
+++ b/imageprocessor_amd/csrc/ipx_device.h
@@ -117,5 +117,39 @@
     }
 }
 
+__device__ __forceinline__ void cover_text(uint8_t *frame, int stride, Rect bbox, const DevCover &cm, int first, int step, uint32_t sr,
+                                           uint32_t sg, uint32_t sb, uint32_t sa)
+{
+    constexpr int ROWS = kCoverRows, N = kCoverItems;
+    const int gw = bbox.x1 - bbox.x0, nitems = gw * ((bbox.y1 - bbox.y0 + ROWS - 1) / ROWS);
+    uint32_t d[N][ROWS], d0[N][ROWS], m1[N][ROWS], m2[N][ROWS];
+    uint8_t *q[N];
+#pragma unroll
+    for (int j = 0; j < N; j++) {
+        const int i = first + j * step;
+        const bool on = i < nitems;
+        const int gy = on ? i / gw : 0, x = bbox.x0 + (on ? i - gy * gw : 0), y0 = bbox.y0 + gy * ROWS;
+        q[j] = frame + (size_t)y0 * stride + (size_t)x * 4;
+        const uint8_t *c1 = cm.cov1 + (size_t)(y0 - cm.y0) * (size_t)cm.pitch + (size_t)(x - cm.x0), *c2 = cm.cov2 + (c1 - cm.cov1);
+#pragma unroll
+        for (int r = 0; r < ROWS; r++) {
+            const bool in = on && y0 + r < bbox.y1;
+            m1[j][r] = in ? c1[(size_t)r * cm.pitch] : 0u;
+            m2[j][r] = in ? c2[(size_t)r * cm.pitch] : 0u;
+            d0[j][r] = d[j][r] = in ? *(const uint32_t *)(q[j] + (size_t)r * stride) : 0u;
+        }
+    }
+#pragma unroll
+    for (int j = 0; j < N; j++)
+#pragma unroll
+        for (int r = 0; r < ROWS; r++) {
+            if (m1[j][r]) d[j][r] = glyph_over(d[j][r], m1[j][r], sr, sg, sb, sa);
+            if (__any(m2[j][r] != 0u)) {
+                if (m2[j][r]) d[j][r] = glyph_over(d[j][r], m2[j][r], sr, sg, sb, sa);
+            }
+            if (d[j][r] != d0[j][r]) *(uint32_t *)(q[j] + (size_t)r * stride) = d[j][r];
+        }
+}
+
 }
 }
diff --git a/imageprocessor_amd/csrc/ipx_host.cpp b/imageprocessor_amd/csrc/ipx_host.cpp
--- a/imageprocessor_amd/csrc/ipx_host.cpp
+++ b/imageprocessor_amd/csrc/ipx_host.cpp
@@ -1,3 +1,4 @@
+#include <algorithm>
 #include <cmath>
 #include <cstring>
 #include <new>
@@ -54,11 +55,80 @@
     return true;
 }
 
+void cover_build(const GlyphHost *g, size_t n, const uint8_t *blob, CoverMap *out)
+{
+    *out = CoverMap{};
+    constexpr int kFar = 1 << 28;
+    std::vector<Rect> rs(n);
+    Rect bb{0, 0, 0, 0};
+    bool any = false, far = false;
+    for (size_t i = 0; i < n; i++) {
+        const Rect &d = g[i].dr;
+        rs[i] = Rect{0, 0, 0, 0};
+        if (g[i].mw <= 0 || g[i].mh <= 0 || d.empty()) continue;
+        const int v[8] = {d.x0, d.y0, d.x1, d.y1, g[i].mpx, g[i].mpy, g[i].mw, g[i].mh};
+        bool f = false;
+        for (int c : v) f |= c < -kFar || c > kFar;
+        if (f) { far = true; continue; }
+        const Rect r = d.intersect(Rect{0, 0, g[i].mw, g[i].mh}.shifted(d.x0 - g[i].mpx, d.y0 - g[i].mpy));
+        if (r.empty()) continue;
+        rs[i] = r;
+        if (!any) bb = r;
+        else { bb.x0 = std::min(bb.x0, r.x0); bb.y0 = std::min(bb.y0, r.y0); bb.x1 = std::max(bb.x1, r.x1); bb.y1 = std::max(bb.y1, r.y1); }
+        any = true;
+    }
+    if (far) { out->deep = true; return; }
+    if (!any) return;
+    const long long pitch = ((long long)bb.dx() + 3) & ~3ll;
+    if (pitch * bb.dy() > kCoverMaxPlane) { out->deep = true; return; }
+    out->box = bb;
+    out->pitch = (int)pitch;
+    const size_t plane = (size_t)pitch * bb.dy();
+    out->planes.assign(2 * plane, 0);
+    uint8_t *c1 = out->planes.data(), *c2 = c1 + plane;
+    for (size_t i = 0; i < n; i++) {
+        const Rect &r = rs[i];
+        for (int y = r.y0; y < r.y1; y++) {
+            const uint8_t *m = blob + g[i].mask_off + (size_t)(y - g[i].dr.y0 + g[i].mpy) * g[i].mw + (r.x0 - g[i].dr.x0 + g[i].mpx);
+            const size_t row = (size_t)(y - bb.y0) * pitch + (r.x0 - bb.x0);
+            for (int x = 0; x < r.dx(); x++) {
+                if (!m[x]) continue;
+                if (!c1[row + x]) c1[row + x] = m[x];
+                else if (!c2[row + x]) c2[row + x] = m[x];
+                else out->deep = true;
+            }
+        }
+    }
+    if (out->deep) { out->planes.clear(); out->planes.shrink_to_fit(); }
+}
+
 }
 
 using namespace ipx;
 
 extern "C" {
+
+int ipx_debug_cover_map(const ipx_glyph *glyphs, int n, ipx_rect *box, int *pitch, int *deep, uint8_t *planes, size_t planes_cap) try
+{
+    clear_error();
+    if (n < 0 || (n && !glyphs) || !box || !pitch || !deep) { set_error("ipx_debug_cover_map: bad argument"); return IPX_ERR_INVALID; }
+    std::vector<uint8_t> blob;
+    std::vector<GlyphHost> gh((size_t)n);
+    for (int i = 0; i < n; i++) {
+        const ipx_glyph &g = glyphs[i];
+        if (g.mw < 0 || g.mh < 0 || (g.mw && g.mh && (!g.mask || g.mstride < g.mw))) { set_error("ipx_debug_cover_map: glyph %d has a bad mask", i); return IPX_ERR_INVALID; }
+        gh[i] = GlyphHost{blob.size(), g.mw, g.mh, to_rect(g.dr), g.mpx, g.mpy};
+        for (int y = 0; y < g.mh; y++) blob.insert(blob.end(), g.mask + (size_t)y * g.mstride, g.mask + (size_t)y * g.mstride + g.mw);
+    }
+    CoverMap m;
+    cover_build(gh.data(), gh.size(), blob.data(), &m);
+    *box = ipx_rect{m.box.x0, m.box.y0, m.box.x1, m.box.y1};
+    *pitch = m.pitch;
+    *deep = m.deep ? 1 : 0;
+    if (planes && planes_cap >= m.planes.size() && !m.planes.empty()) memcpy(planes, m.planes.data(), m.planes.size());
+    return IPX_OK;
+}
+IPX_CATCH_STATUS
 
 const char *ipx_last_error(void) { return g_err; }
 int ipx_abi_version(void) { return IPX_ABI_VERSION; }
diff --git a/imageprocessor_amd/csrc/ipx_internal.h b/imageprocessor_amd/csrc/ipx_internal.h
--- a/imageprocessor_amd/csrc/ipx_internal.h
+++ b/imageprocessor_amd/csrc/ipx_internal.h
@@ -103,9 +103,39 @@
     int x0, y0, x1, y1;
 };
 constexpr int kMaxGlyphs = 256;
+
+struct GlyphHost {
+    size_t mask_off;
+    int mw, mh;
+    Rect dr;
+    int mpx, mpy;
+};
+struct CoverMap {
+    Rect box{0, 0, 0, 0};
+    int pitch = 0;
+    bool deep = false;
+    std::vector<uint8_t> planes;
+};
+constexpr long long kCoverMaxPlane = 4ll << 20;
+void cover_build(const GlyphHost *g, size_t n, const uint8_t *blob, CoverMap *out);
+struct DevCover {
+    const uint8_t *cov1, *cov2;
+    int pitch, x0, y0, x1, y1;
+};
+constexpr int kCoverRows = 4, kCoverItems = 4;
+inline int cover_blocks(const Rect &bbox, int threads)
+{
+    const long long items = (long long)bbox.dx() * ((bbox.dy() + kCoverRows - 1) / kCoverRows);
+    return (int)((items + (long long)threads * kCoverItems - 1) / ((long long)threads * kCoverItems));
+}
+inline bool cover_usable(const DevCover &c, const Rect &bbox)
+{
+    return c.cov1 && !bbox.empty() && bbox.x0 >= c.x0 && bbox.y0 >= c.y0 && bbox.x1 <= c.x1 && bbox.y1 <= c.y1;
+}
+
 hipError_t launch_stream_copy(void *dst, const void *src, size_t bytes, hipStream_t s);
 hipError_t launch_composite(uint8_t *dst, int dstride, size_t frame_stride, int nframes,
-                            const DevGlyph *glyphs_dev, int n, Rect bbox, uint32_t sr, uint32_t sg,
+                            const DevGlyph *glyphs_dev, int n, Rect bbox, const DevCover &cover, uint32_t sr, uint32_t sg,
                             uint32_t sb, uint32_t sa, hipStream_t s);
 struct DevText {
     int first, n;
diff --git a/imageprocessor_amd/csrc/ipx_kernels.hip b/imageprocessor_amd/csrc/ipx_kernels.hip
--- a/imageprocessor_amd/csrc/ipx_kernels.hip
+++ b/imageprocessor_amd/csrc/ipx_kernels.hip
@@ -1,4 +1,5 @@
 #include <algorithm>
+#include <cstdlib>
 
 #include "ipx_internal.h"
 
@@ -186,6 +187,12 @@
     }
 }
 
+__global__ __launch_bounds__(256) void composite_cover_kernel(uint8_t *dst, int dstride, size_t frame_stride, Rect bbox, DevCover cover,
+                                                              uint32_t sr, uint32_t sg, uint32_t sb, uint32_t sa)
+{
+    cover_text(dst + blockIdx.y * frame_stride, dstride, bbox, cover, (int)blockIdx.x * (256 * kCoverItems) + (int)threadIdx.x, 256, sr, sg, sb, sa);
+}
+
 __global__ __launch_bounds__(256) void composite_texts_kernel(uint8_t *dst, int dstride, size_t frame_stride,
                                                               const DevText *__restrict__ texts, const DevGlyph *__restrict__ glyphs,
                                                               const int *__restrict__ map, int first)
@@ -369,10 +376,19 @@
 }
 
 hipError_t launch_composite(uint8_t *dst, int dstride, size_t frame_stride, int nframes,
-                            const DevGlyph *glyphs_dev, int n, Rect bbox, uint32_t sr, uint32_t sg,
+                            const DevGlyph *glyphs_dev, int n, Rect bbox, const DevCover &cover, uint32_t sr, uint32_t sg,
                             uint32_t sb, uint32_t sa, hipStream_t s)
 {
     if (n <= 0 || bbox.empty() || nframes <= 0) return hipSuccess;
+    const bool map = cover_usable(cover, bbox);
+    if (getenv("IPX_KS_DEBUG")) fprintf(stderr, "[ipx text] composite launch: %s\n", map ? "coverage map" : "glyph walk");
+    if (map) {
+        for (int f0 = 0; f0 < nframes; f0 += 65535) {
+            const dim3 grid(cover_blocks(bbox, 256), std::min(65535, nframes - f0));
+            hipLaunchKernelGGL(composite_cover_kernel, grid, dim3(256), 0, s, dst + (size_t)f0 * frame_stride, dstride, frame_stride, bbox, cover, sr, sg, sb, sa);
+        }
+        return hipGetLastError();
+    }
     dim3 block(64, 4), grid((bbox.dx() + 63) / 64, (bbox.dy() + 4 * kCompositeRows - 1) / (4 * kCompositeRows), nframes);
     hipLaunchKernelGGL(composite_kernel, grid, block, 0, s, dst, dstride, frame_stride, glyphs_dev, n,
                        bbox, sr, sg, sb, sa);
diff --git a/imageprocessor_amd/csrc/ipx_ks.h b/imageprocessor_amd/csrc/ipx_ks.h
--- a/imageprocessor_amd/csrc/ipx_ks.h
+++ b/imageprocessor_amd/csrc/ipx_ks.h
@@ -96,7 +96,7 @@
     int *redo;
     uint2 *fix; int *fix_count; int fix_cap[2], fix_stride;
 };
-struct KsText { const DevGlyph *gl; int n; Rect bbox; uint32_t sr, sg, sb, sa; };
+struct KsText { const DevGlyph *gl; int n; Rect bbox; uint32_t sr, sg, sb, sa; DevCover cover; };
 struct KsFix { uint2 *list = nullptr; int *count = nullptr; int cap[2] = {0, 0}; KsAxisDev ax[2], ay[2]; };
 struct KsFusedGeom { int nseg = 0; const KsSeg *segs = nullptr; const void *rows[2] = {nullptr, nullptr}; const int32_t *rowoff[2] = {nullptr, nullptr}; };
 struct KsFusedPlan {
@@ -131,7 +131,7 @@
     int R[2], chunks[2];
     uint8_t *wm; int wm_stride; size_t wm_fs;
     KsText text;
-    int tbx, tby;
+    int tb, tbx;
 };
 hipError_t launch_ks_tail(KsTailArgs t, hipStream_t s);
 
diff --git a/imageprocessor_amd/csrc/ipx_ks_tail.hip b/imageprocessor_amd/csrc/ipx_ks_tail.hip
--- a/imageprocessor_amd/csrc/ipx_ks_tail.hip
+++ b/imageprocessor_amd/csrc/ipx_ks_tail.hip
@@ -1,4 +1,5 @@
 #include <algorithm>
+#include <cstdio>
 #include <cstdlib>
 
 #include "ipx_ks_exact.h"
@@ -50,9 +51,10 @@
 template <int K0, int K1>
 __global__ __launch_bounds__(kTailThreads) void ks_tail_kernel(KsTailArgs t)
 {
-    __shared__ DevGlyph tab[kMaxGlyphs];
-    const int nx = t.chunks[0] + t.chunks[1], per = nx + t.tbx * t.tby, b = (int)blockIdx.x;
-    const int frame = b / per, c = b - frame * per;
+    extern __shared__ __align__(16) unsigned char tail_lds[];
+    DevGlyph *tab = (DevGlyph *)tail_lds;
+    const int nx = t.chunks[0] + t.chunks[1], per = nx + t.tb, b = (int)blockIdx.x;
+    const int frame = b / per, c = (b - frame * per + frame) % per;
     if (c < nx) {
         const int k = c >= t.chunks[0] ? 1 : 0, chunk = c - (k ? t.chunks[0] : 0);
         if (K0 == K1 || k == 0)
@@ -61,13 +63,18 @@
             tail_exact<K1>(t.g[1], t.list[1], t.list_stride, t.count[1], t.count_stride, t.cap[1], t.R[1], frame, chunk, t.chunks[1]);
         return;
     }
-    tail_text(t, tab, frame, c - nx);
+    if (t.text.cover.cov1)
+        cover_text(t.wm + (size_t)frame * t.wm_fs, t.wm_stride, t.text.bbox, t.text.cover, (c - nx) * (kTailThreads * kCoverItems) + (int)threadIdx.x,
+                   kTailThreads, t.text.sr, t.text.sg, t.text.sb, t.text.sa);
+    else
+        tail_text(t, tab, frame, c - nx);
 }
 
 template <int K0, int K1>
 void tail_go(const KsTailArgs &t, unsigned blocks, hipStream_t s)
 {
-    hipLaunchKernelGGL((ks_tail_kernel<K0, K1>), dim3(blocks), dim3(kTailThreads), 0, s, t);
+    const size_t lds = t.tb && !t.text.cover.cov1 ? kMaxGlyphs * sizeof(DevGlyph) : 0;
+    hipLaunchKernelGGL((ks_tail_kernel<K0, K1>), dim3(blocks), dim3(kTailThreads), lds, s, t);
 }
 
 template <int S, int C>
@@ -80,11 +87,8 @@
     return true;
 }
 
-}
-
-hipError_t launch_ks_tail(KsTailArgs t, hipStream_t s)
+hipError_t tail_launch(KsTailArgs t, hipStream_t s)
 {
-    if (t.nframes <= 0) return hipSuccess;
     const char *ev = getenv("IPX_KS_TAIL_BLOCKS");
     const int budget = ev && atoi(ev) > 0 ? atoi(ev) : 2048;
     for (int k = 0; k < 2; k++) {
@@ -97,9 +101,12 @@
     }
     const bool text = t.wm && t.text.gl && t.text.n > 0 && !t.text.bbox.empty();
     if (!text) t.text.n = 0;
+    if (!text || !cover_usable(t.text.cover, t.text.bbox)) t.text.cover = DevCover{};
     t.tbx = text ? (t.text.bbox.dx() + 63) / 64 : 0;
-    t.tby = text ? (t.text.bbox.dy() + 4 * kTextRows - 1) / (4 * kTextRows) : 0;
-    const long long blocks = (long long)t.nframes * (t.chunks[0] + t.chunks[1]) + (long long)t.nframes * t.tbx * t.tby;
+    t.tb = !text ? 0 : t.text.cover.cov1 ? cover_blocks(t.text.bbox, kTailThreads)
+                                         : t.tbx * ((t.text.bbox.dy() + 4 * kTextRows - 1) / (4 * kTextRows));
+    if (text && getenv("IPX_KS_DEBUG")) fprintf(stderr, "[ipx text] tail launch: %s, %d blocks per frame\n", t.text.cover.cov1 ? "coverage map" : "glyph walk", t.tb);
+    const long long blocks = (long long)t.nframes * (t.chunks[0] + t.chunks[1]) + (long long)t.nframes * t.tb;
     if (blocks <= 0) return hipSuccess;
     if (blocks > 0x7fffffffLL) return hipErrorInvalidValue;
     const int k0 = t.chunks[0] ? t.g[0].kind : t.g[1].kind, k1 = t.chunks[1] ? t.g[1].kind : k0;
@@ -112,3 +119,19 @@
 }
 
 }
+
+hipError_t launch_ks_tail(KsTailArgs t, hipStream_t s)
+{
+    if (t.nframes <= 0) return hipSuccess;
+#if IPX_TAIL_SPLIT
+    KsTailArgs exact = t, text = t;
+    exact.wm = nullptr;
+    for (int k = 0; k < 2; k++) { text.list[k] = nullptr; text.cap[k] = 0; }
+    const hipError_t e = tail_launch(exact, s);
+    return e == hipSuccess ? tail_launch(text, s) : e;
+#else
+    return tail_launch(t, s);
+#endif
+}
+
+}
diff --git a/imageprocessor_amd/csrc/ipx_runtime.hip b/imageprocessor_amd/csrc/ipx_runtime.hip
--- a/imageprocessor_amd/csrc/ipx_runtime.hip
+++ b/imageprocessor_amd/csrc/ipx_runtime.hip
@@ -197,13 +197,18 @@
     return IPX_OK;
 }
 
+DevCover cover_of(const ipx_glyphset *gs)
+{
+    return gs && env_int("IPX_TEXT_MAP", 1) != 0 ? gs->cover : DevCover{};
+}
+
 int dev_composite(hipStream_t s, uint8_t *dst, int dw, int dh, int dstride, size_t frame_stride,
                   int nframes, const ipx_glyphset *gs)
 {
     ClippedGlyphs c;
     int rc = glyphs_for_frame(gs, dw, dh, &c);
     if (rc) return rc;
-    IPX_HIP(launch_composite(dst, dstride, frame_stride, nframes, c.dev, c.n, c.bbox,
+    IPX_HIP(launch_composite(dst, dstride, frame_stride, nframes, c.dev, c.n, c.bbox, cover_of(gs),
                              gs->col[0] * 0x101u, gs->col[1] * 0x101u, gs->col[2] * 0x101u,
                              gs->col[3] * 0x101u, s));
     return IPX_OK;
@@ -712,10 +717,8 @@
 }
 IPX_CATCH_STATUS
 
-int ipx_glyphset_create(ipx_ctx *ctx, const ipx_glyph *glyphs, int n, const uint8_t col[4],
-                        ipx_glyphset **out) try
-{
-    IPX_ENTER(ctx);
+static int glyphset_make(ipx_ctx *ctx, const ipx_glyph *glyphs, int n, const uint8_t col[4], bool with_map, ipx_glyphset **out)
+{
     if (!out || n < 0 || (n && !glyphs) || !col) { set_error("ipx_glyphset_create: bad argument"); return IPX_ERR_INVALID; }
     if (n > kMaxGlyphs) { set_error("ipx_glyphset_create: %d glyphs exceed the limit of %d", n, kMaxGlyphs); return IPX_ERR_UNSUPPORTED; }
     *out = nullptr;
@@ -744,8 +747,27 @@
             return IPX_ERR_HIP;
         }
     }
+    CoverMap cm;
+    if (with_map) cover_build(gs->g.data(), gs->g.size(), blob.data(), &cm);
+    if (!cm.deep && !cm.planes.empty()) {
+        hipError_t e = hipMalloc((void **)&gs->cover_dev, cm.planes.size());
+        if (e == hipSuccess) e = hipMemcpy(gs->cover_dev, cm.planes.data(), cm.planes.size(), hipMemcpyHostToDevice);
+        if (e != hipSuccess) {
+            set_error("glyph coverage map upload failed: %s", hipGetErrorString(e));
+            ipx_glyphset_destroy(ctx, gs);
+            return IPX_ERR_HIP;
+        }
+        gs->cover = DevCover{gs->cover_dev, gs->cover_dev + cm.planes.size() / 2, cm.pitch, cm.box.x0, cm.box.y0, cm.box.x1, cm.box.y1};
+    }
     *out = gs;
     return IPX_OK;
+}
+
+int ipx_glyphset_create(ipx_ctx *ctx, const ipx_glyph *glyphs, int n, const uint8_t col[4],
+                        ipx_glyphset **out) try
+{
+    IPX_ENTER(ctx);
+    return glyphset_make(ctx, glyphs, n, col, true, out);
 }
 IPX_CATCH_STATUS
 
@@ -755,6 +777,7 @@
     (void)hipSetDevice(ctx ? ctx->device : gs->device);
     for (auto &kv : gs->clipped) if (kv.second.dev) (void)hipFree(kv.second.dev);
     if (gs->masks_dev) (void)hipFree(gs->masks_dev);
+    if (gs->cover_dev) (void)hipFree(gs->cover_dev);
     delete gs;
 }
 
@@ -865,7 +888,7 @@
     IPX_FRAME("ipx_composite_glyphs_rgba8", "destination", dst, dw, dh, dstride);
     if (!n || !dw || !dh) return IPX_OK;
     ipx_glyphset *gs = nullptr;
-    int rc = ipx_glyphset_create(ctx, glyphs, n, col, &gs);
+    int rc = glyphset_make(ctx, glyphs, n, col, false, &gs);
     if (rc) return rc;
     {
         LaneLease lane(ctx);
@@ -1266,7 +1289,7 @@
 {
     if (!wm || pl->glyphs.n <= 0 || !pl->p.glyphs) return hipSuccess;
     const uint8_t *c = pl->p.glyphs->col;
-    return launch_composite(wm, pl->p.sw * 4, wm_frame_stride, n, pl->glyphs.dev, pl->glyphs.n, pl->glyphs.bbox, c[0] * 0x101u, c[1] * 0x101u,
+    return launch_composite(wm, pl->p.sw * 4, wm_frame_stride, n, pl->glyphs.dev, pl->glyphs.n, pl->glyphs.bbox, cover_of(pl->p.glyphs), c[0] * 0x101u, c[1] * 0x101u,
                             c[2] * 0x101u, c[3] * 0x101u, s);
 }
 
@@ -1334,7 +1357,7 @@
         KsText text{}, *txt = nullptr;
         if (wm && pl->glyphs.n > 0 && pl->p.glyphs) {
             const uint8_t *c = pl->p.glyphs->col;
-            text = KsText{pl->glyphs.dev, pl->glyphs.n, pl->glyphs.bbox, c[0] * 0x101u, c[1] * 0x101u, c[2] * 0x101u, c[3] * 0x101u};
+            text = KsText{pl->glyphs.dev, pl->glyphs.n, pl->glyphs.bbox, c[0] * 0x101u, c[1] * 0x101u, c[2] * 0x101u, c[3] * 0x101u, cover_of(pl->p.glyphs)};
             txt = &text;
         }
         bool matched = false, text_done = false;
diff --git a/imageprocessor_amd/csrc/ipx_runtime_internal.h b/imageprocessor_amd/csrc/ipx_runtime_internal.h
--- a/imageprocessor_amd/csrc/ipx_runtime_internal.h
+++ b/imageprocessor_amd/csrc/ipx_runtime_internal.h
@@ -60,13 +60,6 @@
     static constexpr size_t kFlatChromaBytes = (size_t)64 << 10;
 };
 
-struct GlyphHost {
-    size_t mask_off;
-    int mw, mh;
-    Rect dr;
-    int mpx, mpy;
-};
-
 struct ClippedGlyphs {
     DevGlyph *dev = nullptr;
     int n = 0;
@@ -78,6 +71,8 @@
     std::vector<GlyphHost> g;
     uint8_t *masks_dev = nullptr;
     size_t masks_bytes = 0;
+    uint8_t *cover_dev = nullptr;
+    DevCover cover{};
     uint8_t col[4] = {0, 0, 0, 0};
     mutable std::mutex mu;
     mutable std::map<std::pair<int, int>, ClippedGlyphs> clipped;
diff --git a/include/ipx.h b/include/ipx.h
--- a/include/ipx.h
+++ b/include/ipx.h
@@ -108,6 +108,7 @@
 int ipx_glyphset_create(ipx_ctx *ctx, const ipx_glyph *glyphs, int n, const uint8_t col[4],
                         ipx_glyphset **out);
 void ipx_glyphset_destroy(ipx_ctx *ctx, ipx_glyphset *gs);
+int ipx_debug_cover_map(const ipx_glyph *glyphs, int n, ipx_rect *box, int *pitch, int *deep, uint8_t *planes, size_t planes_cap);
 int ipx_dev_composite_glyphs_rgba8(ipx_ctx *ctx, void *stream, uint8_t *dst, int dw, int dh,
                                    int dstride, const ipx_glyphset *gs);
 
```

After: 255,600 (median of 6 runs). Within noise of the previous version (+2.1%).
